# yzqin/s4g-release

Measured on AMD Instinct MI355X. Metric: scenes/sec (25.6k-pt clouds) end-to-end grasp inference, higher is better.
Workload: dtype f32 (f16x2 split)

## Files before the change

include/s4g_ops.h:

```cpp
#ifndef S4G_OPS_H_
#define S4G_OPS_H_

#include <stddef.h>
#include <stdint.h>

#ifdef __cplusplus
extern "C" {
#endif

#define S4G_ABI_VERSION 14


#define S4G_OK 0
#define S4G_EINVAL (-1)
#define S4G_EWORKSPACE (-2)
#define S4G_EUNSUPPORTED (-3)

#define S4G_FLAG_FMAD 1

typedef void *s4g_stream_t;

#define S4G_OP_FPS 1
#define S4G_OP_BALL_QUERY 2
#define S4G_OP_THREE_NN 3

int s4g_abi_version(void);
int s4g_build_variants(void);
int s4g_test_knobs_enabled(void);
const char *s4g_error_string(int code);

size_t s4g_workspace_bytes(int op, int64_t B, int64_t d0, int64_t d1, int64_t d2);

int s4g_fps_f32(const float *xyz_b3n, int64_t B, int64_t N, int64_t M,
                int64_t *idx_bm, void *ws, size_t ws_bytes, int flags,
                s4g_stream_t stream);

int s4g_ball_query_f32(const float *xyz_b3n, const float *ctr_b3m, int64_t B,
                       int64_t N, int64_t M, float radius, int64_t K,
                       int64_t *idx_bmk, int64_t *cnt_bm, void *ws,
                       size_t ws_bytes, int flags, s4g_stream_t stream);

int s4g_group_points_f32(const float *in_bcn, const int64_t *idx_bmk, int64_t B,
                         int64_t C, int64_t N, int64_t M, int64_t K,
                         float *out_bcmk, s4g_stream_t stream);

int s4g_group_points_xyz_f32(const float *xyz_b3n, const int64_t *idx_bmk, int64_t B, int64_t N,
                             int64_t M, int64_t K, float *out_b3mk, void *ws, size_t ws_bytes,
                             s4g_stream_t stream);
int s4g_group_points_ws_f32(const float *feat_bcn, const int64_t *idx_bmk, int64_t B, int64_t C,
                            int64_t N, int64_t M, int64_t K, float *out_bcmk, void *ws,
                            size_t ws_bytes, s4g_stream_t stream);
int s4g_group_points_backward_f32(const float *gout_bcmk,
                                  const int64_t *idx_bmk, int64_t B, int64_t C,
                                  int64_t N, int64_t M, int64_t K,
                                  float *gin_bcn, s4g_stream_t stream);

int s4g_gather_points_f32(const float *in_bcn, const int64_t *idx_bm, int64_t B,
                          int64_t C, int64_t N, int64_t M, float *out_bcm,
                          s4g_stream_t stream);

int s4g_three_nn_f32(const float *q_b3n1, const float *k_b3n2, int64_t B,
                     int64_t N1, int64_t N2, int64_t *idx_bn3, float *d2_bn3,
                     void *ws, size_t ws_bytes, int flags, s4g_stream_t stream);

int s4g_three_interpolate_f32(const float *feat_bcn2, const int64_t *idx_bn3,
                              const float *w_bn3, int64_t B, int64_t C,
                              int64_t N2, int64_t N1, float *out_bcn1,
                              int flags, s4g_stream_t stream);

int s4g_three_interpolate_ws_f32(const float *feat_bcn2, const int64_t *idx_bn3, const float *w_bn3,
                                 int64_t B, int64_t C, int64_t N2, int64_t N1, float *out_bcn1,
                                 void *ws, size_t ws_bytes, int flags, s4g_stream_t stream);
int s4g_interp_add_cl_f32(const float *y_pc, const float *sparse_rc, const int32_t *nidx_p3,
                          const float *nw_p3, const float *bias_c, int64_t B, int64_t N1, int64_t N2,
                          int64_t C, int relu, float *out_pc, float *out_amax64, s4g_stream_t stream);
int s4g_three_interpolate_backward_f32(const float *gout_bcn1,
                                       const int64_t *idx_bn3,
                                       const float *w_bn3, int64_t B, int64_t C,
                                       int64_t N2, int64_t N1, float *gin_bcn2,
                                       s4g_stream_t stream);

size_t s4g_scatter_det_workspace_bytes(int64_t B, int64_t N, int64_t T);
size_t s4g_scatter_det_workspace_bytes_c(int64_t B, int64_t C, int64_t N, int64_t T, int weighted);
int s4g_group_points_backward_det_f32(const float *gout_bcmk, const int64_t *idx_bmk, int64_t B, int64_t C,
                                      int64_t N, int64_t M, int64_t K, float *gin_bcn, void *ws,
                                      size_t ws_bytes, s4g_stream_t stream);
int s4g_three_interpolate_backward_det_f32(const float *gout_bcn1, const int64_t *idx_bn3, const float *w_bn3,
                                           int64_t B, int64_t C, int64_t N2, int64_t N1, float *gin_bcn2,
                                           void *ws, size_t ws_bytes, s4g_stream_t stream);

int s4g_interp_weights_f32(const float *d2_bn3, int64_t B, int64_t N1,
                           float eps, float *w_bn3, s4g_stream_t stream);


#define S4G_GEMM_LOAD_PLAIN 0
#define S4G_GEMM_LOAD_GATHER 1
#define S4G_GEMM_LOAD_INTERP 2
#define S4G_GEMM_LOAD_GATHER_MLP1 3
#define S4G_GEMM_LOAD_GATHER_ADD 4
#define S4G_GEMM_LOAD_INTERP_ADD 5
#define S4G_GEMM_LOAD_CHANNEL_FIRST 6
#define S4G_GEMM_EPI_STORE 0
#define S4G_GEMM_EPI_MAX 1
#define S4G_GEMM_EPI_CHANNEL_FIRST 2
#define S4G_GEMM_EPI_MAX_CHANNEL_FIRST 3
#define S4G_GEMM_FP32 0
#define S4G_GEMM_BF16X3 1
#define S4G_GEMM_BF16 2
#define S4G_GEMM_F16X2 3

typedef struct s4g_gemm_desc {
  int32_t loader, epilogue, groups, relu;
  int32_t P, Cin, Kpad, Cout;
  const float *W;
  const float *bias;
  int32_t w_gstride, b_gstride;
  const float *A;
  int32_t lda, a_coff, a_gcol;
  const int32_t *gidx;
  const float *feat;
  const float *xyz;
  const float *ctr;
  int32_t Cf, N, M, K;
  const int32_t *nidx;
  const float *nw;
  const float *sparse;
  const float *dense;
  int32_t C2, C1, N2, N1;
  float *out;
  int32_t ldc, c_coff, c_gcol;
  float *cf_ptr[4];
  int32_t cf_start[5];
  int32_t cf_sigmoid_from, cf_N;
  int32_t precision, Kpad16;
  const void *W_bf16x3;
  const float *mlp1_w;
  const void *W_f16x2;
  const float *w_inv_scale;
  const float *a_amax, *a_amax2;
  float a_amax_floor;
  float *out_amax;
  const void *W_f16x2_frag;
  const void *W2_f16x2_frag;
  const float *w2_inv_scale;
  const float *bias2;
  int32_t Cout2, relu2;
  const void *W3_f16x2_frag;
  const float *w3_inv_scale;
  const float *bias3;
  int32_t Cout3, relu3;
  const float *loader_bias;
  int32_t rows_per_scene;
  const float *rel_xyz4;
  const int32_t *seg4;
  const int32_t *seg_rows;
  float *out2;
  int32_t ldc2, split_n;
  float *out_amax2;
  int32_t a_L;
} s4g_gemm_desc_t;

int s4g_mlp_gemm_f32(const s4g_gemm_desc_t *desc, s4g_stream_t stream);

typedef struct s4g_heads_desc {
  int32_t precision, P, N, ldx;
  int32_t C, H0, H1, H2, H3;
  const float *X;
  const void *W_frag[5];
  const float *bias[5];
  const float *w_inv_scale[5];
  float *out[4];
  int32_t channels[4];
  int32_t sigmoid_head;
  const float *a_amax;
  float a_amax_floor;
  int32_t rows_per_scene;
  const void *pre_W_frag[2];
  const float *pre_bias[2];
  const float *pre_w_inv_scale[2];
  const int32_t *pre_nidx;
  const float *pre_nw;
  const float *pre_sparse;
  const float *pre_dense;
  const float *pre_lbias;
  const float *pre_a_amax2;
  int32_t pre_N2;
  int64_t out_batch_stride;
  int32_t head_mask;
} s4g_heads_desc_t;

int s4g_heads_chain_f32(const s4g_heads_desc_t *desc, s4g_stream_t stream);

int s4g_amax_per_scene_f32(const float *x, int64_t B, int64_t n_per_scene, float *out_slots, s4g_stream_t stream);

int s4g_gemm_chain_supported(int loader, int epilogue, int C, int Kpad16);

int s4g_ball_query_i32(const float *xyz_b3n, const float *ctr_b3m, int64_t B,
                       int64_t N, int64_t M, float radius, int64_t K,
                       int32_t *idx_bmk, int32_t *cnt_bm, void *ws,
                       size_t ws_bytes, int flags, s4g_stream_t stream);
int s4g_three_nn_weights_i32(const float *q_b3n1, const float *k_b3n2, int64_t B,
                             int64_t N1, int64_t N2, float eps, int32_t *idx_bn3,
                             float *w_bn3, void *ws, size_t ws_bytes, int flags,
                             s4g_stream_t stream);
size_t s4g_three_nn_grid_workspace_bytes(int64_t B, int64_t N1, int64_t N2);
size_t s4g_three_nn_grid_header_offset(int64_t B, int64_t N2);
int s4g_three_nn_weights_grid_i32(const float *q_b3n1, const float *k_b3n2, int64_t B,
                                  int64_t N1, int64_t N2, float eps, float cell,
                                  int32_t *idx_bn3, float *w_bn3, void *ws,
                                  size_t ws_bytes, int flags, s4g_stream_t stream);

int s4g_three_nn_grid_f32(const float *q_b3n1, const float *k_b3n2, int64_t B, int64_t N1,
                          int64_t N2, float cell, int64_t *idx_bn3, float *d2_bn3, void *ws,
                          size_t ws_bytes, int flags, s4g_stream_t stream);

int s4g_query_group_f32(const float *xyz_b3n, const float *ctr_b3m, int64_t B,
                        int64_t N, int64_t M, float radius, int64_t K,
                        int64_t *idx_bmk, int64_t *cnt_bm, float *grouped_b3mk,
                        void *ws, size_t ws_bytes, int flags, s4g_stream_t stream);

int s4g_group_rel_xyz_i32(const float *xyz_b3n, const float *ctr_b3m, const int32_t *idx_bmk,
                          int64_t B, int64_t N, int64_t M, int64_t K, float *rel_pk4,
                          s4g_stream_t stream);

int s4g_group_rel_xyz_unique_i32(const float *xyz_b3n, const float *ctr_b3m, const int32_t *idx_bmk,
                                 const int32_t *cnt_bm, int64_t B, int64_t N, int64_t M, int64_t K,
                                 float *rel_pk4, int32_t *seg4, int32_t *row_start_bm, int32_t *rows_b,
                                 s4g_stream_t stream);

int s4g_fps_gather_i32(const float *xyz_b3n, int64_t B, int64_t N, int64_t M,
                       int32_t *idx_bm, float *ctr_b3m, void *ws, size_t ws_bytes,
                       int flags, s4g_stream_t stream);

int s4g_fps_gather_ex_i32(const float *xyz_b3n, int64_t B, int64_t N, int64_t M, int32_t *idx_bm,
                          float *ctr_b3m, float *dist_bm, const int32_t *run_b, void *ws,
                          size_t ws_bytes, int flags, s4g_stream_t stream);
int s4g_fps_prefix_check_f32(const float *ctr_b3m, const float *dist_bm, int64_t B, int64_t M1,
                             int64_t M2, int32_t *run_b, int flags, s4g_stream_t stream);

int s4g_fps_prepass_f32(const float *xyz_b3n, int64_t B, int64_t N, int64_t G, int32_t *perm_bn,
                        float *gbox_bg6, s4g_stream_t stream);

int s4g_expected_score_f32(const float *logits_bcn, int64_t B, int64_t C, int64_t N,
                           const float *values_c, float *score_bn, s4g_stream_t stream);
int s4g_decode_poses_f32(const float *xyz_b3n, const float *frame_R_b9n,
                         const float *frame_t_btn, const int64_t *sel_bk, int64_t B,
                         int64_t N, int64_t K, int64_t TC, const float *t_bins,
                         float *H_bk44, s4g_stream_t stream);

int s4g_contact_heads_f32(const float *raw_b17m, const float *xyz_b3n, const int64_t *index_bm, int64_t B,
                          int64_t N, int64_t M, float *out_b20m, s4g_stream_t stream);
int s4g_decode_poses_abs_f32(const float *frame_R_b9n, const float *frame_t_b3n, const int64_t *sel_bk,
                             int64_t B, int64_t N, int64_t K, float *H_bk44, s4g_stream_t stream);

int s4g_collision_counts_f32(const float *xyz_b3n, const float *g2l_bk44, int64_t B,
                             int64_t N, int64_t K, const float *gripper6,
                             int32_t *counts_bk2, s4g_stream_t stream);
int s4g_collision_counts_n_f32(const float *xyz_b3n, const float *g2l_bk44, int64_t B, int64_t N,
                               int64_t K, const float *gripper6, const int64_t *pose_count_b,
                               int invert_se3, int32_t *counts_bk2, s4g_stream_t stream);

size_t s4g_eval_frames_workspace_bytes(int64_t B, int64_t N, int64_t K);
int s4g_eval_frames_f32(const float *xyz_b3n, const float *normals_b3n, const int32_t *labels_bn,
                        const float *g2l_bk44, int64_t B, int64_t N, int64_t K, const float *params10,
                        const int64_t *pose_count_b, int invert_se3, int32_t *ints_bk8, float *floats_bk5,
                        void *workspace, size_t workspace_bytes, s4g_stream_t stream);

size_t s4g_local_search_workspace_bytes(int64_t B, int64_t N, int64_t F, int64_t L, int64_t T);
int s4g_local_search_f32(const float *points_bf3, const float *frames_bf33, const float *xyz_b3n,
                         const float *normals_b3n, const int32_t *labels_bn, int64_t B, int64_t N, int64_t F,
                         int64_t L, int64_t T, const float *params13, int32_t no_label, const float *tables_3l2t,
                         const int64_t *frame_count_b, int32_t *ints_bfp6, float *scores_bfp, int32_t *slab_bfl,
                         int32_t *valid_bf, int32_t *valid_index_bf, int64_t *count_b, void *workspace,
                         size_t workspace_bytes, s4g_stream_t stream);

int s4g_best_placement_f32(const float *points_bf3, const float *frames_bf33, const float *scores_bfp,
                           const float *tables_3l2t, int64_t B, int64_t F, int64_t L, int64_t T, int32_t *index_bf,
                           float *score_bf, float *g2l_bf44, int32_t *valid_index_bf, int64_t *count_b,
                           s4g_stream_t stream);
size_t s4g_close_region_workspace_bytes(int64_t B, int64_t N, int64_t F, int64_t capacity);
int s4g_close_region_f32(const float *g2l_bf44, const float *xyz_b3n, const float *normals_b3n,
                         const int32_t *live_bf, const int64_t *frame_count_b, int64_t B, int64_t N, int64_t F,
                         int64_t capacity, int64_t R, const float *params13, int32_t *count_bf, int64_t *offset_bf1,
                         float *points_b3c, float *normals_b3c, int32_t *index_bc, float *maps_bf12rr,
                         int32_t *flags_bf, void *workspace, size_t workspace_bytes, s4g_stream_t stream);

size_t s4g_gpd_pack_bytes(int Cin, int classes);
int s4g_gpd_pack_f32(const float *conv1_w, const float *conv1_b, const float *conv2_w, const float *conv2_b,
                     const float *fc1_w, const float *fc1_b, const float *fc2_w, const float *fc2_b, int Cin, int classes,
                     void *packed, s4g_stream_t stream);
size_t s4g_gpd_workspace_bytes(int64_t chunk, int Cin, int classes);
int s4g_gpd_forward_f32(const float *maps, int64_t image_stride, int64_t channel_stride, const int32_t *index, int64_t G,
                        int64_t num_images, const void *packed, int Cin, int classes, int64_t chunk, float *pool1,
                        float *pool2, float *hidden, float *logits, void *workspace, size_t workspace_bytes,
                        s4g_stream_t stream);

size_t s4g_pngpd_pack_bytes(int classes);
int s4g_pngpd_pack_f32(const float *const *weights12, const float *const *biases12, int classes, void *packed,
                       s4g_stream_t stream);
size_t s4g_pngpd_workspace_bytes(int64_t chunk, int classes);
int s4g_pngpd_forward_f32(const float *points, int64_t set_stride, int64_t channel_stride, int64_t n_points,
                          const int64_t *offset, const int32_t *count, const int32_t *flags, int64_t F, int64_t capacity,
                          const int32_t *index, int64_t G, int64_t num_sets, const void *packed, int classes,
                          int64_t chunk, float *stn_global, float *trans, float *global_feat, float *hidden,
                          int32_t *status, float *logits, void *workspace, size_t workspace_bytes, s4g_stream_t stream);

size_t s4g_darboux_frames_workspace_bytes(int64_t B, int64_t N, int64_t F);
int s4g_darboux_frames_f32(const float *xyz_b3n, const float *normals_b3n, const int32_t *frame_index_bf,
                           const int64_t *frame_count_b, int64_t B, int64_t N, int64_t F, float radius,
                           int32_t min_neighbours, float *frames_bf33, float *points_bf3, int32_t *count_bf,
                           int32_t *flags_bf, void *workspace, size_t workspace_bytes, s4g_stream_t stream);

size_t s4g_match_normals_workspace_bytes(int64_t B, int64_t N, int64_t M);
int s4g_match_normals_f32(const float *query_b3n, const float *scene_b3m, const float *scene_normals_b3m,
                          const float *camera_b3 , int64_t B, int64_t N, int64_t M, float radius,
                          int32_t max_nn, float *normals_b3n, int32_t *count_bn, int32_t *flags_bn,
                          void *workspace, size_t workspace_bytes, s4g_stream_t stream);

size_t s4g_estimate_normals_workspace_bytes(int64_t B, int64_t N);
int s4g_estimate_normals_f32(const float *cloud_b3n, const float *camera_b3 ,
                             const int32_t *live_b , int64_t B, int64_t N, float radius,
                             int32_t max_nn, float *normals_b3n, int32_t *count_bn, int32_t *flags_bn,
                             void *workspace, size_t workspace_bytes, s4g_stream_t stream);

int s4g_match_nearest_f32(const float *query_b3n, const float *scene_b3m, int64_t B, int64_t N, int64_t M,
                          float radius, int32_t *nearest_bn, void *workspace, size_t workspace_bytes,
                          s4g_stream_t stream);

size_t s4g_contact_search_workspace_bytes(int64_t B, int64_t M, int64_t F, int64_t P);
int s4g_contact_search_f32(const float *g2l_bf44, const float *xyz_b3m, const int32_t *labels_bm, int64_t B, int64_t M,
                           int64_t F, int64_t nz, int64_t ny, int64_t nx, const float *params10, int32_t no_label,
                           const float *tables_2z3y2x, const int64_t *frame_count_b, int32_t *ints_bfp4,
                           int32_t *table_bf, int32_t *valid_bf, int32_t *label_bf, int32_t *fail_bf, void *workspace,
                           size_t workspace_bytes, s4g_stream_t stream);

int s4g_contact_select_f32(const int32_t *nearest_bn, const float *cloud_b3n, const float *scene_normals_b3m,
                           const float *camera_b3, const int32_t *offsets_bm1, const int32_t *order_bf,
                           const int32_t *valid_bf, const float *search_bf, const float *antipodal_bf, int64_t B,
                           int64_t N, int64_t M, int64_t F, float *normals_b3n, int32_t *best_frame_bn,
                           float *point_score_bn, int32_t *valid_index_bn, int64_t *count_b, s4g_stream_t stream);

size_t s4g_contact_pairs_workspace_bytes(int64_t B, int64_t N);
int s4g_contact_pairs_f32(const float *xyz_b3n, const float *normals_b3n, const int64_t *count_b, int64_t B, int64_t N,
                          int64_t max_pairs, double max_distance, double cos_threshold, int32_t *pairs_bp2,
                          float *pair_score_bp, int64_t *pair_count_b, int32_t *flags_b, void *workspace,
                          size_t workspace_bytes, s4g_stream_t stream);
size_t s4g_contact_pair_grade_workspace_bytes(int64_t B, int64_t N, int64_t P, int64_t T, int64_t W);
int s4g_contact_pair_grade_f32(const float *xyz_b3n, const int64_t *count_b, const int32_t *pairs_bp2,
                               const float *pair_score_bp, const int64_t *pair_count_b, int64_t B, int64_t N, int64_t P,
                               int64_t T, int64_t W, const float *params5, const double *gates3,
                               const float *tables_12t2w, int64_t max_frames, int32_t *counts_bptw3,
                               int32_t *close_plane_bp, float *score_bpt, int32_t *valid_bpt, int32_t *fail_bp,
                               float *g2l_bf44, float *search_score_bf, float *antipodal_score_bf,
                               int32_t *frame_source_bf, int32_t *frame_point_index_bf, int64_t *frame_count_b,
                               int32_t *flags_b, void *workspace, size_t workspace_bytes, s4g_stream_t stream);

size_t s4g_darboux_object_frames_workspace_bytes(int64_t B, int64_t N);
int s4g_darboux_object_frames_f32(const float *xyz_b3n, const float *normals_b3n, const int64_t *count_b, int64_t B,
                                  int64_t N, float radius, int32_t min_neighbours, float *frames_bn33,
                                  float *inv_frames_bn33, int32_t *neighbours_bn, int32_t *flags_bn, void *workspace,
                                  size_t workspace_bytes, s4g_stream_t stream);
size_t s4g_darboux_object_grade_workspace_bytes(int64_t B, int64_t N, int64_t F, int64_t L, int64_t T, int64_t S);
int s4g_darboux_object_grade_f32(const float *xyz_b3n, const float *normals_b3n, const int64_t *count_b,
                                 const float *frames_bf33, const float *inv_frames_bf33, const int32_t *frame_index_bf,
                                 int64_t B, int64_t N, int64_t F, int64_t L, int64_t T, int64_t S, const float *params9,
                                 const float *tables_3l2t2s, int32_t *search_bf2lt, float *antipodal_bf2lt,
                                 int32_t *counts_bf2lts3, int32_t *slab_bf2l, int32_t *fail_bf2, void *workspace,
                                 size_t workspace_bytes, s4g_stream_t stream);

size_t s4g_sort_pairs_workspace_bytes(int64_t n);
int s4g_sort_pairs_u32(uint32_t *keys_in, uint32_t *vals_in, int64_t n, int bits, uint32_t *keys_out,
                       uint32_t *vals_out, void *ws, size_t ws_bytes, s4g_stream_t stream);
size_t s4g_exclusive_scan_workspace_bytes(int64_t n);
int s4g_exclusive_scan_i32(const int32_t *in, int32_t *out, int64_t n, void *ws, size_t ws_bytes,
                           s4g_stream_t stream);

int s4g_crop_indices_f32(const float *xyz_3n, int64_t N, const float *workspace6,
// ... 33 lines not shown
```

s4g_release_amd/_cabi.py:

```python
import ctypes
import os

_HERE = os.path.dirname(os.path.abspath(__file__))
LIB_PATH = os.environ.get("S4G_HIP_LIB") or os.path.join(_HERE, "libs4g_hip.so")

S4G_ABI_VERSION = 14
S4G_EINVAL = -1
S4G_EWORKSPACE = -2
S4G_EUNSUPPORTED = -3
S4G_FLAG_FMAD = 1
S4G_OP_FPS, S4G_OP_BALL_QUERY, S4G_OP_THREE_NN = 1, 2, 3

_vp = ctypes.c_void_p
_i64 = ctypes.c_int64
_sz = ctypes.c_size_t
_int = ctypes.c_int
_f32 = ctypes.c_float

_i32 = ctypes.c_int32


class GemmDesc(ctypes.Structure):
    _fields_ = [
        ("loader", _i32), ("epilogue", _i32), ("groups", _i32), ("relu", _i32),
        ("P", _i32), ("Cin", _i32), ("Kpad", _i32), ("Cout", _i32),
        ("W", _vp), ("bias", _vp), ("w_gstride", _i32), ("b_gstride", _i32),
        ("A", _vp), ("lda", _i32), ("a_coff", _i32), ("a_gcol", _i32),
        ("gidx", _vp), ("feat", _vp), ("xyz", _vp), ("ctr", _vp),
        ("Cf", _i32), ("N", _i32), ("M", _i32), ("K", _i32),
        ("nidx", _vp), ("nw", _vp), ("sparse", _vp), ("dense", _vp),
        ("C2", _i32), ("C1", _i32), ("N2", _i32), ("N1", _i32),
        ("out", _vp), ("ldc", _i32), ("c_coff", _i32), ("c_gcol", _i32),
        ("cf_ptr", _vp * 4), ("cf_start", _i32 * 5), ("cf_sigmoid_from", _i32), ("cf_N", _i32),
        ("precision", _i32), ("Kpad16", _i32), ("W_bf16x3", _vp), ("mlp1_w", _vp),
        ("W_f16x2", _vp), ("w_inv_scale", _vp), ("a_amax", _vp), ("a_amax2", _vp),
        ("a_amax_floor", _f32), ("out_amax", _vp), ("W_f16x2_frag", _vp),
        ("W2_f16x2_frag", _vp), ("w2_inv_scale", _vp), ("bias2", _vp), ("Cout2", _i32), ("relu2", _i32),
        ("W3_f16x2_frag", _vp), ("w3_inv_scale", _vp), ("bias3", _vp), ("Cout3", _i32), ("relu3", _i32),
        ("loader_bias", _vp), ("rows_per_scene", _i32), ("rel_xyz4", _vp), ("seg4", _vp), ("seg_rows", _vp),
        ("out2", _vp), ("ldc2", _i32), ("split_n", _i32), ("out_amax2", _vp),
        ("a_L", _i32),
    ]


class HeadsDesc(ctypes.Structure):
    _fields_ = [
        ("precision", _i32), ("P", _i32), ("N", _i32), ("ldx", _i32),
        ("C", _i32), ("H0", _i32), ("H1", _i32), ("H2", _i32), ("H3", _i32),
        ("X", _vp), ("W_frag", _vp * 5), ("bias", _vp * 5), ("w_inv_scale", _vp * 5),
        ("out", _vp * 4), ("channels", _i32 * 4), ("sigmoid_head", _i32),
        ("a_amax", _vp), ("a_amax_floor", _f32), ("rows_per_scene", _i32),
        ("pre_W_frag", _vp * 2), ("pre_bias", _vp * 2), ("pre_w_inv_scale", _vp * 2),
        ("pre_nidx", _vp), ("pre_nw", _vp), ("pre_sparse", _vp), ("pre_dense", _vp),
        ("pre_lbias", _vp), ("pre_a_amax2", _vp), ("pre_N2", _i32), ("out_batch_stride", _i64), ("head_mask", _i32),
    ]


SIGNATURES = {
    "s4g_mlp_gemm_f32": (_int, [ctypes.POINTER(GemmDesc), _vp]),
    "s4g_heads_chain_f32": (_int, [ctypes.POINTER(HeadsDesc), _vp]),
    "s4g_ball_query_i32": (_int, [_vp, _vp, _i64, _i64, _i64, _f32, _i64, _vp, _vp, _vp, _sz,
                                  _int, _vp]),
    "s4g_three_nn_weights_i32": (_int, [_vp, _vp, _i64, _i64, _i64, _f32, _vp, _vp, _vp, _sz,
                                        _int, _vp]),
    "s4g_three_nn_grid_workspace_bytes": (_sz, [_i64, _i64, _i64]),
    "s4g_three_nn_grid_header_offset": (_sz, [_i64, _i64]),
    "s4g_three_nn_weights_grid_i32": (_int, [_vp, _vp, _i64, _i64, _i64, _f32, _f32, _vp, _vp, _vp,
                                             _sz, _int, _vp]),
    "s4g_three_nn_grid_f32": (_int, [_vp, _vp, _i64, _i64, _i64, _f32, _vp, _vp, _vp, _sz, _int, _vp]),
    "s4g_group_points_xyz_f32": (_int, [_vp, _vp, _i64, _i64, _i64, _i64, _vp, _vp, _sz, _vp]),
    "s4g_gemm_chain_supported": (_int, [_int, _int, _int, _int]),
    "s4g_amax_per_scene_f32": (_int, [_vp, _i64, _i64, _vp, _vp]),
    "s4g_interp_add_cl_f32": (_int, [_vp, _vp, _vp, _vp, _vp, _i64, _i64, _i64, _i64, _int, _vp, _vp, _vp]),
    "s4g_group_points_ws_f32": (_int, [_vp, _vp, _i64, _i64, _i64, _i64, _i64, _vp, _vp, _sz, _vp]),
    "s4g_three_interpolate_ws_f32": (_int, [_vp, _vp, _vp, _i64, _i64, _i64, _i64, _vp, _vp, _sz, _int, _vp]),
    "s4g_fps_gather_i32": (_int, [_vp, _i64, _i64, _i64, _vp, _vp, _vp, _sz, _int, _vp]),
    "s4g_fps_prepass_f32": (_int, [_vp, _i64, _i64, _i64, _vp, _vp, _vp]),
    "s4g_fps_gather_ex_i32": (_int, [_vp, _i64, _i64, _i64, _vp, _vp, _vp, _vp, _vp, _sz, _int, _vp]),
    "s4g_fps_prefix_check_f32": (_int, [_vp, _vp, _i64, _i64, _i64, _vp, _int, _vp]),
    "s4g_build_variants": (_int, []),
    "s4g_test_knobs_enabled": (_int, []),
    "s4g_fps_f64": (_int, [_vp, _i64, _i64, _i64, _vp, _vp, _sz, _int, _vp]),
    "s4g_ball_query_f64": (_int, [_vp, _vp, _i64, _i64, _i64, _f32, _i64, _vp, _vp, _int, _vp]),
    "s4g_three_nn_f64": (_int, [_vp, _vp, _i64, _i64, _i64, _vp, _vp, _int, _vp]),
    "s4g_group_points_f64": (_int, [_vp, _vp, _i64, _i64, _i64, _i64, _i64, _vp, _vp]),
    "s4g_group_points_backward_f64": (_int, [_vp, _vp, _i64, _i64, _i64, _i64, _i64, _vp, _vp]),
    "s4g_three_interpolate_f64": (_int, [_vp, _vp, _vp, _i64, _i64, _i64, _i64, _vp, _int, _vp]),
    "s4g_three_interpolate_backward_f64": (_int, [_vp, _vp, _vp, _i64, _i64, _i64, _i64, _vp, _vp]),
    "s4g_scatter_det_workspace_bytes": (_sz, [_i64, _i64, _i64]),
    "s4g_scatter_det_workspace_bytes_c": (_sz, [_i64, _i64, _i64, _i64, _int]),
    "s4g_group_points_backward_det_f32": (_int, [_vp, _vp, _i64, _i64, _i64, _i64, _i64, _vp, _vp, _sz, _vp]),
    "s4g_three_interpolate_backward_det_f32": (_int, [_vp, _vp, _vp, _i64, _i64, _i64, _i64, _vp, _vp, _sz, _vp]),
    "s4g_group_rel_xyz_i32": (_int, [_vp, _vp, _vp, _i64, _i64, _i64, _i64, _vp, _vp]),
    "s4g_group_rel_xyz_unique_i32": (_int, [_vp, _vp, _vp, _vp, _i64, _i64, _i64, _i64, _vp, _vp, _vp, _vp, _vp]),
    "s4g_expected_score_f32": (_int, [_vp, _i64, _i64, _i64, _vp, _vp, _vp]),
    "s4g_decode_poses_f32": (_int, [_vp, _vp, _vp, _vp, _i64, _i64, _i64, _i64, _vp, _vp, _vp]),
    "s4g_contact_heads_f32": (_int, [_vp, _vp, _vp, _i64, _i64, _i64, _vp, _vp]),
    "s4g_decode_poses_abs_f32": (_int, [_vp, _vp, _vp, _i64, _i64, _i64, _vp, _vp]),
    "s4g_collision_counts_f32": (_int, [_vp, _vp, _i64, _i64, _i64, ctypes.POINTER(ctypes.c_float),
                                        _vp, _vp]),
    "s4g_collision_counts_n_f32": (_int, [_vp, _vp, _i64, _i64, _i64, ctypes.POINTER(ctypes.c_float),
                                          _vp, _int, _vp, _vp]),
    "s4g_eval_frames_workspace_bytes": (_sz, [_i64, _i64, _i64]),
    "s4g_eval_frames_f32": (_int, [_vp, _vp, _vp, _vp, _i64, _i64, _i64, ctypes.POINTER(ctypes.c_float), _vp, _int,
                                   _vp, _vp, _vp, _sz, _vp]),
    "s4g_local_search_workspace_bytes": (_sz, [_i64, _i64, _i64, _i64, _i64]),
    "s4g_local_search_f32": (_int, [_vp, _vp, _vp, _vp, _vp, _i64, _i64, _i64, _i64, _i64,
                                    ctypes.POINTER(ctypes.c_float), _i32, _vp, _vp, _vp, _vp, _vp, _vp, _vp, _vp, _vp,
                                    _sz, _vp]),
    "s4g_best_placement_f32": (_int, [_vp, _vp, _vp, _vp, _i64, _i64, _i64, _i64, _vp, _vp, _vp, _vp, _vp, _vp]),
    "s4g_close_region_workspace_bytes": (_sz, [_i64, _i64, _i64, _i64]),
    "s4g_close_region_f32": (_int, [_vp, _vp, _vp, _vp, _vp, _i64, _i64, _i64, _i64, _i64,
                                    ctypes.POINTER(ctypes.c_float), _vp, _vp, _vp, _vp, _vp, _vp, _vp, _vp, _sz, _vp]),
    "s4g_gpd_pack_bytes": (_sz, [_int, _int]),
    "s4g_gpd_pack_f32": (_int, [_vp, _vp, _vp, _vp, _vp, _vp, _vp, _vp, _int, _int, _vp, _vp]),
    "s4g_gpd_workspace_bytes": (_sz, [_i64, _int, _int]),
    "s4g_gpd_forward_f32": (_int, [_vp, _i64, _i64, _vp, _i64, _i64, _vp, _int, _int, _i64, _vp, _vp, _vp, _vp, _vp, _sz,
                                   _vp]),
    "s4g_pngpd_pack_bytes": (_sz, [_int]),
    "s4g_pngpd_pack_f32": (_int, [_vp, _vp, _int, _vp, _vp]),
    "s4g_pngpd_workspace_bytes": (_sz, [_i64, _int]),
    "s4g_pngpd_forward_f32": (_int, [_vp, _i64, _i64, _i64, _vp, _vp, _vp, _i64, _i64, _vp, _i64, _i64, _vp, _int, _i64,
                                     _vp, _vp, _vp, _vp, _vp, _vp, _vp, _sz, _vp]),
    "s4g_darboux_frames_workspace_bytes": (_sz, [_i64, _i64, _i64]),
    "s4g_darboux_frames_f32": (_int, [_vp, _vp, _vp, _vp, _i64, _i64, _i64, _f32, _i32, _vp, _vp, _vp, _vp, _vp, _sz,
                                      _vp]),
    "s4g_match_normals_workspace_bytes": (_sz, [_i64, _i64, _i64]),
    "s4g_match_normals_f32": (_int, [_vp, _vp, _vp, _vp, _i64, _i64, _i64, _f32, _i32, _vp, _vp, _vp, _vp, _sz, _vp]),
    "s4g_match_nearest_f32": (_int, [_vp, _vp, _i64, _i64, _i64, _f32, _vp, _vp, _sz, _vp]),
    "s4g_estimate_normals_workspace_bytes": (_sz, [_i64, _i64]),
    "s4g_estimate_normals_f32": (_int, [_vp, _vp, _vp, _i64, _i64, _f32, _i32, _vp, _vp, _vp, _vp, _sz, _vp]),
    "s4g_contact_search_workspace_bytes": (_sz, [_i64, _i64, _i64, _i64]),
    "s4g_contact_search_f32": (_int, [_vp, _vp, _vp, _i64, _i64, _i64, _i64, _i64, _i64, ctypes.POINTER(ctypes.c_float),
                                      _i32, _vp, _vp, _vp, _vp, _vp, _vp, _vp, _vp, _sz, _vp]),
    "s4g_contact_select_f32": (_int, [_vp, _vp, _vp, _vp, _vp, _vp, _vp, _vp, _vp, _i64, _i64, _i64, _i64, _vp, _vp,
                                      _vp, _vp, _vp, _vp]),
    "s4g_contact_pairs_workspace_bytes": (_sz, [_i64, _i64]),
    "s4g_contact_pairs_f32": (_int, [_vp, _vp, _vp, _i64, _i64, _i64, ctypes.c_double, ctypes.c_double, _vp, _vp, _vp,
                                     _vp, _vp, _sz, _vp]),
    "s4g_contact_pair_grade_workspace_bytes": (_sz, [_i64, _i64, _i64, _i64, _i64]),
    "s4g_contact_pair_grade_f32": (_int, [_vp, _vp, _vp, _vp, _vp, _i64, _i64, _i64, _i64, _i64,
                                          ctypes.POINTER(ctypes.c_float), ctypes.POINTER(ctypes.c_double), _vp, _i64,
                                          _vp, _vp, _vp, _vp, _vp, _vp, _vp, _vp, _vp, _vp, _vp, _vp, _vp, _sz, _vp]),
    "s4g_darboux_object_frames_workspace_bytes": (_sz, [_i64, _i64]),
    "s4g_darboux_object_frames_f32": (_int, [_vp, _vp, _vp, _i64, _i64, _f32, _i32, _vp, _vp, _vp, _vp, _vp, _sz, _vp]),
    "s4g_darboux_object_grade_workspace_bytes": (_sz, [_i64, _i64, _i64, _i64, _i64, _i64]),
    "s4g_darboux_object_grade_f32": (_int, [_vp, _vp, _vp, _vp, _vp, _vp, _i64, _i64, _i64, _i64, _i64, _i64,
                                            ctypes.POINTER(ctypes.c_float), _vp, _vp, _vp, _vp, _vp, _vp, _vp, _sz,
                                            _vp]),
    "s4g_sort_pairs_workspace_bytes": (_sz, [_i64]),
    "s4g_sort_pairs_u32": (_int, [_vp, _vp, _i64, _int, _vp, _vp, _vp, _sz, _vp]),
    "s4g_exclusive_scan_workspace_bytes": (_sz, [_i64]),
    "s4g_exclusive_scan_i32": (_int, [_vp, _vp, _i64, _vp, _sz, _vp]),
    "s4g_query_group_f32": (_int, [_vp, _vp, _i64, _i64, _i64, _f32, _i64, _vp, _vp, _vp, _vp, _sz,
                                   _int, _vp]),
    "s4g_crop_indices_f32": (_int, [_vp, _i64, ctypes.POINTER(ctypes.c_float), _vp, _vp, _vp]),
    "s4g_voxel_down_sample_workspace_bytes": (_sz, [_i64]),
    "s4g_voxel_down_sample_f32": (_int, [_vp, _i64, _f32, ctypes.POINTER(ctypes.c_float),
                                         ctypes.POINTER(ctypes.c_int32), _vp, _vp, _vp, _sz, _vp]),
    "s4g_radius_outlier_workspace_bytes": (_sz, [_i64]),
    "s4g_radius_outlier_mask_f32": (_int, [_vp, _i64, _f32, _i32, _vp, _vp, _sz, _int, _vp]),
    "s4g_abi_version": (_int, []),
    "s4g_error_string": (ctypes.c_char_p, [_int]),
    "s4g_workspace_bytes": (_sz, [_int, _i64, _i64, _i64, _i64]),
    "s4g_fps_f32": (_int, [_vp, _i64, _i64, _i64, _vp, _vp, _sz, _int, _vp]),
    "s4g_ball_query_f32": (_int, [_vp, _vp, _i64, _i64, _i64, _f32, _i64, _vp, _vp, _vp, _sz,
                                  _int, _vp]),
    "s4g_group_points_f32": (_int, [_vp, _vp, _i64, _i64, _i64, _i64, _i64, _vp, _vp]),
    "s4g_group_points_backward_f32": (_int, [_vp, _vp, _i64, _i64, _i64, _i64, _i64, _vp, _vp]),
    "s4g_gather_points_f32": (_int, [_vp, _vp, _i64, _i64, _i64, _i64, _vp, _vp]),
    "s4g_three_nn_f32": (_int, [_vp, _vp, _i64, _i64, _i64, _vp, _vp, _vp, _sz, _int, _vp]),
    "s4g_three_interpolate_f32": (_int, [_vp, _vp, _vp, _i64, _i64, _i64, _i64, _vp, _int, _vp]),
    "s4g_three_interpolate_backward_f32": (_int, [_vp, _vp, _vp, _i64, _i64, _i64, _i64, _vp,
                                                  _vp]),
    "s4g_interp_weights_f32": (_int, [_vp, _i64, _i64, _f32, _vp, _vp]),
}

_lib = None


def lib():
    global _lib
    if _lib is not None:
        return _lib
    if not os.path.exists(LIB_PATH):
        raise RuntimeError(
            "libs4g_hip.so not found at %s -- build it with "
            "`python -c 'import __graft_entry__ as g; g.build()'` or "
            "`make -C s4g_release_amd/csrc`. There is no CPU fallback." % LIB_PATH)
    import torch
    if os.environ.get("S4G_HIP_LIB"):
        import warnings
        warnings.warn("S4G_HIP_LIB overrides the shipped library: loading %s" % LIB_PATH, RuntimeWarning,
                      stacklevel=2)
    L = ctypes.CDLL(LIB_PATH)
    for name, (res, args) in SIGNATURES.items():
        try:
            fn = getattr(L, name)
        except AttributeError:
            raise RuntimeError("libs4g_hip.so does not export %s" % name)
        fn.restype = res
        fn.argtypes = args
    ver = L.s4g_abi_version()
    if ver != S4G_ABI_VERSION:
        raise RuntimeError("libs4g_hip.so ABI version %d != expected %d" % (ver, S4G_ABI_VERSION))
    _lib = L
    return _lib


def knob(name, default=None):
    if os.environ.get("S4G_TEST_KNOBS") != "1":
        return default
    return os.environ.get(name, default)


def check(code, what):
    if code != 0:
        msg = lib().s4g_error_string(code)
        raise RuntimeError("%s failed: %s (code %d)" % (what, msg.decode() if msg else "?", code))
```

s4g_release_amd/csrc/group.hip:

```cpp
#include "s4g_common.h"

namespace s4g {

constexpr int GP_THREADS = 256;
constexpr int GP_CG = 8;

__global__ __launch_bounds__(GP_THREADS) void group_points_vec4_kernel(
    const float* __restrict__ in, const int64_t* __restrict__ idx, int C, int N,
    int64_t MK, float* __restrict__ out) {
  const int b = blockIdx.z;
  const int c0 = blockIdx.y * GP_CG;
  const int64_t t4 = ((int64_t)blockIdx.x * GP_THREADS + threadIdx.x) * 4;
  if (t4 >= MK) return;
  const longlong2* ip =
      reinterpret_cast<const longlong2*>(idx + (size_t)b * MK + t4);
  const longlong2 a = ip[0], c = ip[1];
  const int j0 = (int)a.x, j1 = (int)a.y, j2 = (int)c.x, j3 = (int)c.y;
  const int cend = min(c0 + GP_CG, C);
  for (int ch = c0; ch < cend; ++ch) {
    const float* __restrict__ src = in + ((size_t)b * C + ch) * N;
    float4 v;
    v.x = src[j0];
    v.y = src[j1];
    v.z = src[j2];
// ... 6 lines not shown
                                                                float4* __restrict__ aos) {
  const int j = blockIdx.x * GP_THREADS + threadIdx.x;
  const int b = blockIdx.y;
  if (j >= N) return;
  const float* p = in + (size_t)b * 3 * N;
  aos[(size_t)b * N + j] = make_float4(p[j], p[N + j], p[2 * (size_t)N + j], 0.f);
}

__global__ __launch_bounds__(GP_THREADS) void group_xyz_aos_kernel(const float4* __restrict__ aos,
                                                                   const int64_t* __restrict__ idx,
                                                                   int N, int64_t MK,
                                                                   float* __restrict__ out) {
  const int b = blockIdx.y;
  const int64_t t4 = ((int64_t)blockIdx.x * GP_THREADS + threadIdx.x) * 4;
  if (t4 >= MK) return;
  const longlong2* ip = reinterpret_cast<const longlong2*>(idx + (size_t)b * MK + t4);
  const longlong2 a = ip[0], c = ip[1];
  const float4* __restrict__ src = aos + (size_t)b * N;
  const float4 p0 = src[(int)a.x], p1 = src[(int)a.y], p2 = src[(int)c.x], p3 = src[(int)c.y];
  float* o = out + (size_t)b * 3 * MK + t4;
  *reinterpret_cast<float4*>(o) = make_float4(p0.x, p1.x, p2.x, p3.x);
  *reinterpret_cast<float4*>(o + MK) = make_float4(p0.y, p1.y, p2.y, p3.y);
  *reinterpret_cast<float4*>(o + 2 * MK) = make_float4(p0.z, p1.z, p2.z, p3.z);
}

__global__ __launch_bounds__(GP_THREADS) void group_rel_xyz_kernel(const float* __restrict__ xyz,
                                                                   const float* __restrict__ ctr,
                                                                   const int* __restrict__ idx, int N,
                                                                   int M, int K,
                                                                   float4* __restrict__ out) {
  const int b = blockIdx.y;
  const int64_t MK = (int64_t)M * K;
  const int64_t t = (int64_t)blockIdx.x * GP_THREADS + threadIdx.x;
  if (t >= MK) return;
  const int m = (int)(t / K);
  const int j = idx[(size_t)b * MK + t];
  const float* __restrict__ x = xyz + (size_t)b * 3 * N;
  const float* __restrict__ c = ctr + (size_t)b * 3 * M;
  out[(size_t)b * MK + t] = make_float4(__fsub_rn(x[j], c[m]), __fsub_rn(x[N + j], c[M + m]),
                                        __fsub_rn(x[2 * (size_t)N + j], c[2 * (size_t)M + m]), 0.f);
}

constexpr int GU_THREADS = 1024, GU_TILE = 256;
__global__ __launch_bounds__(GU_THREADS) void group_unique_scan_kernel(const int* __restrict__ cnt, int M, int K,
                                                                       int* __restrict__ row_start,
                                                                       int* __restrict__ rows,
                                                                       float4* __restrict__ out,
                                                                       int* __restrict__ seg4) {
  __shared__ int wsum[GU_THREADS / 64];
  __shared__ int total_s;
  const int b = blockIdx.x, t = threadIdx.x, lane = t & 63, wave = t >> 6;
  const int per = (M + GU_THREADS - 1) / GU_THREADS;
  const int m0 = t * per;
  int local = 0;
  for (int i = 0; i < per; ++i) {
    const int m = m0 + i;
    if (m < M) local += (max(cnt[(size_t)b * M + m], 1) + 3) & ~3;
  }
  int incl = local;
#pragma unroll
  for (int o = 1; o < 64; o <<= 1) {
    const int v = __shfl_up(incl, o);
    if (lane >= o) incl += v;
  }
  if (lane == 63) wsum[wave] = incl;
  __syncthreads();
  if (t == 0) {
    int run = 0;
    for (int w = 0; w < GU_THREADS / 64; ++w) {
      const int v = wsum[w];
      wsum[w] = run;
      run += v;
    }
    total_s = run;
  }
  __syncthreads();
  int start = wsum[wave] + incl - local;
  for (int i = 0; i < per; ++i) {
    const int m = m0 + i;
    if (m < M) {
      row_start[(size_t)b * M + m] = start;
      start += (max(cnt[(size_t)b * M + m], 1) + 3) & ~3;
    }
  }
  if (total_s > (int)((int64_t)M * K / 8 * 7) || (total_s + GU_TILE - 1) / GU_TILE * GU_TILE >= M * K) {
    for (int i = 0; i < per; ++i) {
      const int m = m0 + i;
      if (m < M) row_start[(size_t)b * M + m] = m * K;
    }
    if (t == 0) rows[b] = M * K;
    return;
  }
  const int total = total_s;
  const int padded = (total + GU_TILE - 1) / GU_TILE * GU_TILE;
  if (t == 0) rows[b] = padded;
  const size_t base = (size_t)b * M * K;
  for (int r = total + t; r < padded; r += GU_THREADS) {
    out[base + r] = make_float4(0.f, 0.f, 0.f, 0.f);
    if ((r & 3) == 0) seg4[(base + r) >> 2] = -1;
  }
}

__global__ __launch_bounds__(GP_THREADS) void group_rel_unique_kernel(const float* __restrict__ xyz,
                                                                      const float* __restrict__ ctr,
                                                                      const int* __restrict__ idx,
                                                                      const int* __restrict__ cnt,
                                                                      const int* __restrict__ row_start,
                                                                      const int* __restrict__ rows, int N,
                                                                      int M, int K, float4* __restrict__ out,
                                                                      int* __restrict__ seg4) {
  const int b = blockIdx.y;
  const int64_t MK = (int64_t)M * K;
  const int64_t t = (int64_t)blockIdx.x * GP_THREADS + threadIdx.x;
  if (t >= MK) return;
  const int m = (int)(t / K), k = (int)(t - (int64_t)m * K);
  const int c4 = rows[b] == M * K ? K : (max(cnt[(size_t)b * M + m], 1) + 3) & ~3;
  if (k >= c4) return;
  const int j = idx[(size_t)b * MK + t];
  const float* __restrict__ x = xyz + (size_t)b * 3 * N;
  const float* __restrict__ c = ctr + (size_t)b * 3 * M;
  const size_t row = (size_t)b * MK + row_start[(size_t)b * M + m] + k;
  out[row] = make_float4(__fsub_rn(x[j], c[m]), __fsub_rn(x[N + j], c[M + m]),
                         __fsub_rn(x[2 * (size_t)N + j], c[2 * (size_t)M + m]), 0.f);
  if ((k & 3) == 0) seg4[row >> 2] = b * M + m;
}

__global__ __launch_bounds__(GP_THREADS) void group_points_scalar_kernel(
    const float* __restrict__ in, const int64_t* __restrict__ idx, int C, int N,
    int64_t MK, float* __restrict__ out) {
  const int b = blockIdx.z;
  const int c0 = blockIdx.y * GP_CG;
  const int64_t t = (int64_t)blockIdx.x * GP_THREADS + threadIdx.x;
  if (t >= MK) return;
  const int j = (int)idx[(size_t)b * MK + t];
  const int cend = min(c0 + GP_CG, C);
  for (int ch = c0; ch < cend; ++ch)
    out[((size_t)b * C + ch) * MK + t] = in[((size_t)b * C + ch) * N + j];
}

__global__ __launch_bounds__(GP_THREADS) void group_points_backward_kernel(
    const float* __restrict__ gout, const int64_t* __restrict__ idx, int C,
    int N, int64_t MK, float* __restrict__ gin) {
  const int b = blockIdx.z;
  const int c0 = blockIdx.y * GP_CG;
  const int64_t t = (int64_t)blockIdx.x * GP_THREADS + threadIdx.x;
  if (t >= MK) return;
  const int j = (int)idx[(size_t)b * MK + t];
  const int cend = min(c0 + GP_CG, C);
  for (int ch = c0; ch < cend; ++ch)
    atomicAdd(gin + ((size_t)b * C + ch) * N + j,
              gout[((size_t)b * C + ch) * MK + t]);
}

}

extern "C" int s4g_group_points_f32(const float* in_bcn,
                                    const int64_t* idx_bmk, int64_t B,
                                    int64_t C, int64_t N, int64_t M, int64_t K,
                                    float* out_bcmk, s4g_stream_t stream) {
  if (B < 0 || C < 0 || N <= 0 || M < 0 || K < 0 || B > 65535 ||
      N >= (1ll << 31))
    return S4G_EINVAL;
  const int64_t MK = M * K;
  if (B == 0 || C == 0 || MK == 0) return S4G_OK;
  if (!in_bcn || !idx_bmk || !out_bcmk) return S4G_EINVAL;
  hipStream_t st = (hipStream_t)stream;
  const unsigned gy = (unsigned)((C + s4g::GP_CG - 1) / s4g::GP_CG);
  if (gy > 65535) return S4G_EINVAL;
  const bool aligned = ((uintptr_t)idx_bmk % 16 == 0) && ((uintptr_t)out_bcmk % 16 == 0);
  if (MK % 4 == 0 && aligned) {
    const dim3 grid((unsigned)((MK / 4 + s4g::GP_THREADS - 1) / s4g::GP_THREADS),
                    gy, (unsigned)B);
    hipLaunchKernelGGL(s4g::group_points_vec4_kernel, grid,
                       dim3(s4g::GP_THREADS), 0, st, in_bcn, idx_bmk, (int)C,
                       (int)N, MK, out_bcmk);
  } else {
    const dim3 grid((unsigned)((MK + s4g::GP_THREADS - 1) / s4g::GP_THREADS),
                    gy, (unsigned)B);
    hipLaunchKernelGGL(s4g::group_points_scalar_kernel, grid,
                       dim3(s4g::GP_THREADS), 0, st, in_bcn, idx_bmk, (int)C,
                       (int)N, MK, out_bcmk);
  }
  S4G_LAUNCH_CHECK();
  return S4G_OK;
}

extern "C" int s4g_group_points_xyz_f32(const float* xyz_b3n, const int64_t* idx_bmk, int64_t B,
                                        int64_t N, int64_t M, int64_t K, float* out_b3mk,
                                        void* ws, size_t ws_bytes, s4g_stream_t stream) {
  const int64_t MK = M * K;
  const bool aligned = ((uintptr_t)idx_bmk % 16 == 0) && ((uintptr_t)out_b3mk % 16 == 0) &&
                       ((uintptr_t)ws % 16 == 0);
  if (!ws || ws_bytes < (size_t)B * (size_t)N * sizeof(float4) || MK % 4 != 0 || !aligned ||
      B <= 0 || B > 65535 || N <= 0 || N >= (1ll << 31) || MK == 0)
    return s4g_group_points_f32(xyz_b3n, idx_bmk, B, 3, N, M, K, out_b3mk, stream);
  if (!xyz_b3n || !idx_bmk || !out_b3mk) return S4G_EINVAL;
  hipStream_t st = (hipStream_t)stream;
  float4* aos = (float4*)ws;
  hipLaunchKernelGGL(s4g::xyz_to_aos_kernel, dim3((unsigned)((N + s4g::GP_THREADS - 1) / s4g::GP_THREADS), (unsigned)B),
                     dim3(s4g::GP_THREADS), 0, st, xyz_b3n, (int)N, aos);
  S4G_LAUNCH_CHECK();
  hipLaunchKernelGGL(s4g::group_xyz_aos_kernel,
                     dim3((unsigned)((MK / 4 + s4g::GP_THREADS - 1) / s4g::GP_THREADS), (unsigned)B),
                     dim3(s4g::GP_THREADS), 0, st, aos, idx_bmk, (int)N, MK, out_b3mk);
  S4G_LAUNCH_CHECK();
  return S4G_OK;
}

extern "C" int s4g_group_rel_xyz_i32(const float* xyz_b3n, const float* ctr_b3m, const int32_t* idx_bmk,
                                     int64_t B, int64_t N, int64_t M, int64_t K, float* rel_pk4,
                                     s4g_stream_t stream) {
  if (B < 0 || N <= 0 || M < 0 || K < 0 || B > 65535 || N >= (1ll << 31) || M * K >= (1ll << 31))
    return S4G_EINVAL;
  const int64_t MK = M * K;
  if (B == 0 || MK == 0) return S4G_OK;
  if (!xyz_b3n || !ctr_b3m || !idx_bmk || !rel_pk4 || ((uintptr_t)rel_pk4 & 15)) return S4G_EINVAL;
  hipStream_t st = (hipStream_t)stream;
  hipLaunchKernelGGL(s4g::group_rel_xyz_kernel,
                     dim3((unsigned)((MK + s4g::GP_THREADS - 1) / s4g::GP_THREADS), (unsigned)B),
                     dim3(s4g::GP_THREADS), 0, st, xyz_b3n, ctr_b3m, idx_bmk, (int)N, (int)M, (int)K,
                     reinterpret_cast<float4*>(rel_pk4));
  S4G_LAUNCH_CHECK();
  return S4G_OK;
}

extern "C" int s4g_group_rel_xyz_unique_i32(const float* xyz_b3n, const float* ctr_b3m, const int32_t* idx_bmk,
                                            const int32_t* cnt_bm, int64_t B, int64_t N, int64_t M, int64_t K,
                                            float* rel_pk4, int32_t* seg4, int32_t* row_start_bm,
                                            int32_t* rows_b, s4g_stream_t stream) {
  if (B < 0 || N <= 0 || M < 0 || K < 0 || B > 65535 || N >= (1ll << 31) || B * M * K >= (1ll << 31))
    return S4G_EINVAL;
  const int64_t MK = M * K;
  if (B == 0 || MK == 0) return S4G_OK;
  if ((K & 3) || (MK % s4g::GU_TILE) || M > s4g::GU_THREADS * 64) return S4G_EUNSUPPORTED;
  if (!xyz_b3n || !ctr_b3m || !idx_bmk || !cnt_bm || !rel_pk4 || !seg4 || !row_start_bm || !rows_b ||
      ((uintptr_t)rel_pk4 & 15))
    return S4G_EINVAL;
  hipStream_t st = (hipStream_t)stream;
  hipLaunchKernelGGL(s4g::group_unique_scan_kernel, dim3((unsigned)B), dim3(s4g::GU_THREADS), 0, st, cnt_bm, (int)M,
                     (int)K, row_start_bm, rows_b, reinterpret_cast<float4*>(rel_pk4), seg4);
  S4G_LAUNCH_CHECK();
  hipLaunchKernelGGL(s4g::group_rel_unique_kernel,
                     dim3((unsigned)((MK + s4g::GP_THREADS - 1) / s4g::GP_THREADS), (unsigned)B),
                     dim3(s4g::GP_THREADS), 0, st, xyz_b3n, ctr_b3m, idx_bmk, cnt_bm, row_start_bm, rows_b, (int)N, (int)M,
                     (int)K, reinterpret_cast<float4*>(rel_pk4), seg4);
  S4G_LAUNCH_CHECK();
  return S4G_OK;
}

extern "C" int s4g_group_points_backward_f32(const float* gout_bcmk,
                                             const int64_t* idx_bmk, int64_t B,
                                             int64_t C, int64_t N, int64_t M,
                                             int64_t K, float* gin_bcn,
                                             s4g_stream_t stream) {
  if (B < 0 || C < 0 || N <= 0 || M < 0 || K < 0 || B > 65535 ||
      N >= (1ll << 31))
    return S4G_EINVAL;
  if (B == 0 || C == 0) return S4G_OK;
  if (!gin_bcn) return S4G_EINVAL;
  hipStream_t st = (hipStream_t)stream;
  hipError_t e = hipMemsetAsync(gin_bcn, 0, sizeof(float) * (size_t)(B * C * N), st);
  if (e != hipSuccess) return (int)e;
  const int64_t MK = M * K;
  if (MK == 0) return S4G_OK;
  if (!gout_bcmk || !idx_bmk) return S4G_EINVAL;
  const unsigned gy = (unsigned)((C + s4g::GP_CG - 1) / s4g::GP_CG);
  if (gy > 65535) return S4G_EINVAL;
  const dim3 grid((unsigned)((MK + s4g::GP_THREADS - 1) / s4g::GP_THREADS), gy,
                  (unsigned)B);
  hipLaunchKernelGGL(s4g::group_points_backward_kernel, grid,
                     dim3(s4g::GP_THREADS), 0, st, gout_bcmk, idx_bmk, (int)C,
                     (int)N, MK, gin_bcn);
  S4G_LAUNCH_CHECK();
  return S4G_OK;
}

extern "C" int s4g_gather_points_f32(const float* in_bcn, const int64_t* idx_bm,
                                     int64_t B, int64_t C, int64_t N, int64_t M,
                                     float* out_bcm, s4g_stream_t stream) {
  return s4g_group_points_f32(in_bcn, idx_bm, B, C, N, M, 1, out_bcm, stream);
}
```

s4g_release_amd/csrc/mlp_gemm.hip:

```cpp
#include <stdlib.h>

#include "mlp_common.h"

#include <type_traits>

#ifndef S4G_CHAIN_ABLATE
#define S4G_CHAIN_ABLATE 0
#endif

namespace s4g {


constexpr int GM_BM = 128;
constexpr int GM_BN = 128;
constexpr int GM_BK = 32;
constexpr int GM_LDS = 36;
constexpr int GM_THREADS = 256;

enum { LOAD_PLAIN = 0, LOAD_GATHER = 1, LOAD_INTERP = 2, LOAD_GATHER_MLP1 = 3, LOAD_GATHER_ADD = 4,
       LOAD_INTERP_ADD = 5, LOAD_CHANNEL_FIRST = 6,
       LOAD_REL_MLP1 = 64,
       LOAD_ADD_MFMA0 = 65 };
enum { EPI_STORE = 0, EPI_MAX = 1, EPI_CHANNEL_FIRST = 2, EPI_MAX_CF = 3 };

struct GemmParams {
  int P, Cin, Kpad, Cout, relu;
  const float* W;
  const float* bias;
  const float* A;
  int lda, a_coff, a_gcol;
  int aL;
  const int* gidx;
  const float* feat;
  const float* xyz;
  const float* ctr;
  int Cf, N, M, K;
  int nscenes;
  const float4* mlp1;
  const float4* rel4;
  const int* seg4;
  const int* seg_rows;
  float* out2;
  int ldc2, split_n;
  uint32_t* out_amax2;
  const int* nidx;
  const float* nw;
  const float* sparse;
  const float* dense;
  int C2, C1, N2, N1;
  float* out;
  int ldc, c_coff, c_gcol;
  int w_gstride, b_gstride;
  float* cf_ptr[4];
  int cf_start[5];
  int cf_sigmoid_from;
  int cf_N;
  int mtiles, ntiles;
  const uint16_t* W3;
  int Kpad16;
  int bf16_single;
  size_t w3_plane;
  const uint16_t* Wh2;
  const float* w_inv_scale;
  const float* a_amax;
  const float* a_amax2;
  float a_amax_floor;
  uint32_t* out_amax;
  int rps;
  const uint16_t* Wfrag;
  const float* lbias;
  const uint16_t* Wfrag2;
  const float* w_inv_scale2;
  const float* bias2;
  int Cout2, relu2;
  const uint16_t* Wfrag3;
  const float* w_inv_scale3;
  const float* bias3;
  int Cout3, relu3;
};

__device__ __forceinline__ float4 f4zero() { return make_float4(0.f, 0.f, 0.f, 0.f); }

__device__ __forceinline__ void gather_row_bm(int M, int K, int p0, int r, int& b, int& m) {
  const int MK = M * K;
  const int b0 = __builtin_amdgcn_readfirstlane(p0 / MK);
  int rem = p0 - b0 * MK + r;
  b = b0;
  while (rem >= MK) {
    rem -= MK;
    ++b;
  }
  m = (K & (K - 1)) == 0 ? rem >> (31 - __clz(K)) : rem / K;
}

template <int LOADER, int RPT = 4, int RS = 32>
struct ALoader {
  static __device__ __forceinline__ int srow(int t) { return LOADER == LOAD_CHANNEL_FIRST ? (t & 31) : (t >> 3); }
  static __device__ __forceinline__ int chunk(int t) { return LOADER == LOAD_CHANNEL_FIRST ? (t >> 5) : (t & 7); }
  const float* src0[RPT];
  bool ok[RPT];
  float rel[RPT][3];
  int i3[RPT][3];
  float w3[RPT][3];
  size_t drow[RPT];

  __device__ __forceinline__ void init(const GemmParams& p, int p0, int g, int t) {
    constexpr bool GATHERS = LOADER == LOAD_GATHER_MLP1 || LOADER == LOAD_GATHER_ADD || LOADER == LOAD_GATHER;
    int pp_[RPT], j_[RPT], b_[RPT], m_[RPT];
#pragma unroll
    for (int s = 0; s < RPT; ++s) {
      const int r = srow(t) + RS * s;
      const int pos = p0 + r;
      ok[s] = pos < p.P;
      pp_[s] = ok[s] ? pos : 0;
      j_[s] = b_[s] = m_[s] = 0;
      if constexpr (GATHERS) {
        if (!(LOADER == LOAD_GATHER_MLP1 && p.rel4)) {
          gather_row_bm(p.M, p.K, p0, ok[s] ? r : 0, b_[s], m_[s]);
          j_[s] = p.gidx[pp_[s]];
        }
      }
    }
#pragma unroll
    for (int s = 0; s < RPT; ++s) {
      const int pp = pp_[s], j = j_[s], b = b_[s], m = m_[s];
      if constexpr (LOADER == LOAD_PLAIN) {
        src0[s] = p.A + (size_t)pp * p.lda + p.a_coff + g * p.a_gcol;
      } else if constexpr (LOADER == LOAD_CHANNEL_FIRST) {
        const int b = pp / p.aL;
        src0[s] = p.A + (size_t)b * p.Cin * p.aL + (pp - b * p.aL);
      } else if constexpr (LOADER == LOAD_GATHER_MLP1) {
        if (p.rel4) {
          const float4 r4 = p.rel4[pp];
          rel[s][0] = r4.x;
          rel[s][1] = r4.y;
          rel[s][2] = r4.z;
          continue;
        }
        const float* x = p.xyz + (size_t)b * 3 * p.N;
        const float* c = p.ctr + (size_t)b * 3 * p.M;
        rel[s][0] = __fsub_rn(x[j], c[m]);
        rel[s][1] = __fsub_rn(x[p.N + j], c[p.M + m]);
        rel[s][2] = __fsub_rn(x[2 * p.N + j], c[2 * p.M + m]);
      } else if constexpr (LOADER == LOAD_GATHER_ADD) {
        src0[s] = p.feat + ((size_t)b * p.N + j) * p.Cf;
        const float* x = p.xyz + (size_t)b * 3 * p.N;
        const float* c = p.ctr + (size_t)b * 3 * p.M;
        rel[s][0] = __fsub_rn(x[j], c[m]);
        rel[s][1] = __fsub_rn(x[p.N + j], c[p.M + m]);
        rel[s][2] = __fsub_rn(x[2 * p.N + j], c[2 * p.M + m]);
      } else if constexpr (LOADER == LOAD_GATHER) {
        src0[s] = p.feat ? p.feat + ((size_t)b * p.N + j) * p.Cf : nullptr;
        if ((t & 7) == ((p.Cf & 31) >> 2)) {
          const float* x = p.xyz + (size_t)b * 3 * p.N;
          const float* c = p.ctr + (size_t)b * 3 * p.M;
          rel[s][0] = __fsub_rn(x[j], c[m]);
          rel[s][1] = __fsub_rn(x[p.N + j], c[p.M + m]);
          rel[s][2] = __fsub_rn(x[2 * p.N + j], c[2 * p.M + m]);
        }
      } else {
        const int bq = pp / p.N1;
#pragma unroll
        for (int k = 0; k < 3; ++k) {
          i3[s][k] = bq * p.N2 + p.nidx[(size_t)pp * 3 + k];
          w3[s][k] = p.nw[(size_t)pp * 3 + k];
        }
        drow[s] = (size_t)pp;
      }
    }
  }

  __device__ __forceinline__ float4 load(const GemmParams& p, int s, int k0, int t) const {
    if constexpr (LOADER == LOAD_GATHER_MLP1) {
      const bool live = ok[s] && k0 < p.Cin;
      const int kk = k0 < p.Cin ? k0 : 0;
      float4 r;
      float* rp = reinterpret_cast<float*>(&r);
#pragma unroll
      for (int e = 0; e < 4; ++e) {
        const float4 w = p.mlp1[kk + e];
        const float v = __fmaf_rn(w.z, rel[s][2], __fmaf_rn(w.y, rel[s][1], __fmaf_rn(w.x, rel[s][0], w.w)));
        rp[e] = live ? fmaxf(v, 0.f) : 0.f;
      }
      return r;
    }
    if constexpr (LOADER == LOAD_GATHER_ADD) {
      const bool live = ok[s] && k0 < p.Cin;
      const int kk = k0 < p.Cin ? k0 : 0;
      const float4 f = *reinterpret_cast<const float4*>(src0[s] + kk);
      const float fv[4] = {f.x, f.y, f.z, f.w};
      float4 r;
      float* rp = reinterpret_cast<float*>(&r);
#pragma unroll
      for (int e = 0; e < 4; ++e) {
        const float4 w = p.mlp1[kk + e];
        const float v = __fmaf_rn(w.z, rel[s][2], __fmaf_rn(w.y, rel[s][1], __fmaf_rn(w.x, rel[s][0], w.w)));
        rp[e] = live ? fmaxf(__fadd_rn(fv[e], v), 0.f) : 0.f;
      }
      return r;
    }
    if (!ok[s]) return f4zero();
    if constexpr (LOADER == LOAD_PLAIN) {
      if (k0 >= p.Cin) return f4zero();
      return *reinterpret_cast<const float4*>(src0[s] + k0);
    } else if constexpr (LOADER == LOAD_CHANNEL_FIRST) {
      float v[4];
#pragma unroll
      for (int e = 0; e < 4; ++e) v[e] = k0 + e < p.Cin ? src0[s][(size_t)(k0 + e) * p.aL] : 0.f;
      return make_float4(v[0], v[1], v[2], v[3]);
    } else if constexpr (LOADER == LOAD_INTERP_ADD) {
      if (k0 >= p.Cin) return f4zero();
      const float4 a = *reinterpret_cast<const float4*>(p.sparse + (size_t)i3[s][0] * p.C2 + k0);
      const float4 b = *reinterpret_cast<const float4*>(p.sparse + (size_t)i3[s][1] * p.C2 + k0);
      const float4 c = *reinterpret_cast<const float4*>(p.sparse + (size_t)i3[s][2] * p.C2 + k0);
      const float4 bb = *reinterpret_cast<const float4*>(p.lbias + k0);
      float4 y = f4zero();
      if (p.dense) y = *reinterpret_cast<const float4*>(p.dense + drow[s] * p.C2 + k0);
      const float av[4] = {a.x, a.y, a.z, a.w}, bv[4] = {b.x, b.y, b.z, b.w}, cv[4] = {c.x, c.y, c.z, c.w};
      const float yv[4] = {y.x, y.y, y.z, y.w}, bi[4] = {bb.x, bb.y, bb.z, bb.w};
      float4 r;
      float* rp = reinterpret_cast<float*>(&r);
#pragma unroll
      for (int e = 0; e < 4; ++e) {
        float acc = __fmul_rn(av[e], w3[s][0]);
        acc = __fadd_rn(acc, __fmul_rn(bv[e], w3[s][1]));
        acc = __fadd_rn(acc, __fmul_rn(cv[e], w3[s][2]));
        rp[e] = fmaxf(__fadd_rn(__fadd_rn(yv[e], acc), bi[e]), 0.f);
      }
      return r;
    } else if constexpr (LOADER == LOAD_GATHER) {
      if (k0 < p.Cf) return *reinterpret_cast<const float4*>(src0[s] + k0);
      if (k0 == p.Cf) return make_float4(rel[s][0], rel[s][1], rel[s][2], 0.f);
      return f4zero();
    } else {
      if (k0 < p.C2) {
        const float4 a = *reinterpret_cast<const float4*>(p.sparse + (size_t)i3[s][0] * p.C2 + k0);
        const float4 b = *reinterpret_cast<const float4*>(p.sparse + (size_t)i3[s][1] * p.C2 + k0);
        const float4 c = *reinterpret_cast<const float4*>(p.sparse + (size_t)i3[s][2] * p.C2 + k0);
        float4 r;
        r.x = __fadd_rn(__fadd_rn(__fmul_rn(a.x, w3[s][0]), __fmul_rn(b.x, w3[s][1])), __fmul_rn(c.x, w3[s][2]));
        r.y = __fadd_rn(__fadd_rn(__fmul_rn(a.y, w3[s][0]), __fmul_rn(b.y, w3[s][1])), __fmul_rn(c.y, w3[s][2]));
        r.z = __fadd_rn(__fadd_rn(__fmul_rn(a.z, w3[s][0]), __fmul_rn(b.z, w3[s][1])), __fmul_rn(c.z, w3[s][2]));
        r.w = __fadd_rn(__fadd_rn(__fmul_rn(a.w, w3[s][0]), __fmul_rn(b.w, w3[s][1])), __fmul_rn(c.w, w3[s][2]));
        return r;
      }
// ... 572 lines not shown
#pragma unroll
    for (int pl = 0; pl < PL; ++pl)
#pragma unroll
      for (int s = 0; s < WPT; ++s)
        rw[pl][s] = (wlive && wok[s])
                        ? *reinterpret_cast<const uint4*>(Wg + pl * p.w3_plane + woff[s] + kt * BK)
                        : make_uint4(0u, 0u, 0u, 0u);
  };
  auto lstore = [&]() {
#pragma unroll
    for (int s = 0; s < RPT; ++s) {
      uint16_t* dst = Ah + (srow + RS * s) * GH_STR + (((chunk >> 1) ^ ((srow >> 2) & 3)) * 8) + (chunk & 1) * 4;
      if constexpr (PL == 2) {
        uint2 h, l;
        split2_h<LOADER == LOAD_GATHER>(ra[s], sa, h, l);
        *reinterpret_cast<uint2*>(dst) = h;
        *reinterpret_cast<uint2*>(dst + APLANE) = l;
      } else {
        *reinterpret_cast<uint2*>(dst) = make_uint2(cvt_pk_bf16(ra[s].x, ra[s].y), cvt_pk_bf16(ra[s].z, ra[s].w));
      }
    }
#pragma unroll
    for (int pl = 0; pl < PL; ++pl)
#pragma unroll
      for (int s = 0; s < WPT; ++s)
        *reinterpret_cast<uint4*>(Wh + pl * WPLANE + (wrow + WRS * s) * GH_STR +
                                  ((wchunk ^ ((wrow >> 2) & 3)) * 8)) = rw[pl][s];
  };

#define S4G_H2_TERM(PA, PB)                                                        \
  acc[0][cp] = chain_mfma<PL>(af[0][PA], bf[0][PB], acc[0][cp]);                     \
  acc[0][cp + 1] = chain_mfma<PL>(af[0][PA], bf[1][PB], acc[0][cp + 1]);             \
  acc[1][cp] = chain_mfma<PL>(af[1][PA], bf[0][PB], acc[1][cp]);                     \
  acc[1][cp + 1] = chain_mfma<PL>(af[1][PA], bf[1][PB], acc[1][cp + 1]);
  auto compute_ks = [&](int ks) {
    uint4 af[2][PL];
#pragma unroll
    for (int rb = 0; rb < 2; ++rb)
#pragma unroll
      for (int pl = 0; pl < PL; ++pl)
        af[rb][pl] = *reinterpret_cast<const uint4*>(Ah + pl * APLANE + a_row + rb * 32 * GH_STR + f_off[ks]);
#pragma unroll
    for (int cp = 0; cp < NCB; cp += 2) {
      uint4 bf[2][PL];
#pragma unroll
      for (int cb = 0; cb < 2; ++cb)
#pragma unroll
        for (int pl = 0; pl < PL; ++pl)
          bf[cb][pl] = *reinterpret_cast<const uint4*>(Wh + pl * WPLANE + b_row + (cp + cb) * 32 * GH_STR + f_off[ks]);
      if constexpr (PL == 2) {
        S4G_H2_TERM(0, 1)
        S4G_H2_TERM(1, 0)
      }
      S4G_H2_TERM(0, 0)
    }
  };

  gload(0);
  for (int kt = 0; kt < ntile_k; ++kt) {
    lstore();
    __syncthreads();
    if (kt + 1 < ntile_k) gload(kt + 1);
    const int krem = p.Kpad16 - kt * BK;
    const int nks = krem >= BK ? 2 : 1;
    for (int ks = 0; ks < nks; ++ks) compute_ks(ks);
    __syncthreads();
  }
#undef S4G_H2_TERM

  float tmax = 0.f;
#pragma unroll
  for (int cb = 0; cb < NCB; ++cb) {
    const int n = n0 + wc * 32 * NCB + cb * 32 + li;
    const bool nok = n < p.Cout;
    const float sc = nok ? (PL == 2 ? inv_sa * p.w_inv_scale[(size_t)g * p.b_gstride + n] : 1.f) : 0.f;
    const float bias = nok ? bg[n] : 0.f;
    float mx = -__builtin_inff(), mn = __builtin_inff();
#pragma unroll
    for (int rb = 0; rb < 2; ++rb)
#pragma unroll
      for (int r = 0; r < 16; ++r) {
        const float v = acc[rb][cb][r] * sc;
        acc[rb][cb][r] = v;
        mx = fmaxf(mx, v);
        mn = fminf(mn, v);
      }
    const float hi = mx + bias, lo = mn + bias;
    tmax = fmaxf(tmax, p.relu ? hi : fmaxf(fabsf(hi), fabsf(lo)));
  }
  if (PL == 2 && po.out_amax) {
    const uint32_t wm = wave_max_u32(__float_as_uint(fmaxf(tmax, 0.f)));
    if (lane == 0) amax_publish(po.out_amax, wm, blockIdx.x * 4 + wave, p0, p_hi, p.rps);
  }
  if constexpr (EPI == EPI_MAX_CF)
    max_cf_epilogue<NCB>(po, acc, bg, p0, n0, wr, wc, li, lh, smemf);
  else
    gemm_epilogue<EPI, NCB>(po, acc, bg, g, p0, n0, wave, wr, wc, li, lh, smemf);
}

template <int LOADER, int EPI, int NCB, int PL>
static int launch_gemm_f16x2_cfg(GemmParams p, int groups, hipStream_t st) {
  constexpr int BN = 64 * NCB;
  p.ntiles = (p.Cout + BN - 1) / BN;
  size_t lds = sizeof(uint16_t) * PL * (GM_BM + BN) * GH_STR;
  const size_t epi = sizeof(float) * 4 * 32 * (32 * NCB + 4);
  if (lds < epi) lds = epi;
  static LdsAttrCache lds_cache;
  if (int rc = allow_dynamic_lds(reinterpret_cast<const void*>(&mlp_gemm_f16x2_kernel<LOADER, EPI, NCB, PL>), lds, lds_cache)) return rc;
  const dim3 grid((unsigned)(p.mtiles * p.ntiles), (unsigned)groups);
  hipLaunchKernelGGL((mlp_gemm_f16x2_kernel<LOADER, EPI, NCB, PL>), grid, dim3(256), lds, st, p);
  S4G_LAUNCH_CHECK();
  return S4G_OK;
}

__device__ __forceinline__ void chain_keep_alive(const f32x16& v) { asm volatile("" ::"v"(v)); }

#ifdef S4G_CHAIN_STAMPS
__device__ unsigned long long g_chain_stamps[512 * 16];
#define S4G_STAMP(i)                                                                       \
  do {                                                                                     \
    const unsigned sb_ = gridDim.x >= 1024 ? blockIdx.x - gridDim.x / 2 : blockIdx.x;    \
    if (threadIdx.x == 0 && sb_ < 512u && blockIdx.y == 0)                                 \
      g_chain_stamps[sb_ * 16 + (i)] = __builtin_amdgcn_s_memtime();                      \
  } while (0)
#else
#define S4G_STAMP(i)
#endif
constexpr int GF_RING_F16X2 = 2;
#ifndef S4G_CHAIN_RING1
#define S4G_CHAIN_RING1 2
#endif
#ifndef S4G_CHAIN_BF16_NRB
#define S4G_CHAIN_BF16_NRB 4
#endif

template <int LOADER, int EPI2, int RW, int KC, int PL>
__global__ __launch_bounds__(RW == 8 ? 512 : 256, (PL == 1 && RW != 8 && S4G_CHAIN_BF16_NRB == 2) ? 3 : 2) void mlp_chain_kernel(const GemmParams p) {
  constexpr int GF_RING = PL == 2 ? GF_RING_F16X2 : S4G_CHAIN_RING1;
  constexpr int NRB = PL == 1 ? S4G_CHAIN_BF16_NRB : 2, WROWS = 32 * NRB;
  constexpr int CW = RW == 8 ? 8 : 4 / RW, RWN = RW == 8 ? 1 : RW;
  constexpr int BM = WROWS * RWN, K = 64 * CW, NW = RWN * CW;
  constexpr int RS = 8 * NW, RPT = BM / RS;
  constexpr int astr = K + 8, aplane = BM * astr, KS = K >> 4;
  extern __shared__ __attribute__((aligned(16))) float smemf[];
  uint16_t* Ah = reinterpret_cast<uint16_t*>(smemf);
  float* scr = reinterpret_cast<float*>(Ah + PL * aplane);
  const int g = blockIdx.y;

  const int t = threadIdx.x;
  const int lane = t & 63;
  const int wave = t >> 6;

  constexpr bool ADD0 = LOADER == LOAD_ADD_MFMA0;
  constexpr bool ADD_BOUNDS = LOADER == LOAD_GATHER_ADD || LOADER == LOAD_INTERP_ADD || ADD0;
  constexpr bool MFMA0 = LOADER == LOAD_REL_MLP1;
  static_assert(!(MFMA0 || ADD0) || (PL == 2 && KC == 1), "phase 0 on the matrix cores: f16x2, one panel");
  static_assert(!ADD0 || EPI2 == EPI_MAX, "a wave's 64 rows are one centroid's neighbours");
  constexpr bool SEGMAX = (LOADER == LOAD_GATHER_MLP1 || MFMA0) && EPI2 == EPI_MAX;
  const int tile = blockIdx.x;
  const int p0 = tile * BM;
  bool seg_scene = false;
  if constexpr (SEGMAX) {
    if (p.seg_rows) {
      const int sc = p0 / p.rps;
      const int nrows = p.seg_rows[sc];
      if (p0 - sc * p.rps >= nrows) return;
      seg_scene = nrows < p.rps;
    }
  }
  const int p_hi = min(p0 + BM, p.P) - 1;
  const int am_s0 = p.rps > 0 ? p0 / p.rps : 0, am_s1 = p.rps > 0 ? p_hi / p.rps : 0;
  float am_v1 = 0.f, am_v2 = 0.f;
  if (PL == 2 && p.a_amax) am_v1 = p.a_amax[(size_t)am_s0 * 64 + lane];
  if (PL == 2 && p.a_amax2) am_v2 = p.a_amax2[(size_t)am_s0 * 64 + lane];

  const int wr = wave / CW, wc = wave % CW;
  const int li = lane & 31, lh = lane >> 5;
  const int wc_u = __builtin_amdgcn_readfirstlane(wc);
  const uint32_t wf_lane = (uint32_t)lane * 16u;
  constexpr size_t cb_stride = (size_t)KS * PL * 1024;
  constexpr size_t strip_stride = (size_t)CW * 2 * cb_stride;
  constexpr int kchunks = KC;
  const size_t cbs1 = (size_t)kchunks * cb_stride;
  const WRef w1 = wref(p.Wfrag + (size_t)g * p.Cout * p.Kpad16 * PL, (size_t)(wc_u * 2) * cbs1);
  const bool tri = p.Wfrag3 != nullptr;
  const WRef wmid = wref(p.Wfrag2 + (size_t)g * p.Cout2 * K * PL, (size_t)(wc_u * 2) * cb_stride);
  const int CoutF = tri ? p.Cout3 : p.Cout2;
  const float* __restrict__ scF = PL == 2 ? (tri ? p.w_inv_scale3 : p.w_inv_scale2) + (size_t)g * CoutF : nullptr;
  const float* __restrict__ bgF = (tri ? p.bias3 : p.bias2) + (size_t)g * CoutF;
  const WRef w2 = tri ? wref(p.Wfrag3 + (size_t)g * CoutF * K * PL, (size_t)(wc_u * 2) * cb_stride) : wmid;
  const int nstrip2 = (CoutF + 64 * CW - 1) / (64 * CW);
  const bool active0 = wc_u * 64 < CoutF;

  uint4 ring[GF_RING][2][PL];
#pragma unroll
  for (int d = 0; d < GF_RING; ++d)
#pragma unroll
    for (int cb = 0; cb < 2; ++cb)
#pragma unroll
      for (int pl = 0; pl < PL; ++pl)
        ring[d][cb][pl] = wref_load(w1, wf_lane + pl * 1024, (uint32_t)(cb * cbs1 + (size_t)d * PL * 1024));

  S4G_STAMP(0);
  ALoader<LOADER, RPT, RS> ld;
  float4 rv0[NRB];
  float4 wv0 = f4zero();
  constexpr int NKT0 = ADD0 ? K / 32 : 1, RPT0 = ADD0 ? RPT : 1;
  float4 fa[NKT0][RPT0];
  constexpr int fstr = K + 4;
  if constexpr (ADD0) {
    const int rows_left = p.P - p0;
    const __amdgpu_buffer_rsrc_t ridx = __builtin_amdgcn_make_buffer_rsrc(
        const_cast<int*>(p.gidx + p0), 0, (rows_left < BM ? rows_left : BM) * 4, 0x00020000);
    const __amdgpu_buffer_rsrc_t rxyz = __builtin_amdgcn_make_buffer_rsrc(
        const_cast<float*>(p.xyz), 0, p.nscenes * 3 * p.N * 4, 0x00020000);
    const __amdgpu_buffer_rsrc_t rfeat = __builtin_amdgcn_make_buffer_rsrc(
        const_cast<float*>(p.feat), 0, p.nscenes * p.N * p.Cf * 4, 0x00020000);
    constexpr uint32_t OOB = 0x80000000u;
    int jr[NRB], jg[RPT];
#pragma unroll
    for (int rb = 0; rb < NRB; ++rb)
      jr[rb] = __builtin_amdgcn_raw_buffer_load_b32(ridx, (wr * WROWS + rb * 32 + li) * 4, 0, 0);
#pragma unroll
    for (int s = 0; s < RPT; ++s) jg[s] = __builtin_amdgcn_raw_buffer_load_b32(ridx, ((t >> 3) + RS * s) * 4, 0, 0);
    {
      int bw, mw;
      gather_row_bm(p.M, p.K, p0, __builtin_amdgcn_readfirstlane(wr * WROWS), bw, mw);
      bw = __builtin_amdgcn_readfirstlane(bw);
      mw = __builtin_amdgcn_readfirstlane(mw);
      const bool okw = p0 + wr * WROWS < p.P;
      float cx = 0.f, cy = 0.f, cz = 0.f;
      if (okw) {
        const float* c = p.ctr + (size_t)bw * 3 * p.M + mw;
        cx = c[0];
        cy = c[p.M];
        cz = c[2 * p.M];
      }
      const uint32_t xb = okw ? (uint32_t)(bw * 3 * p.N) * 4u : OOB;
#pragma unroll
      for (int rb = 0; rb < NRB; ++rb) {
        const uint32_t vo = xb + (uint32_t)jr[rb] * 4u;
        const float x = __builtin_bit_cast(float, __builtin_amdgcn_raw_buffer_load_b32(rxyz, vo, 0, 0));
        const float y = __builtin_bit_cast(float, __builtin_amdgcn_raw_buffer_load_b32(rxyz, vo + (uint32_t)p.N * 4u, 0, 0));
        const float z = __builtin_bit_cast(float, __builtin_amdgcn_raw_buffer_load_b32(rxyz, vo + (uint32_t)p.N * 8u, 0, 0));
        rv0[rb] = make_float4(__fsub_rn(x, cx), __fsub_rn(y, cy), __fsub_rn(z, cz), 0.f);
      }
    }
    uint32_t rowoff[RPT];
#pragma unroll
    for (int s = 0; s < RPT; ++s) {
      const int c64 = (RS * s) / 64 * 64;
      int bc, mc;
      gather_row_bm(p.M, p.K, p0, c64, bc, mc);
      bc = __builtin_amdgcn_readfirstlane(bc);
      rowoff[s] = p0 + c64 < p.P ? (uint32_t)((bc * p.N + jg[s]) * p.Cf + (t & 7) * 4) * 4u : OOB;
    }
    if (p.Cin >= K) {
#pragma unroll
      for (int kt = 0; kt < NKT0; ++kt)
#pragma unroll
        for (int s = 0; s < RPT; ++s)
          fa[kt][s] = __builtin_bit_cast(float4, __builtin_amdgcn_raw_buffer_load_b128(rfeat, rowoff[s] + kt * 128, 0, 0));
    } else {
#pragma unroll
      for (int kt = 0; kt < NKT0; ++kt)
#pragma unroll
        for (int s = 0; s < RPT; ++s)
          fa[kt][s] = __builtin_bit_cast(float4, __builtin_amdgcn_raw_buffer_load_b128(
                                                     rfeat, kt * 32 + (t & 7) * 4 < p.Cin ? rowoff[s] + kt * 128 : OOB, 0, 0));
    }
    const int ch = wc * 64 + lane;
    if (ch < p.Cin) wv0 = p.mlp1[ch];
  } else if constexpr (MFMA0) {
    const int rows_left = p.P - p0;
    const __amdgpu_buffer_rsrc_t rrel = __builtin_amdgcn_make_buffer_rsrc(
        const_cast<float4*>(p.rel4 + p0), 0, (rows_left < BM ? rows_left : BM) * 16, 0x00020000);
#pragma unroll
    for (int rb = 0; rb < NRB; ++rb)
      rv0[rb] = __builtin_bit_cast(float4, __builtin_amdgcn_raw_buffer_load_b128(
                                               rrel, (wr * WROWS + rb * 32 + li) * 16, 0, 0));
    const int ch = wc * 64 + lane;
    if (ch < p.Cin) wv0 = p.mlp1[ch];
  } else {
    ld.init(p, p0, g, t);
  }
  S4G_STAMP(1);
  float amax = PL == 2 ? p.a_amax_floor : 1.f;
  if (PL == 2 && p.a_amax) {
    float m = __uint_as_float(wave_max_u32(__float_as_uint(am_v1)));
    for (int sc = am_s0 + 1; sc <= am_s1; ++sc) m = fmaxf(m, amax_slots(p.a_amax + (size_t)sc * 64, lane));
    amax = ADD_BOUNDS ? amax + m : fmaxf(amax, m);
  }
  if (PL == 2 && p.a_amax2) {
    float m = __uint_as_float(wave_max_u32(__float_as_uint(am_v2)));
    for (int sc = am_s0 + 1; sc <= am_s1; ++sc) m = fmaxf(m, amax_slots(p.a_amax2 + (size_t)sc * 64, lane));
    amax = ADD_BOUNDS ? amax + m : fmaxf(amax, m);
  }
  uint32_t ex = __float_as_uint(amax) >> 23;
  ex = ex < 15u ? 15u : (ex > 240u ? 240u : ex);
  ex = __builtin_amdgcn_readfirstlane(ex);
  const float sa = PL == 2 ? __uint_as_float((268u - ex) << 23) : 1.f;
  const float inv_sa = PL == 2 ? __uint_as_float((ex - 14u) << 23) : 1.f;
  auto load_panel = [&](int kc, auto depth_tag) {
    constexpr int DEPTH = decltype(depth_tag)::value;
    const int chunk = t & 7, srow = t >> 3;
    constexpr int NKT = K / 32;
#pragma unroll
    for (int kt0 = 0; kt0 < NKT; kt0 += DEPTH) {
      float4 ra[DEPTH][RPT];
#pragma unroll
      for (int kt = 0; kt < DEPTH; ++kt)
#pragma unroll
        for (int s = 0; s < RPT; ++s) ra[kt][s] = ld.load(p, s, kc * K + (kt0 + kt) * 32 + chunk * 4, t);
#pragma unroll
      for (int kt = 0; kt < DEPTH; ++kt)
#pragma unroll
        for (int s = 0; s < RPT; ++s) {
          uint16_t* dst = Ah + (srow + RS * s) * astr + (kt0 + kt) * 32 + chunk * 4;
          if constexpr (PL == 2) {
            uint2 h, l;
            split2_h<false>(ra[kt][s], sa, h, l);
            *reinterpret_cast<uint2*>(dst) = h;
            *reinterpret_cast<uint2*>(dst + aplane) = l;
          } else {
            *reinterpret_cast<uint2*>(dst) = make_uint2(cvt_pk_bf16(ra[kt][s].x, ra[kt][s].y),
                                                        cvt_pk_bf16(ra[kt][s].z, ra[kt][s].w));
          }
        }
      if (DEPTH < NKT) __builtin_amdgcn_sched_barrier(0);
    }
  };
  const uint16_t* a_lane = Ah + (wr * WROWS + li) * astr + 8 * lh;
  float* epi_s = scr + wave * 128;
  f32x16 acc[2][NRB];
  if constexpr (MFMA0 || ADD0) {
    float m = 0.f;
#pragma unroll
    for (int rb = 0; rb < NRB; ++rb)
      m = fmaxf(m, fmaxf(fmaxf(fabsf(rv0[rb].x), fabsf(rv0[rb].y)), fabsf(rv0[rb].z)));
    uint32_t ea = wave_max_u32(__float_as_uint(m)) >> 23;
    ea = ea < 90u ? 90u : (ea > 240u ? 240u : ea);
    ea = __builtin_amdgcn_readfirstlane(ea);
    const float s_a = __uint_as_float((268u - ea) << 23), inv_a = __uint_as_float((ea - 14u) << 23);
    const float one = __uint_as_float((ea + 1u) << 23), inv_one = __uint_as_float((253u - ea) << 23);
    const float bq = wv0.w * inv_one;
    const float mw = fmaxf(fmaxf(fabsf(wv0.x), fabsf(wv0.y)), fmaxf(fabsf(wv0.z), fabsf(bq)));
    uint32_t ew = __float_as_uint(mw) >> 23;
    ew = ew < 15u ? 15u : (ew > 240u ? 240u : ew);
    const float s_w = __uint_as_float((268u - ew) << 23);
    epi_s[lane] = __uint_as_float((ew - 14u) << 23) * inv_a * (ADD0 ? 1.f : sa);
    uint32_t wh01, wl01, wh23, wl23;
    split_quad_h(wv0.x, wv0.y, wv0.z, bq, s_w, wh01, wl01, wh23, wl23);
    uint4 af0[NRB][2], bf0[2][2];
#pragma unroll
    for (int cb = 0; cb < 2; ++cb) {
      bf0[cb][0] = make_uint4(lh == cb ? wh01 : 0u, lh == cb ? wh23 : 0u, 0u, 0u);
      bf0[cb][1] = make_uint4(lh == cb ? wl01 : 0u, lh == cb ? wl23 : 0u, 0u, 0u);
    }
#pragma unroll
    for (int rb = 0; rb < NRB; ++rb) {
      const float one_r = p0 + wr * WROWS + rb * 32 + li < p.P ? one : 0.f;
      uint32_t h01, l01, h23, l23;
      split_quad_h(rv0[rb].x, rv0[rb].y, rv0[rb].z, one_r, s_a, h01, l01, h23, l23);
      af0[rb][0] = make_uint4(h01, h23, 0u, 0u);
      af0[rb][1] = make_uint4(l01, l23, 0u, 0u);
    }
    f32x16 z16;
#pragma unroll
    for (int r = 0; r < 16; ++r) z16[r] = 0.f;
#pragma unroll
    for (int rb = 0; rb < NRB; ++rb)
      asm volatile("s_nop 7" : "+v"(af0[rb][0].x), "+v"(af0[rb][0].y), "+v"(af0[rb][1].x), "+v"(af0[rb][1].y));
    __builtin_amdgcn_sched_barrier(0);
#pragma unroll
    for (int cb = 0; cb < 2; ++cb)
#pragma unroll
      for (int rb = 0; rb < NRB; ++rb) {
        acc[cb][rb] = chain_mfma<PL>(bf0[cb][1], af0[rb][0], z16);
        acc[cb][rb] = chain_mfma<PL>(bf0[cb][0], af0[rb][1], acc[cb][rb]);
        acc[cb][rb] = chain_mfma<PL>(bf0[cb][0], af0[rb][0], acc[cb][rb]);
      }
    if constexpr (ADD0) {
      float* Fs = smemf;
#pragma unroll
      for (int kt = 0; kt < NKT0; ++kt)
#pragma unroll
        for (int s = 0; s < RPT; ++s)
          *reinterpret_cast<float4*>(Fs + ((t >> 3) + RS * s) * fstr + kt * 32 + (t & 7) * 4) = fa[kt][s];
      __syncthreads();
#pragma unroll
      for (int nb = 0; nb < 2; ++nb)
#pragma unroll
        for (int j = 0; j < 4; ++j) {
          const float4 f4 = *reinterpret_cast<const float4*>(epi_s + nb * 32 + 8 * j + 4 * lh);
#pragma unroll
          for (int pb = 0; pb < NRB; ++pb) {
            const float4 fv = *reinterpret_cast<const float4*>(Fs + (wr * WROWS + pb * 32 + li) * fstr + wc * 64 + nb * 32 +
                                                               8 * j + 4 * lh);
            acc[nb][pb][4 * j] = __fmaf_rn(acc[nb][pb][4 * j], f4.x, fv.x);
            acc[nb][pb][4 * j + 1] = __fmaf_rn(acc[nb][pb][4 * j + 1], f4.y, fv.y);
            acc[nb][pb][4 * j + 2] = __fmaf_rn(acc[nb][pb][4 * j + 2], f4.z, fv.z);
            acc[nb][pb][4 * j + 3] = __fmaf_rn(acc[nb][pb][4 * j + 3], f4.w, fv.w);
          }
        }
      __syncthreads();
#pragma unroll
      for (int nb = 0; nb < 2; ++nb)
#pragma unroll
        for (int j = 0; j < 4; ++j)
#pragma unroll
          for (int pb = 0; pb < NRB; ++pb) {
            uint16_t* dst = Ah + (wr * WROWS + pb * 32 + li) * astr + wc * 64 + nb * 32 + 8 * j + 4 * lh;
            uint2 h, l;
            split_quad_h(fmaxf(acc[nb][pb][4 * j], 0.f), fmaxf(acc[nb][pb][4 * j + 1], 0.f),
                         fmaxf(acc[nb][pb][4 * j + 2], 0.f), fmaxf(acc[nb][pb][4 * j + 3], 0.f), sa, h.x, l.x, h.y, l.y);
            *reinterpret_cast<uint2*>(dst) = h;
            *reinterpret_cast<uint2*>(dst + aplane) = l;
          }
    } else {
#pragma unroll
      for (int nb = 0; nb < 2; ++nb)
#pragma unroll
        for (int j = 0; j < 4; ++j) {
          const float4 f4 = *reinterpret_cast<const float4*>(epi_s + nb * 32 + 8 * j + 4 * lh);
#pragma unroll
          for (int pb = 0; pb < NRB; ++pb) {
            uint16_t* dst = Ah + (wr * WROWS + pb * 32 + li) * astr + wc * 64 + nb * 32 + 8 * j + 4 * lh;
            uint2 h, l;
            split_quad_h2(fmaxf(acc[nb][pb][4 * j], 0.f), fmaxf(acc[nb][pb][4 * j + 1], 0.f),
                          fmaxf(acc[nb][pb][4 * j + 2], 0.f), fmaxf(acc[nb][pb][4 * j + 3], 0.f), f4.x, f4.y, f4.z, f4.w,
                          h.x, l.x, h.y, l.y);
            *reinterpret_cast<uint2*>(dst) = h;
            *reinterpret_cast<uint2*>(dst + aplane) = l;
          }
        }
    }
  } else {
    if (!(S4G_CHAIN_ABLATE & 16)) load_panel(0, std::integral_constant<int, (K / 32) / (NRB / 2)>{});
  }
  S4G_STAMP(2);
  __syncthreads();
  S4G_STAMP(3);

  auto zero_acc = [&]() {
#pragma unroll
    for (int i = 0; i < 2; ++i)
#pragma unroll
      for (int j = 0; j < NRB; ++j)
#pragma unroll
        for (int r = 0; r < 16; ++r) acc[i][j][r] = 0.f;
  };
  uint4 afn[NRB][PL];
  auto prime_a = [&]() {
#pragma unroll
    for (int rb = 0; rb < NRB; ++rb)
#pragma unroll
      for (int pl = 0; pl < PL; ++pl)
        afn[rb][pl] = *reinterpret_cast<const uint4*>(a_lane + pl * aplane + rb * 32 * astr);
  };

#define S4G_F2_STRIP(SWAPPED, ZFIRST, wcur, cbs_cur, wnext, cbs_next)                                                     \
  _Pragma("unroll") for (int ks = 0; ks < KS; ++ks) {                                                  \
    const int d = ks % GF_RING;                                                                        \
    const int ksn = ks + 1 == KS ? 0 : ks + 1;                                                         \
    uint4 af[NRB][PL], bf[2][PL];                                                                      \
    _Pragma("unroll") for (int rb = 0; rb < NRB; ++rb) _Pragma("unroll") for (int pl = 0; pl < PL; ++pl) { \
      af[rb][pl] = afn[rb][pl];                                                                        \
      if (!(S4G_CHAIN_ABLATE & 2))                                                                     \
        afn[rb][pl] = *reinterpret_cast<const uint4*>(a_lane + pl * aplane + rb * 32 * astr + ksn * 16); \
    }                                                                                                  \
    _Pragma("unroll") for (int cb = 0; cb < 2; ++cb) _Pragma("unroll") for (int pl = 0; pl < PL; ++pl)  \
      bf[cb][pl] = ring[d][cb][pl];                                                                    \
    {                                                                                                  \
      const int kr = ks + GF_RING;                                                                     \
      const WRef src = kr < KS ? (wcur) : (wnext);                                                     \
      const size_t cbs = kr < KS ? (cbs_cur) : (cbs_next);                                             \
      const int kk = kr < KS ? kr : kr - KS;                                                           \
      _Pragma("unroll") for (int cb = 0; cb < 2; ++cb) _Pragma("unroll") for (int pl = 0; pl < PL; ++pl) \
        if (!(S4G_CHAIN_ABLATE & 1))                                                                   \
          ring[d][cb][pl] = wref_load(src, wf_lane + pl * 1024, (uint32_t)(cb * cbs + (size_t)kk * PL * 1024)); \
    }                                                                                                  \
    if constexpr (PL == 2) {                                                                           \
      S4G_F2_TERM(SWAPPED, 0, 1, (ZFIRST) && ks == 0)                                                  \
      S4G_F2_TERM(SWAPPED, 1, 0, false)                                                                \
      S4G_F2_TERM(SWAPPED, 0, 0, false)                                                                \
    } else {                                                                                           \
      S4G_F2_TERM(SWAPPED, 0, 0, (ZFIRST) && ks == 0)                                                  \
    }                                                                                                  \
    _Pragma("unroll") for (int q = 0; q < 2 * PL; ++q) {                                               \
      __builtin_amdgcn_sched_group_barrier(0x008, 1, 0);                                               \
      __builtin_amdgcn_sched_group_barrier(0x100, 1, 0);                                               \
      __builtin_amdgcn_sched_group_barrier(0x008, 1, 0);                                               \
      __builtin_amdgcn_sched_group_barrier(0x020, 1, 0);                                               \
    }                                                                                                  \
    if constexpr (PL == 2) __builtin_amdgcn_sched_group_barrier(0x008, 4, 0);                          \
    if constexpr (PL == 1 && NRB == 4) {             \
      _Pragma("unroll") for (int q = 0; q < 2; ++q) {                                                  \
        __builtin_amdgcn_sched_group_barrier(0x100, 1, 0);                                             \
        __builtin_amdgcn_sched_group_barrier(0x008, 2, 0);                                             \
      }                                                                                                \
    }                                                                                                  \
    __builtin_amdgcn_sched_barrier(0);                                                                 \
  }
#define S4G_F2_TERM(SWAPPED, PA, PB, Z)                                                                \
  _Pragma("unroll") for (int cb = 0; cb < 2; ++cb) _Pragma("unroll") for (int rb = 0; rb < NRB; ++rb)  \
    if constexpr (SWAPPED)                                                                             \
      acc[cb][rb] = chain_mfma<PL>(bf[cb][PB], af[rb][PA], (Z) ? zero16 : acc[cb][rb]);                \
    else                                                                                               \
      acc[cb][rb] = chain_mfma<PL>(af[rb][PA], bf[cb][PB], (Z) ? zero16 : acc[cb][rb]);
  f32x16 zero16;
#pragma unroll
  for (int r = 0; r < 16; ++r) zero16[r] = 0.f;

  WRef wcur = w1;
  const float* __restrict__ scp = PL == 2 ? p.w_inv_scale + (size_t)g * p.b_gstride : nullptr;
  const float* __restrict__ bp = p.bias + (size_t)g * p.b_gstride;
  int relu_ph = p.relu;
  float inv_in = inv_sa, inv_sh = 1.f;
  const int npanel = tri ? 2 : 1;
  for (int ph = 0; ph < npanel; ++ph) {
  const WRef wnxt = ph + 1 < npanel ? wmid : (active0 ? w2 : wcur);
  prime_a();
  {
    const int n = wc * 64 + lane;
    epi_s[lane] = PL == 2 ? inv_in * scp[n] : 1.f;
    epi_s[64 + lane] = bp[n];
  }
  if (KC > 1 && ph == 0) {
    zero_acc();
    for (int kc = 0; kc < kchunks; ++kc) {
      if (kc > 0) {
        __syncthreads();
        load_panel(kc, std::integral_constant<int, 2>{});
        __syncthreads();
        prime_a();
      }
      const WRef wc1 = w1 + (size_t)kc * cb_stride;
      const bool lastc = kc + 1 == kchunks;
      const WRef wn1 = lastc ? wnxt : wc1 + cb_stride;
      const size_t cbsn = lastc ? cb_stride : cbs1;
      S4G_F2_STRIP(true, false, wc1, cbs1, wn1, cbsn)
    }
  } else {
    S4G_F2_STRIP(true, true, wcur, cb_stride, wnxt, cb_stride)
  }
  S4G_STAMP(4 + 4 * ph);
  if (S4G_CHAIN_ABLATE & 4) {
    chain_keep_alive(acc[0][0]); chain_keep_alive(acc[0][1]); chain_keep_alive(acc[1][0]); chain_keep_alive(acc[1][1]);
    __syncthreads();
    __syncthreads();
  } else {
  float tmax = 0.f;
  const float relu_lo = relu_ph ? 0.f : -__builtin_inff();
#pragma unroll
  for (int nb = 0; nb < 2; ++nb)
#pragma unroll
    for (int j = 0; j < 4; ++j) {
      const float4 sc4 = *reinterpret_cast<const float4*>(epi_s + nb * 32 + 8 * j + 4 * lh);
      const float4 b4 = *reinterpret_cast<const float4*>(epi_s + 64 + nb * 32 + 8 * j + 4 * lh);
      const float scv[4] = {sc4.x, sc4.y, sc4.z, sc4.w};
      const float bv[4] = {b4.x, b4.y, b4.z, b4.w};
#pragma unroll
      for (int pb = 0; pb < NRB; ++pb) {
        const f32x2 x01 = pk_fma(f32x2{acc[nb][pb][4 * j], acc[nb][pb][4 * j + 1]}, f32x2{scv[0], scv[1]}, f32x2{bv[0], bv[1]});
        const f32x2 x23 = pk_fma(f32x2{acc[nb][pb][4 * j + 2], acc[nb][pb][4 * j + 3]}, f32x2{scv[2], scv[3]}, f32x2{bv[2], bv[3]});
        const float x[4] = {fmaxf(x01.x, relu_lo), fmaxf(x01.y, relu_lo), fmaxf(x23.x, relu_lo), fmaxf(x23.y, relu_lo)};
#pragma unroll
        for (int e = 0; e < 4; ++e) acc[nb][pb][4 * j + e] = x[e];
        if constexpr (PL == 2) {
          tmax = fmaxf(fmaxf(tmax, fabsf(x[0])), fabsf(x[1]));
          tmax = fmaxf(fmaxf(tmax, fabsf(x[2])), fabsf(x[3]));
        }
      }
    }
  if constexpr (LOADER == LOAD_PLAIN && EPI2 == EPI_STORE) {
    if (!p.Wfrag2) {
      const bool second = p.split_n > 0 && g * p.c_gcol >= p.split_n;
      float* __restrict__ obase = second ? p.out2 - p.split_n : p.out + p.c_coff;
      const int old = second ? p.ldc2 : p.ldc;
      uint32_t* __restrict__ oamax = second ? p.out_amax2 : p.out_amax;
#pragma unroll
      for (int nb = 0; nb < 2; ++nb)
#pragma unroll
        for (int j = 0; j < 4; ++j) {
          const int nn = wc * 64 + nb * 32 + 8 * j + 4 * lh;
#pragma unroll
          for (int pb = 0; pb < NRB; ++pb) {
            const int row = p0 + wr * WROWS + pb * 32 + li;
            if (row < p.P)
              *reinterpret_cast<float4*>(obase + (size_t)row * old + g * p.c_gcol + nn) =
                  make_float4(acc[nb][pb][4 * j], acc[nb][pb][4 * j + 1], acc[nb][pb][4 * j + 2], acc[nb][pb][4 * j + 3]);
          }
        }
      if (PL == 2 && oamax) {
        const uint32_t wm = wave_max_u32(__float_as_uint(tmax));
        if (lane == 0) amax_publish(oamax, wm, (tile * 4 + wave) * 5 + g, p0, p_hi, p.rps);
      }
      return;
    }
  }
  float sh = 1.f;
  if constexpr (PL == 2) {
    const uint32_t wm = wave_max_u32(__float_as_uint(tmax));
    if (lane == 0) scr[NW * 128 + wave] = __uint_as_float(wm);
  }
  S4G_STAMP(5 + 4 * ph);
  __syncthreads();
  S4G_STAMP(6 + 4 * ph);
  if constexpr (PL == 2) {
    float hmax = scr[NW * 128];
#pragma unroll
    for (int w = 1; w < NW; ++w) hmax = fmaxf(hmax, scr[NW * 128 + w]);
    uint32_t exh = __float_as_uint(hmax) >> 23;
    exh = exh < 15u ? 15u : (exh > 240u ? 240u : exh);
    exh = __builtin_amdgcn_readfirstlane(exh);
    sh = __uint_as_float((268u - exh) << 23);
    inv_sh = __uint_as_float((exh - 14u) << 23);
  }
#pragma unroll
  for (int nb = 0; nb < 2; ++nb)
#pragma unroll
    for (int j = 0; j < 4; ++j)
#pragma unroll
      for (int pb = 0; pb < NRB; ++pb) {
        uint16_t* dst = Ah + (wr * WROWS + pb * 32 + li) * astr + wc * 64 + nb * 32 + 8 * j + 4 * lh;
        if constexpr (PL == 2) {
          const float4 v = make_float4(acc[nb][pb][4 * j], acc[nb][pb][4 * j + 1], acc[nb][pb][4 * j + 2],
                                       acc[nb][pb][4 * j + 3]);
          uint2 h, l;
          split2_h<false>(v, sh, h, l);
          *reinterpret_cast<uint2*>(dst) = h;
          *reinterpret_cast<uint2*>(dst + aplane) = l;
        } else {
          *reinterpret_cast<uint2*>(dst) = make_uint2(cvt_pk_bf16(acc[nb][pb][4 * j], acc[nb][pb][4 * j + 1]),
                                                      cvt_pk_bf16(acc[nb][pb][4 * j + 2], acc[nb][pb][4 * j + 3]));
        }
      }
  S4G_STAMP(7 + 4 * ph);
  __syncthreads();
  }
  inv_in = inv_sh;
  wcur = wmid;
  scp = PL == 2 ? p.w_inv_scale2 + (size_t)g * p.Cout2 : nullptr;
  bp = p.bias2 + (size_t)g * p.Cout2;
  relu_ph = p.relu2;
  }

  GemmParams q = p;
  q.Cout = CoutF;
  q.relu = tri ? p.relu3 : p.relu2;
  prime_a();
  WRef wstrip = w2;
  const float* __restrict__ bg2 = bgF;
  int sidv[NRB / 2][8] = {};
  if constexpr (SEGMAX) {
    if (seg_scene) {
#pragma unroll
      for (int c = 0; c < NRB / 2; ++c) {
        const int4* sp = reinterpret_cast<const int4*>(p.seg4 + ((p0 + wr * WROWS + c * 64 + lh * 32) >> 2));
        const int4 s0 = sp[0], s1 = sp[1];
        sidv[c][0] = s0.x; sidv[c][1] = s0.y; sidv[c][2] = s0.z; sidv[c][3] = s0.w;
        sidv[c][4] = s1.x; sidv[c][5] = s1.y; sidv[c][6] = s1.z; sidv[c][7] = s1.w;
      }
    }
  }
  for (int strip = 0; strip < nstrip2; ++strip, wstrip = wstrip + strip_stride) {
    if ((strip * CW + wc_u) * 64 >= CoutF) break;
    const int n = (strip * CW + wc) * 64 + lane;
    const float e_sc = PL == 2 ? inv_sh * scF[n] : 1.f;
    const float e_bias = bg2[n];
    const WRef wnext = ((strip + 1) * CW + wc_u) * 64 < CoutF ? wstrip + strip_stride : wstrip;
    S4G_STAMP(12 + 2 * (strip & 1));
    S4G_F2_STRIP(EPI2 == EPI_STORE, true, wstrip, cb_stride, wnext, cb_stride)
    S4G_STAMP(13 + 2 * (strip & 1));
    if (S4G_CHAIN_ABLATE & 8) {
      chain_keep_alive(acc[0][0]); chain_keep_alive(acc[0][1]); chain_keep_alive(acc[1][0]); chain_keep_alive(acc[1][1]);
      continue;
    }
    const int n0 = (strip * CW + wc) * 64;
    float omax = 0.f;
    if constexpr (EPI2 == EPI_STORE) {
      epi_s[lane] = e_sc;
      epi_s[64 + lane] = e_bias;
#pragma unroll
      for (int nb = 0; nb < 2; ++nb)
#pragma unroll
        for (int j = 0; j < 4; ++j) {
          const int nn = n0 + nb * 32 + 8 * j + 4 * lh;
          const float4 sc4 = *reinterpret_cast<const float4*>(epi_s + nb * 32 + 8 * j + 4 * lh);
          const float4 b4 = *reinterpret_cast<const float4*>(epi_s + 64 + nb * 32 + 8 * j + 4 * lh);
          const float scv[4] = {sc4.x, sc4.y, sc4.z, sc4.w};
          const float bv[4] = {b4.x, b4.y, b4.z, b4.w};
#pragma unroll
          for (int pb = 0; pb < NRB; ++pb) {
            float v[4];
#pragma unroll
            for (int e = 0; e < 4; ++e) {
              float x = __fmaf_rn(acc[nb][pb][4 * j + e], scv[e], bv[e]);
              if (q.relu) x = fmaxf(x, 0.f);
              v[e] = x;
              omax = fmaxf(omax, fabsf(x));
            }
            const int row = p0 + wr * WROWS + pb * 32 + li;
            if (row < p.P)
              *reinterpret_cast<float4*>(p.out + (size_t)row * p.ldc + p.c_coff + g * p.c_gcol + nn) =
                  make_float4(v[0], v[1], v[2], v[3]);
          }
        }
      if (p.out_amax) {
        const uint32_t wm = wave_max_u32(__float_as_uint(omax));
        if (lane == 0) amax_publish(p.out_amax, wm, tile * 4 + wave + strip, p0, p_hi, p.rps);
      }
    } else if (SEGMAX && seg_scene) {
      uint32_t* __restrict__ outu = reinterpret_cast<uint32_t*>(p.out);
#pragma unroll
      for (int cb = 0; cb < 2; ++cb) {
        const float sc = __shfl(e_sc, cb * 32 + li);
        const float bias = __shfl(e_bias, cb * 32 + li);
        const int nn = n0 + cb * 32 + li;
#pragma unroll
        for (int c = 0; c < NRB / 2; ++c) {
        float v[8];
#pragma unroll
        for (int qd = 0; qd < 4; ++qd) {
          const float o0 = fmaxf(fmaxf(acc[cb][2 * c][4 * qd], acc[cb][2 * c][4 * qd + 1]),
                                 fmaxf(acc[cb][2 * c][4 * qd + 2], acc[cb][2 * c][4 * qd + 3]));
          const float o1 = fmaxf(fmaxf(acc[cb][2 * c + 1][4 * qd], acc[cb][2 * c + 1][4 * qd + 1]),
                                 fmaxf(acc[cb][2 * c + 1][4 * qd + 2], acc[cb][2 * c + 1][4 * qd + 3]));
          const auto r = __builtin_amdgcn_permlane32_swap(__float_as_uint(o0), __float_as_uint(o1), false, false);
          v[2 * qd] = __uint_as_float(r[0]);
          v[2 * qd + 1] = __uint_as_float(r[1]);
        }
        auto emit = [&](int seg, float m) {
// ... 11 lines not shown
          m = chg ? v[i] : fmaxf(m, v[i]);
          cur = sidv[c][i];
        }
        emit(cur, m);
        }
      }
      if (PL == 2 && p.out_amax) {
        const uint32_t wm = wave_max_u32(__float_as_uint(omax));
        if (lane == 0) amax_publish(p.out_amax, wm, tile * 4 + wave + strip, p0, p_hi, p.rps);
      }
    } else if (q.relu && p.K == 64) {
#pragma unroll
      for (int cb = 0; cb < 2; ++cb) {
        const float sc = __shfl(e_sc, cb * 32 + li);
        const float bias = __shfl(e_bias, cb * 32 + li);
        const int nn = n0 + cb * 32 + li;
#pragma unroll
        for (int c = 0; c < NRB / 2; ++c) {
          float m = acc[cb][2 * c][0];
#pragma unroll
          for (int rb = 2 * c; rb < 2 * c + 2; ++rb)
#pragma unroll
            for (int r = 0; r < 16; ++r) m = fmaxf(m, acc[cb][rb][r]);
          m = fmaxf(m, __shfl_xor(m, 32));
          const float v = fmaxf(m * sc + bias, 0.f);
          omax = fmaxf(omax, v);
          const int row0 = p0 + wr * WROWS + c * 64;
          if (nn < CoutF && lh == 0 && row0 < p.P) p.out[(size_t)(row0 >> 6) * p.ldc + p.c_coff + nn] = v;
        }
      }
      if (PL == 2 && p.out_amax) {
        const uint32_t wm = wave_max_u32(__float_as_uint(omax));
        if (lane == 0) amax_publish(p.out_amax, wm, tile * 4 + wave + strip, p0, p_hi, p.rps);
      }
    } else if constexpr (NRB == 2) {
      f32x16 acct[2][2];
#pragma unroll
      for (int cb = 0; cb < 2; ++cb) {
        const float sc = __shfl(e_sc, cb * 32 + li);
        const float bias = __shfl(e_bias, cb * 32 + li);
        float mx = -__builtin_inff(), mn = __builtin_inff();
#pragma unroll
        for (int rb = 0; rb < 2; ++rb)
#pragma unroll
          for (int r = 0; r < 16; ++r) {
            const float v = acc[cb][rb][r] * sc;
            acct[rb][cb][r] = v;
            mx = fmaxf(mx, v);
            mn = fminf(mn, v);
          }
        const float hi = mx + bias, lo = mn + bias;
        omax = fmaxf(omax, q.relu ? hi : fmaxf(fabsf(hi), fabsf(lo)));
      }
      if (p.out_amax) {
        const uint32_t wm = wave_max_u32(__float_as_uint(fmaxf(omax, 0.f)));
        if (lane == 0) amax_publish(p.out_amax, wm, tile * 4 + wave + strip, p0, p_hi, p.rps);
      }
      gemm_epilogue<EPI_MAX, 2>(q, acct, bg2, g, p0, n0, wave, wr, 0, li, lh, smemf);
    }
  }
  S4G_STAMP(11);
#undef S4G_F2_STRIP
#undef S4G_F2_TERM
}

template <int LOADER, int EPI2, int RW, int KC, int PL>
static int launch_mlp_chain(const GemmParams& p, int groups, hipStream_t st) {
  constexpr int CW = RW == 8 ? 8 : 4 / RW, RWN = RW == 8 ? 1 : RW;
  constexpr int NRB = PL == 1 ? S4G_CHAIN_BF16_NRB : 2;
  constexpr int BM = 32 * NRB * RWN, K = 64 * CW, NW = RWN * CW;
  constexpr size_t lds = sizeof(uint16_t) * PL * BM * (size_t)(K + 8) + sizeof(float) * (NW * 128 + 16);
  static_assert(lds <= (RW == 8 ? 160 : 80) * 1024, "two workgroups per CU (one for the 8-wave form)");
  static LdsAttrCache lds_cache;
  if (int rc = allow_dynamic_lds(reinterpret_cast<const void*>(&mlp_chain_kernel<LOADER, EPI2, RW, KC, PL>), lds, lds_cache)) return rc;
  const dim3 grid((unsigned)((p.P + BM - 1) / BM), (unsigned)groups);
  hipLaunchKernelGGL((mlp_chain_kernel<LOADER, EPI2, RW, KC, PL>), grid, dim3(64 * NW), lds, st, p);
  S4G_LAUNCH_CHECK();
  return S4G_OK;
}

template <int LOADER, int EPI, int PL = 2>
static int launch_gemm_f16x2(const GemmParams& p, int groups, hipStream_t st) {
  constexpr int force = 0;
  const int64_t wide_wgs = (int64_t)((p.P + GM_BM - 1) / GM_BM) * ((p.Cout + 255) / 256) * groups;
  const bool wide = force ? force == 4
                          : p.Cout > 256 && wide_wgs >= 512 &&
                                (LOADER == LOAD_PLAIN || LOADER == LOAD_GATHER_MLP1 || LOADER == LOAD_GATHER_ADD);
  if (wide) return launch_gemm_f16x2_cfg<LOADER, EPI, 4, PL>(p, groups, st);
  return launch_gemm_f16x2_cfg<LOADER, EPI, 2, PL>(p, groups, st);
}

template <int LOADER, int EPI, int NS, int WAVES>
static int launch_gemm_bf16x3_cfg(const GemmParams& p, int groups, hipStream_t st) {
  constexpr int BK = 32 * NS;
  size_t lds = sizeof(float) * GM_BM * (BK + 4) + sizeof(uint16_t) * 3 * GM_BN * (BK + 8);
  const size_t epi = sizeof(float) * 4 * 32 * 68;
  if (lds < epi) lds = epi;
  static LdsAttrCache lds_cache;
  if (int rc = allow_dynamic_lds(reinterpret_cast<const void*>(&mlp_gemm_bf16x3_kernel<LOADER, EPI, NS, WAVES>), lds, lds_cache)) return rc;
  const dim3 grid((unsigned)(p.mtiles * p.ntiles), (unsigned)groups);
  hipLaunchKernelGGL((mlp_gemm_bf16x3_kernel<LOADER, EPI, NS, WAVES>), grid, dim3(64 * WAVES), lds,
                     st, p);
  S4G_LAUNCH_CHECK();
  return S4G_OK;
}

template <int LOADER, int EPI>
static int launch_gemm_bf16x3(const GemmParams& p, int groups, hipStream_t st) {
  return launch_gemm_bf16x3_cfg<LOADER, EPI, 1, 4>(p, groups, st);
}

template <int LOADER, int EPI>
static int launch_gemm(const GemmParams& p, int groups, hipStream_t st) {
  const size_t lds = sizeof(float) * 2 * (GM_BM + GM_BN) * GM_LDS;
  static LdsAttrCache lds_cache;
  if (int rc = allow_dynamic_lds(reinterpret_cast<const void*>(&mlp_gemm_kernel<LOADER, EPI>), lds, lds_cache)) return rc;
  const dim3 grid((unsigned)(p.mtiles * p.ntiles), (unsigned)groups);
  hipLaunchKernelGGL((mlp_gemm_kernel<LOADER, EPI>), grid, dim3(GM_THREADS), lds, st, p);
  S4G_LAUNCH_CHECK();
  return S4G_OK;
}

}

#define S4G_FUSED2_LIST(X)                                                                       \
  X(LOAD_GATHER_MLP1, EPI_MAX, 2, 1)                                                             \
  X(LOAD_GATHER_MLP1, EPI_MAX, 1, 1)                                                             \
  X(LOAD_GATHER_ADD, EPI_MAX, 2, 1)                                                              \
  X(LOAD_GATHER_ADD, EPI_MAX, 1, 1)                                                              \
  X(LOAD_GATHER_ADD, EPI_MAX, 8, 1)       \
  X(LOAD_PLAIN, EPI_MAX, 2, 1)                                                                   \
  X(LOAD_PLAIN, EPI_MAX, 1, 1)                                                                   \
  X(LOAD_PLAIN, EPI_MAX, 8, 1)                                                                   \
  X(LOAD_PLAIN, EPI_STORE, 2, 1)                                                                 \
  X(LOAD_PLAIN, EPI_STORE, 1, 1)                                                                 \
  X(LOAD_PLAIN, EPI_STORE, 1, 2)            \
  X(LOAD_PLAIN, EPI_STORE, 1, 4)         \
  X(LOAD_PLAIN, EPI_STORE, 8, 1)                                                                 \
  X(LOAD_INTERP_ADD, EPI_STORE, 2, 1)                                                            \
  X(LOAD_INTERP_ADD, EPI_STORE, 1, 1)                                                            \
  X(LOAD_INTERP_ADD, EPI_STORE, 8, 1)

#ifdef S4G_CHAIN_STAMPS
extern "C" int s4g_debug_chain_stamps(unsigned long long* host_out_512x16) {
  return (int)hipMemcpyFromSymbol(host_out_512x16, HIP_SYMBOL(s4g::g_chain_stamps), sizeof(unsigned long long) * 512 * 16);
}
#endif

extern "C" int s4g_gemm_chain_supported(int loader, int epilogue, int C, int Kpad16) {
  using namespace s4g;
  const int r = C == 128 ? 2 : (C == 256 ? 1 : (C == 512 ? 8 : 0));
  if (r == 0 || Kpad16 <= 0 || Kpad16 % C) return 0;
  const int kc = Kpad16 / C;
#define S4G_FUSED2_Q(L, E, R, KCH) \
  if (loader == L && epilogue == (int)E && r == R && kc == KCH) return 1;
  S4G_FUSED2_LIST(S4G_FUSED2_Q)
#undef S4G_FUSED2_Q
  return 0;
}

extern "C" int s4g_mlp_gemm_f32(const s4g_gemm_desc_t* d, s4g_stream_t stream) {
  using namespace s4g;
  if (!d || d->P < 0 || d->Cout <= 0 || d->groups <= 0 || !d->bias) return S4G_EINVAL;
  const bool split = d->precision == S4G_GEMM_BF16X3 || d->precision == S4G_GEMM_BF16;
  const bool h2 = d->precision == S4G_GEMM_F16X2;
  if (h2) {
    if (!d->W_f16x2 || !d->w_inv_scale || d->Kpad16 <= 0 || (d->Kpad16 & 15) ||
        !(d->a_amax_floor >= 0.f) || (!d->a_amax && !d->a_amax2 && !(d->a_amax_floor > 0.f)))
      return S4G_EINVAL;
  } else if (split) {
    if (!d->W_bf16x3 || d->Kpad16 <= 0 || (d->Kpad16 & 15)) return S4G_EINVAL;
  } else if (d->precision == S4G_GEMM_FP32) {
    if (!d->W || d->Kpad <= 0 || (d->Kpad & 7)) return S4G_EINVAL;
  } else {
    return S4G_EINVAL;
  }
  if (d->P == 0) return S4G_OK;
  GemmParams p;
  p.P = d->P; p.Cin = d->Cin; p.Kpad = d->Kpad; p.Cout = d->Cout; p.relu = d->relu;
  p.W = d->W; p.bias = d->bias;
  p.A = d->A; p.lda = d->lda; p.a_coff = d->a_coff; p.a_gcol = d->a_gcol; p.aL = d->a_L;
  p.gidx = d->gidx; p.feat = d->feat; p.xyz = d->xyz; p.ctr = d->ctr;
  p.Cf = d->Cf; p.N = d->N; p.M = d->M; p.K = d->K;
  p.nscenes = d->M > 0 && d->K > 0 ? (int)((d->P + (int64_t)d->M * d->K - 1) / ((int64_t)d->M * d->K)) : 0;
  p.mlp1 = (const float4*)d->mlp1_w;
  p.rel4 = (const float4*)d->rel_xyz4;
  p.seg4 = d->seg4;
  p.seg_rows = d->seg_rows;
  p.out2 = d->out2;
  p.ldc2 = d->ldc2;
  p.split_n = d->out2 ? d->split_n : 0;
  p.out_amax2 = (uint32_t*)d->out_amax2;
  p.nidx = d->nidx; p.nw = d->nw; p.sparse = d->sparse; p.dense = d->dense;
  p.C2 = d->C2; p.C1 = d->C1; p.N2 = d->N2; p.N1 = d->N1;
  p.out = d->out; p.ldc = d->ldc; p.c_coff = d->c_coff; p.c_gcol = d->c_gcol;
  p.w_gstride = d->w_gstride; p.b_gstride = d->b_gstride;
  for (int i = 0; i < 4; ++i) p.cf_ptr[i] = d->cf_ptr[i];
  for (int i = 0; i < 5; ++i) p.cf_start[i] = d->cf_start[i];
  p.cf_sigmoid_from = d->cf_sigmoid_from; p.cf_N = d->cf_N;
  p.W3 = (const uint16_t*)d->W_bf16x3;
  p.Kpad16 = d->Kpad16;
  p.bf16_single = d->precision == S4G_GEMM_BF16 ? 1 : 0;
  p.w3_plane = (size_t)d->groups * (size_t)d->Cout * (size_t)d->Kpad16;
  p.Wh2 = (const uint16_t*)d->W_f16x2;
  p.w_inv_scale = d->w_inv_scale;
  p.a_amax = d->a_amax; p.a_amax2 = d->a_amax2; p.a_amax_floor = d->a_amax_floor;
  p.out_amax = (uint32_t*)d->out_amax;
  p.rps = d->rows_per_scene > 0 ? d->rows_per_scene : 0;
  p.Wfrag = (const uint16_t*)d->W_f16x2_frag;
  p.lbias = d->loader_bias;
  p.Wfrag2 = (const uint16_t*)d->W2_f16x2_frag;
  p.w_inv_scale2 = d->w2_inv_scale;
  p.bias2 = d->bias2;
  p.Cout2 = d->Cout2;
  p.relu2 = d->relu2;
  p.Wfrag3 = (const uint16_t*)d->W3_f16x2_frag;
  p.w_inv_scale3 = d->w3_inv_scale;
  p.bias3 = d->bias3;
  p.Cout3 = d->Cout3;
  p.relu3 = d->relu3;
  p.mtiles = (d->P + GM_BM - 1) / GM_BM;
  p.ntiles = (d->Cout + GM_BN - 1) / GM_BN;
  hipStream_t st = (hipStream_t)stream;

  if (d->loader == S4G_GEMM_LOAD_PLAIN) {
    if (!d->A || (d->lda & 3) || (d->a_coff & 3) || (d->a_gcol & 3) || (d->Cin & 3)) return S4G_EINVAL;
  } else if (d->loader == S4G_GEMM_LOAD_GATHER) {
    if (!d->gidx || !d->xyz || !d->ctr || (d->Cf & 3) || (d->Cf > 0 && !d->feat) ||
        d->K <= 0 || d->M <= 0 || d->N <= 0 || d->groups != 1)
      return S4G_EINVAL;
  } else if (d->loader == S4G_GEMM_LOAD_GATHER_MLP1) {
    if ((!d->rel_xyz4 && (!d->gidx || !d->xyz || !d->ctr)) || ((uintptr_t)d->rel_xyz4 & 15) ||
        !d->mlp1_w || (d->Cin & 3) || d->K <= 0 || d->M <= 0 || d->N <= 0 || d->groups != 1 ||
        ((uintptr_t)d->mlp1_w & 15))
      return S4G_EINVAL;
    if ((d->seg4 != nullptr) != (d->seg_rows != nullptr)) return S4G_EINVAL;
    if (d->seg4 && (!d->rel_xyz4 || !d->W2_f16x2_frag || d->epilogue != S4G_GEMM_EPI_MAX || d->K != 64 ||
                    d->rows_per_scene <= 0 || (d->rows_per_scene & 255) || !d->relu2 || d->W3_f16x2_frag))
      return S4G_EINVAL;
  } else if (d->loader == S4G_GEMM_LOAD_GATHER_ADD) {
    if (!d->gidx || !d->xyz || !d->ctr || !d->mlp1_w || !d->feat || (d->Cin & 3) || d->Cf != d->Cin ||
        d->K <= 0 || d->M <= 0 || d->N <= 0 || d->groups != 1 || ((uintptr_t)d->mlp1_w & 15) ||
        ((uintptr_t)d->feat & 15))
      return S4G_EINVAL;
  } else if (d->loader == S4G_GEMM_LOAD_INTERP_ADD) {
    if (!d->nidx || !d->nw || !d->sparse || !d->loader_bias || (d->Cin & 3) || d->C2 != d->Cin ||
        d->N1 <= 0 || d->N2 <= 0 || d->groups != 1 ||
        (((uintptr_t)d->sparse | (uintptr_t)d->dense | (uintptr_t)d->loader_bias) & 15))
      return S4G_EINVAL;
  } else if (d->loader == S4G_GEMM_LOAD_INTERP) {
    if (!d->nidx || !d->nw || !d->sparse || (d->C2 & 3) || (d->C1 & 3) ||
        (d->C1 > 0 && !d->dense) || d->N1 <= 0 || d->N2 <= 0 || d->groups != 1)
      return S4G_EINVAL;
  } else if (d->loader == S4G_GEMM_LOAD_CHANNEL_FIRST) {
    if (!d->A || d->Cin < 1 || d->a_L <= 0 || d->P % d->a_L || d->groups != 1 ||
        d->Cin > (h2 ? d->Kpad16 : d->Kpad))
      return S4G_EINVAL;
  } else {
    return S4G_EINVAL;
  }
  if (d->loader != S4G_GEMM_LOAD_GATHER_MLP1 && (d->seg4 || d->seg_rows)) return S4G_EINVAL;
  if (d->out2) {
    const bool bf1_ = d->precision == S4G_GEMM_BF16;
    if (!(h2 || bf1_) || d->loader != S4G_GEMM_LOAD_PLAIN || d->epilogue != S4G_GEMM_EPI_STORE || d->W2_f16x2_frag ||
        d->groups != 1 || d->split_n <= 0 || (d->split_n & 255) || d->split_n >= d->Cout || (d->Cout & 255) ||
        (d->ldc2 & 3) || ((uintptr_t)d->out2 & 15) || d->c_coff != 0 || (d->ldc & 3) || ((uintptr_t)d->out & 15))
      return S4G_EINVAL;
  }
  if (d->epilogue == S4G_GEMM_EPI_MAX) {
    if (!(d->K == 16 || d->K == 32 || d->K == 64) || d->groups != 1 || !d->out) return S4G_EINVAL;
  } else if (d->epilogue == S4G_GEMM_EPI_STORE) {
    if (!d->out) return S4G_EINVAL;
  } else if (d->epilogue == S4G_GEMM_EPI_CHANNEL_FIRST) {
    if (d->cf_N <= 0 || d->groups != 1) return S4G_EINVAL;
  } else if (d->epilogue == S4G_GEMM_EPI_MAX_CHANNEL_FIRST) {
    if (d->relu != 1 || d->K < 1 || d->M < 1 || d->P % ((int64_t)d->M * d->K) || d->groups != 1 || !d->out ||
        d->W2_f16x2_frag || d->out2)
      return S4G_EINVAL;
  } else {
    return S4G_EINVAL;
  }

  if (d->W2_f16x2_frag) {
    const bool c128 = d->Cout == 128 && d->Kpad16 == 128,
               c256 = d->Cout == 256 && (d->Kpad16 == 256 || d->Kpad16 == 512 || d->Kpad16 == 1024),
               c512 = d->Cout == 512 && d->Kpad16 == 512;
    const bool store = d->epilogue == S4G_GEMM_EPI_STORE;
    const bool bf1 = d->precision == S4G_GEMM_BF16;
    if ((!h2 && !bf1) || (!store && (d->epilogue != S4G_GEMM_EPI_MAX || d->K != 64 || (d->P & 63))) ||
        (!c128 && !c256 && !c512) || d->Cout2 <= 0 || (d->Cout2 & 63) || (!store && d->groups != 1) || !d->W_f16x2_frag ||
        (d->W3_f16x2_frag && (d->Cout2 != d->Cout || d->Cout3 <= 0 || (d->Cout3 & 63) ||
                              (h2 && !d->w3_inv_scale) || !d->bias3)) ||
        (h2 && !d->w2_inv_scale) || !d->bias2 ||
        (store && (((d->ldc | d->c_coff | d->c_gcol) & 3) || ((uintptr_t)d->out & 15))))
      return S4G_EINVAL;
    if (bf1 && !store && !(d->W3_f16x2_frag ? d->relu3 : d->relu2)) return S4G_EUNSUPPORTED;
    if (h2 && d->loader == S4G_GEMM_LOAD_GATHER_MLP1 && d->rel_xyz4 && d->epilogue == S4G_GEMM_EPI_MAX &&
        d->Kpad16 == d->Cout && d->Cin <= d->Cout && (c128 || c256)) {
      const char* m0 = s4g::knob("S4G_MLP1_MFMA");
      if (!(m0 && m0[0] == '0'))
        return c128 ? launch_mlp_chain<LOAD_REL_MLP1, EPI_MAX, 2, 1, 2>(p, d->groups, st)
                    : launch_mlp_chain<LOAD_REL_MLP1, EPI_MAX, 1, 1, 2>(p, d->groups, st);
    }
    if (h2 && d->loader == S4G_GEMM_LOAD_GATHER_ADD && d->epilogue == S4G_GEMM_EPI_MAX && d->Kpad16 == d->Cout &&
        (int64_t)p.nscenes * d->N * d->Cf * 4 < (1ll << 31) && (int64_t)p.nscenes * d->N * 12 < (1ll << 31))
      return c128   ? launch_mlp_chain<LOAD_ADD_MFMA0, EPI_MAX, 2, 1, 2>(p, d->groups, st)
             : c256 ? launch_mlp_chain<LOAD_ADD_MFMA0, EPI_MAX, 1, 1, 2>(p, d->groups, st)
                    : launch_mlp_chain<LOAD_ADD_MFMA0, EPI_MAX, 8, 1, 2>(p, d->groups, st);
#define S4G_FUSED2_CASE(L, E, R, KCH)                                                        \
  if (d->loader == L && (int)d->epilogue == (int)E && (c128 ? 2 : (c256 ? 1 : 8)) == R &&     \
      d->Kpad16 / d->Cout == KCH)                                                             \
    return bf1 ? launch_mlp_chain<L, E, R, KCH, 1>(p, d->groups, st)                 \
               : launch_mlp_chain<L, E, R, KCH, 2>(p, d->groups, st);
    S4G_FUSED2_LIST(S4G_FUSED2_CASE)
#undef S4G_FUSED2_CASE
    return S4G_EUNSUPPORTED;
  }
  {
    const char* sc_env = s4g::knob("S4G_GEMM_SINGLE_CHAIN");
    const bool single_chain = !(sc_env && sc_env[0] == '0');
    const bool bf1 = d->precision == S4G_GEMM_BF16;
    const int kc = d->Kpad16 / 256;
    if (single_chain && (h2 || bf1) && d->loader == S4G_GEMM_LOAD_PLAIN && d->epilogue == S4G_GEMM_EPI_STORE &&
        d->W_f16x2_frag && d->groups == 1 && d->Cout % 256 == 0 && d->Kpad16 % 256 == 0 &&
        (kc == 1 || kc == 2 || kc == 4) && ((d->ldc | d->c_coff) & 3) == 0 && ((uintptr_t)d->out & 15) == 0 &&
        (d->Cout >= 1024 || d->Kpad16 >= 1024 || (sc_env && sc_env[0] == '1'))) {
      GemmParams q = p;
      q.Cout = 256;
      q.a_gcol = 0;
      q.c_gcol = 256;
      q.b_gstride = 256;
      const int strips = d->Cout / 256;
#define S4G_SINGLE_CASE(KCH)                                                                     \
  if (kc == KCH)                                                                                 \
    return bf1 ? launch_mlp_chain<LOAD_PLAIN, EPI_STORE, 1, KCH, 1>(q, strips, st)               \
               : launch_mlp_chain<LOAD_PLAIN, EPI_STORE, 1, KCH, 2>(q, strips, st);
      S4G_SINGLE_CASE(1)
      S4G_SINGLE_CASE(2)
      S4G_SINGLE_CASE(4)
#undef S4G_SINGLE_CASE
    }
  }
  constexpr bool bf16_tiled = true;
#define S4G_GEMM_CASE(L, E)                                            \
  if (d->loader == L && d->epilogue == E)                              \
    return h2 ? launch_gemm_f16x2<L, E>(p, d->groups, st)              \
           : (p.bf16_single && bf16_tiled) ? launch_gemm_f16x2<L, E, 1>(p, d->groups, st) \
           : split ? launch_gemm_bf16x3<L, E>(p, d->groups, st)        \
                   : launch_gemm<L, E>(p, d->groups, st);
  S4G_GEMM_CASE(LOAD_PLAIN, EPI_STORE)
  S4G_GEMM_CASE(LOAD_PLAIN, EPI_MAX)
  S4G_GEMM_CASE(LOAD_PLAIN, EPI_CHANNEL_FIRST)
  S4G_GEMM_CASE(LOAD_GATHER, EPI_STORE)
  S4G_GEMM_CASE(LOAD_GATHER, EPI_MAX)
  S4G_GEMM_CASE(LOAD_INTERP, EPI_STORE)
  S4G_GEMM_CASE(LOAD_GATHER_MLP1, EPI_STORE)
  S4G_GEMM_CASE(LOAD_GATHER_MLP1, EPI_MAX)
  S4G_GEMM_CASE(LOAD_GATHER_ADD, EPI_STORE)
  S4G_GEMM_CASE(LOAD_GATHER_ADD, EPI_MAX)
  S4G_GEMM_CASE(LOAD_INTERP_ADD, EPI_STORE)
#undef S4G_GEMM_CASE
#define S4G_GEMM_CASE_CF(L, E)                                                           \
  if (d->loader == L && d->epilogue == E)                                                \
    return h2 ? launch_gemm_f16x2<L, E>(p, d->groups, st)                                \
              : d->precision == S4G_GEMM_FP32 ? launch_gemm<L, E>(p, d->groups, st) : S4G_EUNSUPPORTED;
  S4G_GEMM_CASE_CF(LOAD_CHANNEL_FIRST, EPI_STORE)
  S4G_GEMM_CASE_CF(LOAD_CHANNEL_FIRST, EPI_CHANNEL_FIRST)
  S4G_GEMM_CASE_CF(LOAD_CHANNEL_FIRST, EPI_MAX_CF)
  S4G_GEMM_CASE_CF(LOAD_PLAIN, EPI_MAX_CF)
#undef S4G_GEMM_CASE_CF
  return S4G_EUNSUPPORTED;
}

__global__ __launch_bounds__(256) void amax_per_scene_kernel(const float* __restrict__ x, int64_t n,
                                                             uint32_t* __restrict__ slots) {
  const int b = blockIdx.y;
  const float* xs = x + (size_t)b * n;
  float m = 0.f;
  for (int64_t i = (int64_t)blockIdx.x * 256 + threadIdx.x; i < n; i += (int64_t)gridDim.x * 256)
    m = fmaxf(m, fabsf(xs[i]));
  const uint32_t wm = s4g::wave_max_u32(__float_as_uint(m));
  if ((threadIdx.x & 63) == 0) atomicMax(slots + (size_t)b * 64 + ((blockIdx.x * 4 + (threadIdx.x >> 6)) & 63), wm);
}

extern "C" int s4g_amax_per_scene_f32(const float* x, int64_t B, int64_t n_per_scene, float* out_slots,
                                      s4g_stream_t stream) {
  if (B < 0 || n_per_scene < 0 || B > 65535 || ((!x || !out_slots) && B * n_per_scene > 0)) return S4G_EINVAL;
  if (B == 0 || n_per_scene == 0) return S4G_OK;
  const int64_t want = (n_per_scene + 256 * 16 - 1) / (256 * 16);
  const unsigned wgs = (unsigned)(want < 64 ? want : 64);
  hipLaunchKernelGGL(amax_per_scene_kernel, dim3(wgs, (unsigned)B), dim3(256), 0, (hipStream_t)stream, x, n_per_scene,
                     reinterpret_cast<uint32_t*>(out_slots));
  S4G_LAUNCH_CHECK();
  return S4G_OK;
}
```

s4g_release_amd/csrc/s4g_common.h:

```cpp
#pragma once
#include <hip/hip_runtime.h>
#include <stdint.h>

#include "../../include/s4g_ops.h"

#define S4G_WAVE 64

#define S4G_LAUNCH_CHECK()                        \
  do {                                            \
    hipError_t e_ = hipGetLastError();            \
    if (e_ != hipSuccess) return (int)e_;         \
  } while (0)

#include <atomic>
#include <cstdlib>
#include <cstring>

namespace s4g {
inline bool test_knobs_enabled() {
  const char* m = getenv("S4G_TEST_KNOBS");
  return m && m[0] == '1' && m[1] == 0;
}
inline const char* knob(const char* name) { return test_knobs_enabled() ? getenv(name) : nullptr; }
}

namespace s4g {

struct LdsAttrCache {
  std::atomic<int> bytes[64];
};
inline int allow_dynamic_lds(const void* func, size_t lds_bytes, LdsAttrCache& cache) {
  int dev = 0;
  hipError_t e = hipGetDevice(&dev);
  if (e != hipSuccess) return (int)e;
  const bool slot = dev >= 0 && dev < 64;
  if (slot && cache.bytes[dev].load(std::memory_order_relaxed) >= (int)lds_bytes) return 0;
  e = hipFuncSetAttribute(func, hipFuncAttributeMaxDynamicSharedMemorySize, (int)lds_bytes);
  if (e != hipSuccess) return (int)e;
  if (slot) cache.bytes[dev].store((int)lds_bytes, std::memory_order_relaxed);
  return 0;
}

template <bool FMAD>
__device__ __forceinline__ float dist2(float x1, float y1, float z1, float x2,
                                       float y2, float z2) {
  const float dx = __fsub_rn(x2, x1);
  const float dy = __fsub_rn(y2, y1);
  const float dz = __fsub_rn(z2, z1);
  if constexpr (FMAD) {
    float t = __fmul_rn(dx, dx);
    t = __fmaf_rn(dy, dy, t);
    t = __fmaf_rn(dz, dz, t);
    return t;
  } else {
    return __fadd_rn(__fadd_rn(__fmul_rn(dx, dx), __fmul_rn(dy, dy)),
                     __fmul_rn(dz, dz));
  }
}

template <int CTRL>
__device__ __forceinline__ uint32_t dpp_u32(uint32_t v) {
  return (uint32_t)__builtin_amdgcn_update_dpp(0, (int)v, CTRL, 0xF, 0xF, true);
}

__device__ __forceinline__ uint32_t row16_max_u32(uint32_t v) {
  v = max(v, dpp_u32<0xB1>(v));
  v = max(v, dpp_u32<0x4E>(v));
  v = max(v, dpp_u32<0x141>(v));
  v = max(v, dpp_u32<0x140>(v));
  return v;
}
__device__ __forceinline__ uint32_t row16_min_u32(uint32_t v) {
  v = min(v, dpp_u32<0xB1>(v));
  v = min(v, dpp_u32<0x4E>(v));
  v = min(v, dpp_u32<0x141>(v));
  v = min(v, dpp_u32<0x140>(v));
  return v;
}

__device__ __forceinline__ uint32_t wave_max_u32(uint32_t v) {
  v = row16_max_u32(v);
  const uint32_t a = __builtin_amdgcn_readlane(v, 0);
  const uint32_t b = __builtin_amdgcn_readlane(v, 16);
  const uint32_t c = __builtin_amdgcn_readlane(v, 32);
  const uint32_t d = __builtin_amdgcn_readlane(v, 48);
  return max(max(a, b), max(c, d));
}
__device__ __forceinline__ uint32_t wave_min_u32(uint32_t v) {
  v = row16_min_u32(v);
  const uint32_t a = __builtin_amdgcn_readlane(v, 0);
  const uint32_t b = __builtin_amdgcn_readlane(v, 16);
  const uint32_t c = __builtin_amdgcn_readlane(v, 32);
  const uint32_t d = __builtin_amdgcn_readlane(v, 48);
  return min(min(a, b), min(c, d));
}

__device__ __forceinline__ uint32_t wave_inclusive_scan_u32(uint32_t v) {
#define S4G_DPP0(CTRL, RM) \
  (uint32_t)__builtin_amdgcn_update_dpp(0, (int)v, CTRL, RM, 0xF, true)
  v += S4G_DPP0(0x111, 0xF);
  v += S4G_DPP0(0x112, 0xF);
  v += S4G_DPP0(0x114, 0xF);
  v += S4G_DPP0(0x118, 0xF);
  v += S4G_DPP0(0x142, 0xA);
  v += S4G_DPP0(0x143, 0xC);
#undef S4G_DPP0
  return v;
}

__device__ __forceinline__ int lane_id() {
  return (int)__builtin_amdgcn_mbcnt_hi(~0u, __builtin_amdgcn_mbcnt_lo(~0u, 0));
}

__device__ __forceinline__ int mask_rank(uint64_t mask) {
  return (int)__builtin_amdgcn_mbcnt_hi(
      (uint32_t)(mask >> 32), __builtin_amdgcn_mbcnt_lo((uint32_t)mask, 0));
}

__device__ __forceinline__ bool finite(float v) { return fabsf(v) <= 3.402823466e38f; }
__device__ __forceinline__ bool finite(double v) { return fabs(v) <= 1.7976931348623157e308; }

}
```

s4g_release_amd/fused.py:

```python
import ctypes
import os

import torch

from . import _cabi
from . import functions as _F

_i32 = ctypes.c_int32
_fp = ctypes.c_void_p
GemmDesc = _cabi.GemmDesc
HeadsDesc = _cabi.HeadsDesc

LOAD_PLAIN, LOAD_GATHER, LOAD_INTERP, LOAD_GATHER_MLP1, LOAD_GATHER_ADD, LOAD_INTERP_ADD = 0, 1, 2, 3, 4, 5
EPI_STORE, EPI_MAX, EPI_CF = 0, 1, 2

NETWORK_KINDS = {(9, 4): "PN2_CLS", (6, 3): "PN2"}
HEADS_CLS = ("score", "frame_R", "frame_t", "movable_logits")
HEADS_CONTACT = ("scene_score_logits", "frame_R", "frame_t", "movable_logits")
CONTACT_RAW_CHANNELS = (3, 6, 3, 5)
CONTACT_OUT_CHANNELS = (3, 9, 3, 5)


def fold_conv_bn(block):
    w = block.conv.weight.detach().double().flatten(1)
    if block.bn is None:
        b = block.conv.bias.detach().double() if block.conv.bias is not None else \
            torch.zeros(w.shape[0], dtype=torch.float64, device=w.device)
        return w.float(), b.float()
    bn = block.bn
    scale = bn.weight.detach().double() / torch.sqrt(bn.running_var.detach().double() + bn.eps)
    wf = w * scale[:, None]
    bf = bn.bias.detach().double() - bn.running_mean.detach().double() * scale
    if block.conv.bias is not None:
        bf = bf + block.conv.bias.detach().double() * scale
    return wf.float(), bf.float()


def _pad_k(w, mult=8):
    cout, k = w.shape
    kpad = (k + mult - 1) // mult * mult
    if kpad == k:
        return w.contiguous()
    out = w.new_zeros((cout, kpad))
    out[:, :k] = w
    return out


def split_bf16x3(w):
    w1 = w.to(torch.bfloat16)
    r1 = w - w1.float()
    w2 = r1.to(torch.bfloat16)
    r2 = r1 - w2.float()
    w3 = r2.to(torch.bfloat16)
    return torch.stack([w1, w2, w3], dim=0).contiguous()


def split_f16x2(w):
    amax = w.abs().amax(dim=-1)
    _, ex = torch.frexp(amax)
    ex = torch.where(amax > 0, ex, torch.zeros_like(ex)).clamp(-100, 100)
    one = torch.ones_like(amax)
    s = torch.ldexp(one, 15 - ex)
    ws = w * s[..., None]
    w1 = ws.to(torch.float16)
    w2 = (ws - w1.float()).to(torch.float16)
    return torch.stack([w1, w2], dim=0).contiguous(), torch.ldexp(one, ex - 15).contiguous()


def fragment_order(planes):
    if planes.dim() == 3:
        planes = planes.unsqueeze(1)
    npl, G, cout, k16 = planes.shape
    x = planes.reshape(npl, G, cout // 32, 32, k16 // 16, 2, 8)
    return x.permute(1, 2, 4, 0, 5, 3, 6).contiguous()


class _Layer:

    def __init__(self, W, bias, cin, groups=1):
        self.W = W.contiguous()
        self.bias = bias.contiguous()
        self.groups = groups
        self.cout = self.W.shape[-2]
        self.kpad = self.W.shape[-1]
        self.cin = cin
        self.kpad16 = (self.kpad + 15) // 16 * 16
        w16 = self.W.new_zeros(self.W.shape[:-1] + (self.kpad16,))
        w16[..., :self.kpad] = self.W
        self.W3 = split_bf16x3(w16)
        self.Wh2, self.w_inv_scale = split_f16x2(w16)
        self.Wfrag = fragment_order(self.Wh2) if self.cout % 32 == 0 else None
        self.Wfrag_bf16 = fragment_order(self.W3[:1])[:, :, :, 0].contiguous() if self.cout % 32 == 0 else None


_STREAM_POOL = {}


def _stream_pool(dev, n_geo, n_dense):
    key = (str(dev), int(n_geo), int(n_dense))
    pool = _STREAM_POOL.get(key)
    if pool is None:
        pool = _STREAM_POOL[key] = ([torch.cuda.Stream(device=dev, priority=-1) for _ in range(n_geo)],
                                    [torch.cuda.Stream(device=dev) for _ in range(n_dense)])
    return pool


class FusedPointNet2:

    def __init__(self, net, precision=None, fold_only=False, check_finite=False):
        self.check_finite = bool(check_finite)
        if precision is None:
            precision = os.environ.get("S4G_GEMM_MODE", "f16x2")
        if precision not in ("f16x2", "bf16x3", "fp32", "bf16"):
            raise ValueError("precision must be 'f16x2', 'bf16x3', 'fp32' or 'bf16'")
        self.precision = precision
        self.dense_streams = max(1, int(os.environ.get("S4G_DENSE_STREAMS", "1")))
        self.fuse2 = _cabi.knob("S4G_GEMM_FUSE2", "1") != "0"
        self.fp_linear_first = _cabi.knob("S4G_FP_LINEAR_FIRST", "1") != "0"
        self.geo_streams = max(1, int(os.environ.get("S4G_GEO_STREAMS", "2")))
        self.rel_xyz = _cabi.knob("S4G_REL_XYZ", "1") != "0"
        self.sa_unique = _cabi.knob("S4G_SA_UNIQUE", "1") != "0"
        self.heads_pre = _cabi.knob("S4G_HEADS_PRE", "1") != "0"
        self.merge_shared = _cabi.knob("S4G_MERGE_SHARED", "1") != "0"
        self.fp_chain_next = _cabi.knob("S4G_FP_CHAIN_NEXT", "1") != "0"
        self.fps_prefix = _cabi.knob("S4G_FPS_PREFIX", "1") != "0"
        self.packed_out = _cabi.knob("S4G_PACKED_OUT", "1") != "0"
        p = next(net.parameters())
        self.fold_only = bool(fold_only)
        if not p.is_cuda and not fold_only:
            raise RuntimeError("FusedPointNet2 needs the model on a HIP device (no CPU fallback)")
        if net.training:
            raise RuntimeError("FusedPointNet2 is inference-only: call net.eval() first")
        self.dev = p.device
        if not fold_only:
            _cabi.lib()
        self.sa = []
        for sa in net.sa_modules:
            if sa.sampler is None or sa.grouper is None:
                raise NotImplementedError("fast path covers sampled + grouped SA modules only")
            if sa.grouper.num_neighbours not in (16, 32, 64):
                raise NotImplementedError("fast path needs num_neighbours in {16, 32, 64}")
            layers = []
            mlp1 = None
            for li, blk in enumerate(sa.mlp):
                w, b = fold_conv_bn(blk)
                if li == 0 and sa.in_channels == 0 and len(sa.mlp) > 1 and w.shape[0] % 4 == 0:
                    mlp1 = torch.cat([w[:, :3], b[:, None]], dim=1).contiguous()
                if li == 0:
                    w = torch.cat([w[:, 3:], w[:, :3]], dim=1)
                    cin = w.shape[1]
                else:
                    cin = w.shape[1]
                layers.append(_Layer(_pad_k(w), b, cin))
            radius = float(sa.grouper.radius)
            pre = None
            if (sa.in_channels > 0 and sa.in_channels % 4 == 0 and len(sa.mlp) > 1 and
                    layers[0].cout % 4 == 0 and _cabi.knob("S4G_SA_LINEAR_FIRST", "1") != "0"):
                w0 = layers[0].W[:, :layers[0].cin]
                cf = sa.in_channels
                la = _Layer(_pad_k(w0[:, :cf].contiguous()), torch.zeros_like(layers[0].bias), cf)
                w1 = torch.cat([w0[:, cf:cf + 3], layers[0].bias[:, None]], dim=1).contiguous()
                bound = float((w1[:, :3].abs().sum(dim=1) * radius + w1[:, 3].abs()).max())
                pre = dict(la=la, w1=w1, bound=bound)
            mlp1_bound = 0.0 if mlp1 is None else float(
                (mlp1[:, :3].abs().sum(dim=1) * radius + mlp1[:, 3].abs()).max())
            self.sa.append(dict(M=sa.num_centroids, radius=radius,
# ... 118 lines not shown
        if c2 <= 0 or la.cin != c1 or la.cout % 256 or l0.cout % 256 or l0.cout > 1024 or len(fp["layers"]) < 2:
            return None
        _, lb, _ = self._fp_split(fp, l0, c2, c1)
        m = sa.get("merged")
        if m is None or m[1] is not lb:
            w = torch.cat([la.W[:, :c1], lb.W[:, :c1]], dim=0).contiguous()
            m = sa["merged"] = (_Layer(_pad_k(w), w.new_zeros(w.shape[0]), c1), lb)
        return m

    def _heads_take_tail(self, fi, fl, pending):
        return (self.heads_fused is not None and self.heads_pre and fi == len(self.fp) - 1 and len(fl) == 3 and
                pending["C2"] == 256 and all(l.cin == 256 and l.cout == 256 and l.groups == 1 and
                                             l.Wfrag is not None for l in fl[1:]) and
                self.head_layers[0].cin == 256)

    def _gemm(self, name, layer, P, loader, epi, relu=True, layer2=None, layer3=None, name3="heads.0",
              rows_per_scene=0, relu2=True, name2=None, rows_used=None, **kw):
        d = GemmDesc()
        d.loader, d.epilogue, d.groups, d.relu = loader, epi, layer.groups, int(relu)
        d.P, d.Cin, d.Kpad, d.Cout = P, layer.cin, layer.kpad, layer.cout
        d.rows_per_scene = rows_per_scene or (P // self._batch if P % self._batch == 0 else 0)
        d.W, d.bias = layer.W.data_ptr(), layer.bias.data_ptr()
        d.w_gstride, d.b_gstride = layer.cout * layer.kpad, layer.cout
        d.precision = {"fp32": 0, "bf16x3": 1, "bf16": 2, "f16x2": 3}[self.precision]
        d.Kpad16, d.W_bf16x3 = layer.kpad16, layer.W3.data_ptr()
        d.W_f16x2, d.w_inv_scale = layer.Wh2.data_ptr(), layer.w_inv_scale.data_ptr()
        bf16 = self.precision == "bf16"
        frag = (lambda l: l.Wfrag_bf16) if bf16 else (lambda l: l.Wfrag)
        if layer.Wfrag is not None:
            d.W_f16x2_frag = frag(layer).data_ptr()
        for k, v in kw.items():
            if isinstance(v, torch.Tensor):
                v = v.data_ptr()
            if v is not None:
                setattr(d, k, v)
        flops = 2.0 * P * layer.cout * layer.cin * layer.groups
        if layer2 is not None:
            d.W2_f16x2_frag = frag(layer2).data_ptr()
            d.w2_inv_scale, d.bias2 = layer2.w_inv_scale.data_ptr(), layer2.bias.data_ptr()
            d.Cout2, d.relu2 = layer2.cout, int(relu2)
            flops += 2.0 * P * layer2.cout * layer2.cin * layer2.groups
            name = "%s+%s" % (name, name2 or name[:-1] + str(int(name[-1]) + 1))
        if layer3 is not None:
            d.W3_f16x2_frag = frag(layer3).data_ptr()
            d.w3_inv_scale, d.bias3 = layer3.w_inv_scale.data_ptr(), layer3.bias.data_ptr()
            d.Cout3, d.relu3 = layer3.cout, 1
            flops += 2.0 * P * layer3.cout * layer3.cin * layer3.groups
            name += "+" + name3
        if rows_used is not None:
            per_row = flops / P
            flops = lambda: per_row * float(rows_used.sum().item())
        with _F._timed("gemm[%s P=%d K=%d N=%dx%d]" % (name, P, layer.cin, layer.groups, layer.cout),
                       0, flops):
            rc = _cabi.lib().s4g_mlp_gemm_f32(ctypes.byref(d), _F._stream())
        _cabi.check(rc, "mlp_gemm " + name)

    def _heads(self, x, x_amax, outs, B, N0, pre=None, head_mask=0):
        d = HeadsDesc()
        bf16 = self.precision == "bf16"
        d.precision = 2 if bf16 else 3
        d.P, d.N = B * N0, N0
        d.C, d.H0, d.H1, d.H2, d.H3 = 256, 512, 256, 256, 128
        flops = 0.0
        name = "heads.0-3+logits"
        if pre is None:
            d.X, d.ldx = x.data_ptr(), x.shape[1]
        else:
            frag = (lambda l: l.Wfrag_bf16) if bf16 else (lambda l: l.Wfrag)
            for i, layer in enumerate(pre["layers"]):
                d.pre_W_frag[i] = frag(layer).data_ptr()
                d.pre_bias[i] = layer.bias.data_ptr()
                d.pre_w_inv_scale[i] = layer.w_inv_scale.data_ptr()
                flops += 2.0 * B * N0 * layer.cout * layer.cin
            d.pre_nidx, d.pre_nw = pre["nidx"].data_ptr(), pre["nw"].data_ptr()
            d.pre_sparse, d.pre_N2 = pre["sparse"].data_ptr(), pre["N2"]
            d.pre_dense = None if pre["dense"] is None else pre["dense"].data_ptr()
            d.pre_lbias = pre["loader_bias"].data_ptr()
            d.pre_a_amax2 = None if pre["a_amax2"] is None else pre["a_amax2"].data_ptr()
            x_amax = pre["a_amax"]
            name = "%s+%s" % (pre["name"], name)
        nrun = len([h for h in range(4) if (head_mask or 15) >> h & 1])
        for l, layer in enumerate(self.heads_fused):
            d.W_frag[l] = (layer.Wfrag_bf16 if bf16 else layer.Wfrag).data_ptr()
            d.bias[l] = layer.bias.data_ptr()
            d.w_inv_scale[l] = layer.w_inv_scale.data_ptr()
            if l < 4:
                flops += 2.0 * B * N0 * layer.cout * layer.cin * layer.groups * nrun / 4.0
        flops += 2.0 * B * N0 * sum(c for h, c in enumerate(self.head_channels) if (head_mask or 15) >> h & 1) * 128
        d.head_mask = head_mask
        run = [h for h in range(4) if (head_mask or 15) >> h & 1]
        for h, o in enumerate(outs):
            d.channels[h] = self.head_channels[h]
            if h not in run:
                continue
            d.out[h] = o.data_ptr()
            if o.stride(0) != self.head_channels[h] * N0:
                d.out_batch_stride = o.stride(0)
        d.sigmoid_head = 3
        d.a_amax = None if x_amax is None else x_amax.data_ptr()
        d.a_amax_floor = 0.0 if pre is None else pre["a_amax_floor"]
        d.rows_per_scene = N0
        if head_mask not in (0, 15):
            name += "[heads %s]" % "".join(str(h) for h in range(4) if head_mask >> h & 1)
        with _F._timed("gemm[%s P=%d K=256 N=%dx(512,256,256,128,c)]" % (name, B * N0, nrun), 0, flops):
            rc = _cabi.lib().s4g_heads_chain_f32(ctypes.byref(d), _F._stream())
        _cabi.check(rc, "heads_chain")

    def _fps_gather(self, xyz, M, want_dist=False, run=None):
        B, _, N = xyz.shape
        idx = torch.empty((B, M), dtype=torch.int32, device=xyz.device)
        ctr = torch.empty((B, 3, M), dtype=torch.float32, device=xyz.device)
        ws, nbytes = _F._workspace(_cabi.S4G_OP_FPS, xyz.device, B, N, M, 0)
        dist = torch.empty((B, M), dtype=torch.float32, device=xyz.device) if want_dist else None
        with _F._timed("fps[N=%d,M=%d]" % (N, M), B * (12 * N + 8 * M)):
            if dist is not None or run is not None:
                rc = _cabi.lib().s4g_fps_gather_ex_i32(xyz.data_ptr(), B, N, M, idx.data_ptr(), ctr.data_ptr(),
                                                       None if dist is None else dist.data_ptr(),
                                                       None if run is None else run.data_ptr(),
                                                       _F._ptr(ws), nbytes, _F._DIST_FLAGS, _F._stream())
                if rc == _cabi.S4G_EUNSUPPORTED and run is None:
                    dist, rc = None, 0
                    rc = _cabi.lib().s4g_fps_gather_i32(xyz.data_ptr(), B, N, M, idx.data_ptr(), ctr.data_ptr(),
                                                        _F._ptr(ws), nbytes, _F._DIST_FLAGS, _F._stream())
            else:
                rc = _cabi.lib().s4g_fps_gather_i32(xyz.data_ptr(), B, N, M, idx.data_ptr(),
                                                    ctr.data_ptr(), _F._ptr(ws), nbytes,
                                                    _F._DIST_FLAGS, _F._stream())
        _cabi.check(rc, "fps_gather")
        return (idx, ctr, dist) if want_dist else (idx, ctr)

    def _fps_prefix_check(self, ctr, dist, M2):
        B, _, M1 = ctr.shape
        run = torch.empty((B,), dtype=torch.int32, device=ctr.device)
        with _F._timed("fps_prefix_check[M1=%d,M2=%d]" % (M1, M2), B * 16 * M1):
            rc = _cabi.lib().s4g_fps_prefix_check_f32(ctr.data_ptr(), dist.data_ptr(), B, M1, M2, run.data_ptr(),
                                                      _F._DIST_FLAGS, _F._stream())
        _cabi.check(rc, "fps_prefix_check")
        return run

    def _ball_query(self, xyz, ctr, radius, K):
        B, _, N = xyz.shape
        M = ctr.shape[2]
        idx = torch.empty((B, M, K), dtype=torch.int32, device=xyz.device)
        cnt = torch.empty((B, M), dtype=torch.int32, device=xyz.device)
        ws, nbytes = _F._workspace(_cabi.S4G_OP_BALL_QUERY, xyz.device, B, N, M, K)
        with _F._timed("ball_query[N=%d,M=%d,K=%d]" % (N, M, K),
                       B * (12 * N + 12 * M + 8 * M * K + 8 * M)):
            rc = _cabi.lib().s4g_ball_query_i32(xyz.data_ptr(), ctr.data_ptr(), B, N, M, radius, K,
                                                idx.data_ptr(), cnt.data_ptr(), _F._ptr(ws), nbytes,
                                                _F._DIST_FLAGS, _F._stream())
        _cabi.check(rc, "ball_query_i32")
        return idx, cnt

    def _group_rel_xyz(self, xyz, ctr, gidx):
        B, _, N = xyz.shape
        _, M, K = gidx.shape
        rel = torch.empty((B * M * K, 4), dtype=torch.float32, device=xyz.device)
        with _F._timed("group_rel_xyz[N=%d,M=%d,K=%d]" % (N, M, K), B * M * K * (4 + 12 + 16)):
            rc = _cabi.lib().s4g_group_rel_xyz_i32(xyz.data_ptr(), ctr.data_ptr(), gidx.data_ptr(),
                                                   B, N, M, K, rel.data_ptr(), _F._stream())
        _cabi.check(rc, "group_rel_xyz_i32")
        return rel

    def _group_rel_xyz_unique(self, xyz, ctr, gidx, gcnt):
        B, _, N = xyz.shape
        _, M, K = gidx.shape
        if K % 4 or (M * K) % 256:
            return None
        dev = xyz.device
        rel = torch.empty((B * M * K, 4), dtype=torch.float32, device=dev)
        seg4 = torch.empty((B * M * K // 4,), dtype=torch.int32, device=dev)
        row_start = torch.empty((B, M), dtype=torch.int32, device=dev)
        rows = torch.empty((B,), dtype=torch.int32, device=dev)
        with _F._timed("group_rel_xyz_unique[N=%d,M=%d,K=%d]" % (N, M, K), B * M * K * (4 + 12 + 16)):
            rc = _cabi.lib().s4g_group_rel_xyz_unique_i32(xyz.data_ptr(), ctr.data_ptr(), gidx.data_ptr(),
                                                          gcnt.data_ptr(), B, N, M, K, rel.data_ptr(),
                                                          seg4.data_ptr(), row_start.data_ptr(), rows.data_ptr(),
                                                          _F._stream())
        if rc == _cabi.S4G_EUNSUPPORTED:
            return None
        _cabi.check(rc, "group_rel_xyz_unique_i32")
        return rel, seg4, rows

    def _three_nn(self, q, k, eps, cell=0.0):
        B, _, N1 = q.shape
        N2 = k.shape[2]
        idx = torch.empty((B, N1, 3), dtype=torch.int32, device=q.device)
        w = torch.empty((B, N1, 3), dtype=torch.float32, device=q.device)
        if cell != 0.0 and 2048 <= N2 <= 65536 and _cabi.knob("S4G_NN_MODE", "grid") != "scan":
            nbytes = _cabi.lib().s4g_three_nn_grid_workspace_bytes(B, N1, N2)
            ws = torch.empty(nbytes, dtype=torch.uint8, device=q.device)
            with _F._timed("three_nn[N1=%d,N2=%d]" % (N1, N2), B * (12 * N2 + 12 * N1 + 24 * N1 + 12 * N1)):
                rc = _cabi.lib().s4g_three_nn_weights_grid_i32(q.data_ptr(), k.data_ptr(), B, N1, N2,
                                                               eps, cell, idx.data_ptr(),
                                                               w.data_ptr(), ws.data_ptr(), nbytes,
                                                               _F._DIST_FLAGS, _F._stream())
            _cabi.check(rc, "three_nn_weights_grid_i32")
            return idx, w
        with _F._timed("three_nn[N1=%d,N2=%d]" % (N1, N2), B * (12 * N2 + 12 * N1 + 24 * N1 + 12 * N1)):
            rc = _cabi.lib().s4g_three_nn_weights_i32(q.data_ptr(), k.data_ptr(), B, N1, N2, eps,
                                                      idx.data_ptr(), w.data_ptr(), None, 0,
                                                      _F._DIST_FLAGS, _F._stream())
        _cabi.check(rc, "three_nn_weights_i32")
        return idx, w

    def _sa_unique_ok(self, sa):
        layers = sa["layers"]
        return (self.precision in ("f16x2", "bf16") and len(layers) == 3 and layers[-1].groups == 1 and
                self._fusable(layers[-2], layers[-1], LOAD_GATHER_MLP1, EPI_MAX))

    def _geometry(self, xyz):
        B, _, N0 = xyz.shape
        geo = dict(level_xyz=[xyz], level_n=[N0], sa=[], fp=[], sa_events=[], rel=[])
        n_cur = N0
        run = None
        for li, sa in enumerate(self.sa):
            M, K = sa["M"], sa["K"]
            if not n_cur >= M:
                raise RuntimeError("num_points is not greater than or equal to num_centroids")
            dist = None
            if li == 0 and self.fps_prefix and len(self.sa) > 1 and self.sa[1]["M"] <= M:
                idx, ctr, dist = self._fps_gather(geo["level_xyz"][-1], M, want_dist=True)
            else:
                idx, ctr = self._fps_gather(geo["level_xyz"][-1], M, run=run if li > 0 else None)
            gidx, gcnt = self._ball_query(geo["level_xyz"][-1], ctr, sa["radius"], K)
            geo["sa"].append((idx, ctr, gidx, gcnt))
            rel = None
            if sa["mlp1"] is not None and self.rel_xyz:
                if self.sa_unique and K == 64 and self._sa_unique_ok(sa):
                    rel = self._group_rel_xyz_unique(geo["level_xyz"][-1], ctr, gidx, gcnt)
                    if rel is not None:
                        rel = rel + (torch.zeros((B * M, sa["layers"][-1].cout), dtype=torch.float32,
                                                 device=xyz.device),)
                if rel is None:
                    rel = self._group_rel_xyz(geo["level_xyz"][-1], ctr, gidx)
            geo["rel"].append(rel)
            geo["sa_events"].append(torch.cuda.current_stream().record_event())
            if dist is not None and all(self.sa[l + 1]["M"] <= self.sa[l]["M"] for l in range(1, len(self.sa) - 1)):
                run = self._fps_prefix_check(ctr, dist, self.sa[1]["M"])
            geo["level_xyz"].append(ctr)
            geo["level_n"].append(M)
            n_cur = M
        sparse_xyz = geo["level_xyz"][-1]
        for fi, fp in enumerate(self.fp):
            dense_xyz = geo["level_xyz"][-2 - fi]
            geo["fp"].append(self._three_nn(dense_xyz, sparse_xyz, fp["eps"], -1.0))
            sparse_xyz = dense_xyz
        return geo

    def _dense(self, xyz, geo, topk=None):
        B, _, N0 = xyz.shape
        dev = xyz.device
        self._batch = B
        level_xyz, level_n = geo["level_xyz"], geo["level_n"]
        keep = geo.get("feats")
        n_launch = sum(len(sa["layers"]) for sa in self.sa) + \
            sum(len(fp["layers"]) for fp in self.fp) + len(self.head_layers) + 1 + len(self.sa) + 2 * len(self.fp)
        amax = torch.zeros((n_launch, B, 64), dtype=torch.float32, device=dev)
        rows = iter(amax.unbind(0))
        level_feat = [(None, None)]
        shared = {}
        feat = feat_amax = None
        cur = torch.cuda.current_stream()
        for li, sa in enumerate(self.sa):
            M, K = sa["M"], sa["K"]
            _, ctr, gidx, _ = geo["sa"][li]
            cur.wait_event(geo["sa_events"][li])
            P = B * M * K
            layers = sa["layers"]
            x = x_amax = None
            pre = sa["pre"] if self.precision in ("f16x2", "bf16") else None
            lp = len(layers) - 2
            first_loader = (LOAD_GATHER_MLP1 if (lp == 1 and sa["mlp1"] is not None) else
                            LOAD_GATHER_ADD if (lp == 1 and pre is not None) else LOAD_PLAIN)
            fuse2 = (K == 64 and len(layers) >= 3 and layers[-1].groups == 1 and
                     self._fusable(layers[-2], layers[-1], first_loader, EPI_MAX))
            if pre is not None:
                fpre = torch.empty((B * level_n[li], layers[0].cout), dtype=torch.float32, device=dev)
                fpre_amax = next(rows)
                mg = self._shared_input_layer(li, feat.shape[1])
                if mg is not None:
                    fi = len(self.sa) - 1 - li
                    y = torch.empty((B * level_n[li], mg[1].cout), dtype=torch.float32, device=dev)
                    y_amax = next(rows)
                    self._gemm("sa%d.0f|fp%d.0d" % (li, fi), mg[0], B * level_n[li], LOAD_PLAIN, EPI_STORE,
                               relu=False, out=fpre, ldc=layers[0].cout, A=feat, lda=feat.shape[1],
                               a_amax=feat_amax, out_amax=fpre_amax, out2=y, ldc2=mg[1].cout,
                               split_n=layers[0].cout, out_amax2=y_amax)
                    shared[fi] = (y, y_amax)
                else:
                    self._gemm("sa%d.0f" % li, pre["la"], B * level_n[li], LOAD_PLAIN, EPI_STORE, relu=False,
                               out=fpre, ldc=layers[0].cout, A=feat, lda=feat.shape[1], a_amax=feat_amax,
                               out_amax=fpre_amax)
            for l, layer in enumerate(layers):
                if l == 0 and (sa["mlp1"] is not None or pre is not None):
                    continue
                if fuse2 and l == len(layers) - 1:
                    continue
                last = l == len(layers) - 1 or (fuse2 and l == len(layers) - 2)
                nrow = B * M if last else P
                l2 = layers[-1] if (fuse2 and l == len(layers) - 2) else None
                cout = l2.cout if l2 is not None else layer.cout
                rel = geo["rel"][li] if (l == 1 and sa["mlp1"] is not None) else None
                uniq = isinstance(rel, tuple) and l2 is not None
                out = rel[3] if uniq else torch.empty((nrow, cout), dtype=torch.float32, device=dev)
                out_amax = next(rows)
                kw = dict(out=out, ldc=cout, K=K, out_amax=out_amax, layer2=l2)
                if l == 1 and sa["mlp1"] is not None:
                    kw.update(gidx=gidx, xyz=level_xyz[li], ctr=ctr, N=level_n[li], M=M,
                              mlp1_w=sa["mlp1"], a_amax_floor=sa["mlp1_bound"])
                    if uniq:
                        kw.update(rel_xyz4=rel[0], seg4=rel[1], seg_rows=rel[2], rows_used=rel[2])
                    elif isinstance(rel, tuple):
                        raise RuntimeError("distinct-row records without the fused chain that consumes them")
                    elif rel is not None:
                        kw.update(rel_xyz4=rel)
                    loader = LOAD_GATHER_MLP1
                elif l == 1 and pre is not None:
                    kw.update(gidx=gidx, feat=fpre, Cf=layers[0].cout, xyz=level_xyz[li], ctr=ctr,
                              N=level_n[li], M=M, mlp1_w=pre["w1"], a_amax=fpre_amax,
                              a_amax_floor=pre["bound"])
                    loader = LOAD_GATHER_ADD
                elif l == 0:
                    kw.update(gidx=gidx, feat=feat, xyz=level_xyz[li], ctr=ctr, Cf=sa["cf"],
                              N=level_n[li], M=M, a_amax=feat_amax, a_amax_floor=sa["radius"])
                    loader = LOAD_GATHER
                else:
                    kw.update(A=x, lda=x.shape[1], a_amax=x_amax)
                    loader = LOAD_PLAIN
                self._gemm("sa%d.%d" % (li, l), layer, P, loader, EPI_MAX if last else EPI_STORE,
                           **kw)
                x, x_amax = out, out_amax
            feat, feat_amax = x, x_amax
            level_feat.append((feat, feat_amax))
            if keep is not None:
                keep["sa%d" % li] = feat.view(B, M, -1)

        cur.wait_event(geo["done"])
        (sparse_feat, sparse_amax), n_sparse = level_feat[-1], level_n[-1]
        heads0_fused = False
        heads_pre = None
        carried = None
        sparse_channels = 0
        for fi, fp in enumerate(self.fp):
            (dense_feat, dense_amax), n_dense = level_feat[-2 - fi], level_n[-2 - fi]
            nidx, nw = geo["fp"][fi]
            P = B * n_dense
            x = x_amax = None
            fl = fp["layers"]
            pending = None
            nxt = self.fp[fi + 1] if fi + 1 < len(self.fp) else None
            chain_next = (self.fp_chain_next and nxt is not None and len(fl) == 2 and self.fp_linear_first and
                          self.precision in ("f16x2", "bf16") and level_feat[-3 - fi][0] is None and
                          fl[1].cin == fl[1].cout and fl[1].kpad16 == fl[1].cout and fl[1].Wfrag is not None and
                          nxt["layers"][0].cin == fl[1].cout and nxt["layers"][0].cout % 64 == 0 and
                          nxt["layers"][0].cout <= 1024 and len(nxt["layers"]) >= 2 and
                          bool(_cabi.lib().s4g_gemm_chain_supported(LOAD_INTERP_ADD, EPI_STORE, fl[1].cout,
                                                                     fl[1].kpad16)))
            fuse2 = len(fl) >= 3 and self._fusable(fl[-2], fl[-1])
            h0 = self.head_layers[0]
            fuse3 = (fuse2 and fi == len(self.fp) - 1 and self.heads_fused is None and
                     fl[-1].cout == fl[-2].cout and
                     h0.groups == 1 and h0.cin == fl[-1].cout and h0.kpad16 == fl[-1].cout and
                     h0.cout % 64 == 0 and h0.Wfrag is not None)
            for l, layer in enumerate(fl):
                if fuse2 and l == len(fl) - 1:
                    continue
                if pending is not None and self._heads_take_tail(fi, fl, pending):
                    heads_pre = dict(pending, layers=[fl[-2], fl[-1]], name="fp%d.1+fp%d.2" % (fi, fi))
                    pending = None
                    x = x_amax = None
                    break
                if pending is not None and chain_next and l == 1:
                    nl = nxt["layers"][0]
                    nsp = self._fp_split(nxt, nl, layer.cout, 0)
                    s_next = torch.empty((P, nl.cout), dtype=torch.float32, device=dev)
                    s_next_amax = next(rows)
                    self._gemm("fp%d.%d" % (fi, l), layer, P, LOAD_INTERP_ADD, EPI_STORE, out=s_next,
                               ldc=nl.cout, out_amax=s_next_amax, layer2=nsp[0], relu2=False,
                               name2="fp%d.0s" % (fi + 1), **pending)
                    carried = (s_next, s_next_amax)
                    pending = None
                    x = x_amax = None
                    sparse_channels = layer.cout
                    break
                l2 = fl[-1] if (fuse2 and l == len(fl) - 2) else None
                l3 = h0 if (fuse3 and l2 is not None) else None
                out = torch.empty((P, (l3 or l2 or layer).cout), dtype=torch.float32, device=dev)
                out_amax = next(rows)
                if l == 0 and self.fp_linear_first and layer.cout % 4 == 0 and layer.cout <= 1024:
                    c2 = sparse_channels if sparse_feat is None else sparse_feat.shape[1]
                    c1 = 0 if dense_feat is None else dense_feat.shape[1]
                    la, lb, _ = self._fp_split(fp, layer, c2, c1)
                    s_out = None if carried is not None else \
                        torch.empty((B * n_sparse, layer.cout), dtype=torch.float32, device=dev)
                    in_loader = chain_next or (fuse2 and len(fl) == 3 and
                                               self._fusable(fl[-2], fl[-1], LOAD_INTERP_ADD, EPI_STORE))
                    in_loader = in_loader and self.precision in ("f16x2", "bf16") and len(fl) >= 2
                    if in_loader and fuse2 and not self._fusable(fl[-2], fl[-1], LOAD_INTERP_ADD, EPI_STORE):
                        in_loader = False
                    if carried is not None:
                        s_out, s_amax = carried
                        carried = None
                    else:
                        s_amax = next(rows) if in_loader else None
                        self._gemm("fp%d.0s" % fi, la, B * n_sparse, LOAD_PLAIN, EPI_STORE, relu=False,
                                   out=s_out, ldc=layer.cout, A=sparse_feat, lda=c2, a_amax=sparse_amax,
                                   out_amax=s_amax)
                    y = y_amax = None
                    if lb is not None and fi in shared:
                        y, y_amax = shared.pop(fi)
                    elif lb is not None:
                        y = torch.empty((P, layer.cout), dtype=torch.float32, device=dev)
                        y_amax = next(rows) if in_loader else None
                        self._gemm("fp%d.0d" % fi, lb, P, LOAD_PLAIN, EPI_STORE, relu=False, out=y,
                                   ldc=layer.cout, A=dense_feat, lda=c1, a_amax=dense_amax,
                                   out_amax=y_amax)
                    if in_loader:
                        pending = dict(sparse=s_out, dense=y, C2=layer.cout, N2=n_sparse, N1=n_dense,
                                       nidx=nidx, nw=nw, loader_bias=layer.bias, a_amax=s_amax,
                                       a_amax2=y_amax, a_amax_floor=fp["bias0_max"])
                        continue
                    with _F._timed("interp_add[P=%d,C=%d]" % (P, layer.cout),
                                   P * layer.cout * (8 if y is not None else 4) + P * 24):
                        rc = _cabi.lib().s4g_interp_add_cl_f32(
                            None if y is None else y.data_ptr(), s_out.data_ptr(), nidx.data_ptr(),
                            nw.data_ptr(), layer.bias.data_ptr(), B, n_dense, n_sparse, layer.cout, 1,
                            out.data_ptr(), out_amax.data_ptr(), _F._stream())
                    _cabi.check(rc, "interp_add_cl")
                elif l == 0:
                    c1 = 0 if dense_feat is None else dense_feat.shape[1]
                    self._gemm("fp%d.%d" % (fi, l), layer, P, LOAD_INTERP, EPI_STORE, out=out,
                               ldc=layer.cout, nidx=nidx, nw=nw, sparse=sparse_feat,
                               dense=dense_feat, C2=sparse_feat.shape[1], C1=c1, N2=n_sparse,
                               N1=n_dense, a_amax=sparse_amax, a_amax2=dense_amax,
                               out_amax=out_amax)
                elif pending is not None:
                    self._gemm("fp%d.%d" % (fi, l), layer, P, LOAD_INTERP_ADD, EPI_STORE, out=out,
                               ldc=out.shape[1], out_amax=out_amax, layer2=l2, layer3=l3, **pending)
                    heads0_fused = l3 is not None
                    pending = None
                else:
                    self._gemm("fp%d.%d" % (fi, l), layer, P, LOAD_PLAIN, EPI_STORE, out=out,
                               ldc=out.shape[1], A=x, lda=x.shape[1], a_amax=x_amax,
                               out_amax=out_amax, layer2=l2, layer3=l3)
                    heads0_fused = l3 is not None
                x, x_amax = out, out_amax
            sparse_feat, sparse_amax, n_sparse = x, x_amax, n_dense
            if keep is not None and x is not None and not heads0_fused:
                keep["fp%d" % fi] = x.view(B, n_dense, -1)

        P = B * N0
        x, x_amax = sparse_feat, sparse_amax
        names = ("score", "frame_R", "frame_t", "movable_logits")
        if topk is not None:
            if self.heads_fused is None or heads_pre is None:
                raise NotImplementedError("topk= needs the one-launch heads with the FP tail in front (the shipped widths)")
            return self._heads_topk(heads_pre, B, N0, int(topk), dev)
        if self.heads_fused is not None and (heads_pre is not None or x.shape[1] == 256):
            packed, outs = self._head_outputs(B, N0, dev)
            self._heads(x, x_amax, outs, B, N0, pre=heads_pre)
            return PackedPred(zip(names, outs), packed=packed)
        l0 = self.head_layers[0]
        if not heads0_fused:
            h = torch.empty((P, l0.cout), dtype=torch.float32, device=dev)
            h_amax = next(rows)
            self._gemm("heads.0", l0, P, LOAD_PLAIN, EPI_STORE, out=h, ldc=l0.cout, A=x,
                       lda=x.shape[1], a_amax=x_amax, out_amax=h_amax)
            x, x_amax = h, h_amax
        hl = self.head_layers
        l = 1
        while l < len(hl):
            layer = hl[l]
            l2 = hl[l + 1] if (l + 1 < len(hl) and self._fusable(layer, hl[l + 1])) else None
            l3 = None
            if (l2 is not None and l + 2 < len(hl) and l2.cout == layer.cout and
                    self._fusable(l2, hl[l + 2])):
                l3 = hl[l + 2]
            if l2 is not None and l3 is None and layer.kpad16 != layer.cout:
                l2 = None
            cout = (l3 or l2 or layer).cout
            h = torch.empty((P, layer.groups * cout), dtype=torch.float32, device=dev)
            h_amax = next(rows)
            self._gemm("heads.%d" % l, layer, P, LOAD_PLAIN, EPI_STORE, out=h,
                       ldc=layer.groups * cout, c_gcol=cout, A=x, lda=x.shape[1],
                       a_gcol=layer.cin, a_amax=x_amax, out_amax=h_amax, layer2=l2, layer3=l3,
                       name3="heads.%d" % (l + 2))
            x, x_amax = h, h_amax
            l += 3 if l3 is not None else (2 if l2 is not None else 1)
        names = ("score", "frame_R", "frame_t", "movable_logits")
        packed, outs = self._head_outputs(B, N0, dev)
        starts = [0]
        for c in self.head_channels:
            starts.append(starts[-1] + c)
        if packed is not None:
            cf_ptr = (_fp * 4)(*[packed.data_ptr()] * 4)
            cf_start = (_i32 * 5)(0, *[starts[-1]] * 4)
        else:
            cf_ptr = (_fp * 4)(*[o.data_ptr() for o in outs])
            cf_start = (_i32 * 5)(*starts)
        self._gemm("heads.logits", self.logit_layer, P, LOAD_PLAIN, EPI_CF, relu=False, A=x,
                   lda=x.shape[1], cf_ptr=cf_ptr, cf_start=cf_start,
                   cf_sigmoid_from=self.sigmoid_from, cf_N=N0, a_amax=x_amax)
        return PackedPred(zip(names, outs), packed=packed)

    def _heads_topk(self, pre, B, N0, K, dev):
        K = min(K, N0)
        score = torch.empty((B, self.head_channels[0], N0), dtype=torch.float32, device=dev)
        self._heads(None, None, [score, None, None, None], B, N0, pre=pre, head_mask=1)
        from . import postprocess as _pp
        es = _pp.expected_score(score, "demo")
        sel = torch.topk(es, K, dim=1, largest=True, sorted=True)[1]
        flat = (sel + torch.arange(B, device=dev).view(B, 1) * N0).reshape(-1)
        sub = dict(pre, nidx=pre["nidx"].reshape(B * N0, 3).index_select(0, flat).contiguous(),
                   nw=pre["nw"].reshape(B * N0, 3).index_select(0, flat).contiguous(),
                   dense=None if pre["dense"] is None else pre["dense"].index_select(0, flat).contiguous())
        packed = torch.empty((B, sum(self.head_channels), K), dtype=torch.float32, device=dev)
        outs = list(packed.split(self.head_channels, dim=1))
        outs[0].copy_(torch.gather(score, 2, sel.unsqueeze(1).expand(-1, score.shape[1], -1)))
        self._heads(None, None, outs, B, K, pre=sub, head_mask=0b1110)
        pred = PackedPred(zip(("score", "frame_R", "frame_t", "movable_logits"), outs), packed=packed)
        pred["index"] = sel
        return pred

    def _contact_outputs(self, raw, xyz):
        packed = raw.packed
        B, _, M = packed.shape
        index = raw.get("index")
        N = xyz.shape[2]
        out = torch.empty((B, sum(CONTACT_OUT_CHANNELS), M), dtype=torch.float32, device=packed.device)
        with _F._timed("contact_heads[M=%d]" % M, B * M * 4 * (sum(CONTACT_RAW_CHANNELS) + sum(CONTACT_OUT_CHANNELS) + 3)):
            rc = _cabi.lib().s4g_contact_heads_f32(packed.data_ptr(), xyz.data_ptr(),
                                                   None if index is None else index.data_ptr(), B, N, M,
                                                   out.data_ptr(), _F._stream())
        _cabi.check(rc, "contact_heads")
        pred = PackedPred(zip(HEADS_CONTACT, out.split(CONTACT_OUT_CHANNELS, dim=1)), packed=out)
        if index is not None:
            pred["index"] = index
        return pred

    def _head_outputs(self, B, N0, dev):
        if not self.packed_out and self.kind != "PN2":
            return None, [torch.empty((B, c, N0), dtype=torch.float32, device=dev) for c in self.head_channels]
        packed = torch.empty((B, sum(self.head_channels), N0), dtype=torch.float32, device=dev)
        return packed, list(packed.split(self.head_channels, dim=1))

    @torch.no_grad()
    def submit(self, data_batch, topk=None, keep_feats=False):
        if self.fold_only:
            raise RuntimeError("FusedPointNet2(fold_only=True) holds packed weights only: it cannot run a forward")
        xyz = _F._f32c(data_batch["scene_points"], "scene_points")
        if xyz.dim() != 3 or xyz.size(1) != 3:
            raise RuntimeError("scene_points must be (B, 3, N)")
        dev = xyz.device
        if self.check_finite:
            bad = (~torch.isfinite(xyz)).flatten(1).any(dim=1).nonzero().flatten().tolist()
            if bad:
                raise ValueError("scene_points: non-finite coordinates in scene(s) %s of the batch" % bad)
        _F.OpTimer.begin_pass()
        if self._streams is None or self._streams[0][0].device != dev:
            self._streams = _stream_pool(dev, self.geo_streams, self.dense_streams)
            self._submitted = 0
        gs = self._streams[0][self._submitted % len(self._streams[0])]
        ds = self._streams[1][self._submitted % len(self._streams[1])]
        self._submitted += 1
        with torch.cuda.device(dev):
            cur = torch.cuda.current_stream(dev)
            ev_in = cur.record_event()
            gs.wait_event(ev_in)
            with torch.cuda.stream(gs):
                geo = self._geometry(xyz)
                geo["done"] = gs.record_event()
                if keep_feats:
                    geo["feats"] = {}
            ds.wait_event(ev_in)
            with torch.cuda.stream(ds):
                pred = self._dense(xyz, geo, topk=topk)
                if self.kind == "PN2":
                    pred = self._contact_outputs(pred, xyz)
                ev_out = ds.record_event()
            xyz.record_stream(gs)
            xyz.record_stream(ds)
            for idx, ctr, gidx, gcnt in geo["sa"]:
                for t in (idx, ctr, gidx, gcnt):
                    t.record_stream(ds)
            for t in geo["rel"]:
                for u in (t if isinstance(t, tuple) else (t,)):
                    if u is not None:
                        u.record_stream(ds)
            for nidx, nw in geo["fp"]:
                nidx.record_stream(ds)
                nw.record_stream(ds)
        return Handle(pred, geo, ev_out)

    def graph(self, example_batch):
        return GraphedForward(self, example_batch)

    def __call__(self, data_batch, return_intermediates=False, topk=None):
        h = self.submit(data_batch, topk=topk, keep_feats=return_intermediates)
        pred = h.result()
        if return_intermediates:
            inter = {}
            h.event.synchronize()
            for name, t in h.geo["feats"].items():
                inter["feat_" + name] = t.transpose(1, 2)
            for li, (idx, ctr, gidx, gcnt) in enumerate(h.geo["sa"]):
                inter["fps%d" % li], inter["ball%d" % li], inter["cnt%d" % li] = idx, gidx, gcnt
            for fi, (nidx, nw) in enumerate(h.geo["fp"]):
                inter["nn%d" % fi], inter["nnw%d" % fi] = nidx, nw
            for li, rel in enumerate(h.geo["rel"]):
                if isinstance(rel, tuple):
                    inter["sa%d_rows" % li] = rel[2]
            return pred, inter
        return pred


class PackedPred(dict):

    def __init__(self, items=(), packed=None):
        super().__init__(items)
        self.packed = packed


class GraphedForward:

    def __init__(self, model, example):
        xyz = _F._f32c(example["scene_points"], "scene_points")
        self.static_in = xyz.clone()
        self.model = model
        dev = xyz.device
        side = torch.cuda.Stream(device=dev)
        side.wait_stream(torch.cuda.current_stream(dev))
        with torch.cuda.stream(side):
            for _ in range(2):
                model({"scene_points": self.static_in})
        torch.cuda.current_stream(dev).wait_stream(side)
        torch.cuda.synchronize(dev)
        was = _F.OpTimer.enabled
        _F.OpTimer.enabled = False
        self.graph = torch.cuda.CUDAGraph()
        try:
            with torch.cuda.graph(self.graph):
                self.static_out = model({"scene_points": self.static_in})
        finally:
            _F.OpTimer.enabled = was

    def __call__(self, data_batch):
        xyz = data_batch["scene_points"]
        if tuple(xyz.shape) != tuple(self.static_in.shape):
            raise RuntimeError("graph was recorded for scene_points of shape %s" % (tuple(self.static_in.shape),))
        if xyz.data_ptr() != self.static_in.data_ptr():
            self.static_in.copy_(xyz, non_blocking=True)
        self.graph.replay()
        return self.static_out


class Handle:

    def __init__(self, pred, geo, event):
        self.pred, self.geo, self.event = pred, geo, event

    def result(self):
        cur = torch.cuda.current_stream(next(iter(self.pred.values())).device)
        cur.wait_event(self.event)
        for t in self.pred.values():
            t.record_stream(cur)
        for li, (idx, ctr, gidx, gcnt) in enumerate(self.geo["sa"]):
            for t in (idx, ctr, gidx, gcnt):
                t.record_stream(cur)
        for nidx, nw in self.geo["fp"]:
            nidx.record_stream(cur)
            nw.record_stream(cur)
        return self.pred
```

Before: 2049.

## Split first SA layer into per-point affine and per-centroid term for centred gather

Rewrites the first grouped MLP layer of eligible SA levels as a per-point term and a per-centroid term. The xyz contribution, measured relative to the scene's first point, is folded into the per-point pre-GEMM epilogue, and a new small kernel precomputes the centroid term. A new gather loader then only subtracts the centroid term and applies ReLU, with no per-neighbour xyz work. This removes the per-neighbour xyz reads and the 3-wide dot products from the fused chain. In exchange it adds an extra kernel launch and buffer, forces the pre-GEMM onto the single-chain path, and changes rounding order because the terms are subtracted in fp32 and then split to f16x2.

```diff
diff --git a/include/s4g_ops.h b/include/s4g_ops.h
--- a/include/s4g_ops.h
+++ b/include/s4g_ops.h
@@ -100,6 +100,7 @@
 #define S4G_GEMM_LOAD_GATHER_ADD 4
 #define S4G_GEMM_LOAD_INTERP_ADD 5
 #define S4G_GEMM_LOAD_CHANNEL_FIRST 6
+#define S4G_GEMM_LOAD_GATHER_CENTRED 7
 #define S4G_GEMM_EPI_STORE 0
 #define S4G_GEMM_EPI_MAX 1
 #define S4G_GEMM_EPI_CHANNEL_FIRST 2
@@ -157,6 +158,10 @@
   float *out2;
   int32_t ldc2, split_n;
   float *out_amax2;
+  const float *aff_w;
+  const float *aff_xyz;
+  const float *ctr_term;
+  int32_t aff_N;
   int32_t a_L;
 } s4g_gemm_desc_t;
 
@@ -223,6 +228,9 @@
                           int64_t B, int64_t N, int64_t M, int64_t K, float *rel_pk4,
                           s4g_stream_t stream);
 
+int s4g_centroid_term_f32(const float *xyz_b3n, const float *ctr_b3m, const float *w4, int64_t B, int64_t N,
+                          int64_t M, int64_t C, float *out_bm_c, s4g_stream_t stream);
+
 int s4g_group_rel_xyz_unique_i32(const float *xyz_b3n, const float *ctr_b3m, const int32_t *idx_bmk,
                                  const int32_t *cnt_bm, int64_t B, int64_t N, int64_t M, int64_t K,
                                  float *rel_pk4, int32_t *seg4, int32_t *row_start_bm, int32_t *rows_b,
diff --git a/s4g_release_amd/_cabi.py b/s4g_release_amd/_cabi.py
--- a/s4g_release_amd/_cabi.py
+++ b/s4g_release_amd/_cabi.py
@@ -39,6 +39,7 @@
         ("W3_f16x2_frag", _vp), ("w3_inv_scale", _vp), ("bias3", _vp), ("Cout3", _i32), ("relu3", _i32),
         ("loader_bias", _vp), ("rows_per_scene", _i32), ("rel_xyz4", _vp), ("seg4", _vp), ("seg_rows", _vp),
         ("out2", _vp), ("ldc2", _i32), ("split_n", _i32), ("out_amax2", _vp),
+        ("aff_w", _vp), ("aff_xyz", _vp), ("ctr_term", _vp), ("aff_N", _i32),
         ("a_L", _i32),
     ]
 
@@ -92,6 +93,7 @@
     "s4g_group_points_backward_det_f32": (_int, [_vp, _vp, _i64, _i64, _i64, _i64, _i64, _vp, _vp, _sz, _vp]),
     "s4g_three_interpolate_backward_det_f32": (_int, [_vp, _vp, _vp, _i64, _i64, _i64, _i64, _vp, _vp, _sz, _vp]),
     "s4g_group_rel_xyz_i32": (_int, [_vp, _vp, _vp, _i64, _i64, _i64, _i64, _vp, _vp]),
+    "s4g_centroid_term_f32": (_int, [_vp, _vp, _vp, _i64, _i64, _i64, _i64, _vp, _vp]),
     "s4g_group_rel_xyz_unique_i32": (_int, [_vp, _vp, _vp, _vp, _i64, _i64, _i64, _i64, _vp, _vp, _vp, _vp, _vp]),
     "s4g_expected_score_f32": (_int, [_vp, _i64, _i64, _i64, _vp, _vp, _vp]),
     "s4g_decode_poses_f32": (_int, [_vp, _vp, _vp, _vp, _i64, _i64, _i64, _i64, _vp, _vp, _vp]),
diff --git a/s4g_release_amd/csrc/group.hip b/s4g_release_amd/csrc/group.hip
--- a/s4g_release_amd/csrc/group.hip
+++ b/s4g_release_amd/csrc/group.hip
@@ -182,6 +182,42 @@
               gout[((size_t)b * C + ch) * MK + t]);
 }
 
+__global__ __launch_bounds__(GP_THREADS) void centroid_term_kernel(const float* __restrict__ xyz,
+                                                                   const float* __restrict__ ctr,
+                                                                   const float4* __restrict__ w4, int N, int M, int C4,
+                                                                   float4* __restrict__ out) {
+  const int b = blockIdx.y;
+  const int64_t t = (int64_t)blockIdx.x * GP_THREADS + threadIdx.x;
+  if (t >= (int64_t)M * C4) return;
+  const int m = (int)(t / C4), q = (int)(t - (int64_t)m * C4);
+  const float* x = xyz + (size_t)b * 3 * N;
+  const float* c = ctr + (size_t)b * 3 * M;
+  const float dx = __fsub_rn(c[m], finite_or_zero(x[0]));
+  const float dy = __fsub_rn(c[M + m], finite_or_zero(x[N]));
+  const float dz = __fsub_rn(c[2 * M + m], finite_or_zero(x[2 * (size_t)N]));
+  float r[4];
+#pragma unroll
+  for (int e = 0; e < 4; ++e) {
+    const float4 w = w4[4 * q + e];
+    r[e] = __fmaf_rn(w.x, dx, __fmaf_rn(w.y, dy, __fmul_rn(w.z, dz)));
+  }
+  out[((size_t)b * M + m) * C4 + q] = make_float4(r[0], r[1], r[2], r[3]);
+}
+
+}
+
+extern "C" int s4g_centroid_term_f32(const float* xyz_b3n, const float* ctr_b3m, const float* w4, int64_t B, int64_t N,
+                                     int64_t M, int64_t C, float* out_bm_c, s4g_stream_t stream) {
+  if (B < 0 || N <= 0 || M < 0 || C < 0 || (C & 3) || B > 65535 || N >= (1ll << 31) || M * C >= (1ll << 31))
+    return S4G_EINVAL;
+  if (B == 0 || M == 0 || C == 0) return S4G_OK;
+  if (!xyz_b3n || !ctr_b3m || !w4 || !out_bm_c || (((uintptr_t)w4 | (uintptr_t)out_bm_c) & 15)) return S4G_EINVAL;
+  const int64_t n = M * (C / 4);
+  hipLaunchKernelGGL(s4g::centroid_term_kernel, dim3((unsigned)((n + s4g::GP_THREADS - 1) / s4g::GP_THREADS), (unsigned)B),
+                     dim3(s4g::GP_THREADS), 0, (hipStream_t)stream, xyz_b3n, ctr_b3m, reinterpret_cast<const float4*>(w4),
+                     (int)N, (int)M, (int)(C / 4), reinterpret_cast<float4*>(out_bm_c));
+  S4G_LAUNCH_CHECK();
+  return S4G_OK;
 }
 
 extern "C" int s4g_group_points_f32(const float* in_bcn,
diff --git a/s4g_release_amd/csrc/mlp_gemm.hip b/s4g_release_amd/csrc/mlp_gemm.hip
--- a/s4g_release_amd/csrc/mlp_gemm.hip
+++ b/s4g_release_amd/csrc/mlp_gemm.hip
@@ -19,6 +19,7 @@
 
 enum { LOAD_PLAIN = 0, LOAD_GATHER = 1, LOAD_INTERP = 2, LOAD_GATHER_MLP1 = 3, LOAD_GATHER_ADD = 4,
        LOAD_INTERP_ADD = 5, LOAD_CHANNEL_FIRST = 6,
+       LOAD_GATHER_CENTRED = 7,
        LOAD_REL_MLP1 = 64,
        LOAD_ADD_MFMA0 = 65 };
 enum { EPI_STORE = 0, EPI_MAX = 1, EPI_CHANNEL_FIRST = 2, EPI_MAX_CF = 3 };
@@ -77,6 +78,10 @@
   const float* w_inv_scale3;
   const float* bias3;
   int Cout3, relu3;
+  const float4* aff_w;
+  const float* aff_xyz;
+  int aff_N;
+  const float* ctr_term;
 };
 
 __device__ __forceinline__ float4 f4zero() { return make_float4(0.f, 0.f, 0.f, 0.f); }
@@ -91,6 +96,28 @@
     ++b;
   }
   m = (K & (K - 1)) == 0 ? rem >> (31 - __clz(K)) : rem / K;
+}
+
+__device__ __forceinline__ void plain_row_bi(int N, int p0, int r, int& b, int& i) {
+  const int b0 = __builtin_amdgcn_readfirstlane(p0 / N);
+  i = p0 - b0 * N + r;
+  b = b0;
+  while (i >= N) {
+    i -= N;
+    ++b;
+  }
+}
+
+__device__ __forceinline__ void aff_row_rel(const GemmParams& p, int p0, int r, float& dx, float& dy, float& dz) {
+  int b, i;
+  plain_row_bi(p.aff_N, p0, r, b, i);
+  const float* x = p.aff_xyz + (size_t)b * 3 * p.aff_N;
+  dx = __fsub_rn(x[i], finite_or_zero(x[0]));
+  dy = __fsub_rn(x[p.aff_N + i], finite_or_zero(x[p.aff_N]));
+  dz = __fsub_rn(x[2 * p.aff_N + i], finite_or_zero(x[2 * p.aff_N]));
+}
+__device__ __forceinline__ float aff_add(float v, float wx, float wy, float wz, float wb, float dx, float dy, float dz) {
+  return __fadd_rn(v, __fmaf_rn(wx, dx, __fmaf_rn(wy, dy, __fmaf_rn(wz, dz, wb))));
 }
 
 template <int LOADER, int RPT = 4, int RS = 32>
@@ -969,10 +996,12 @@
   const int wave = t >> 6;
 
   constexpr bool ADD0 = LOADER == LOAD_ADD_MFMA0;
-  constexpr bool ADD_BOUNDS = LOADER == LOAD_GATHER_ADD || LOADER == LOAD_INTERP_ADD || ADD0;
+  constexpr bool CENT = LOADER == LOAD_GATHER_CENTRED;
+  constexpr bool ADD_BOUNDS = LOADER == LOAD_GATHER_ADD || LOADER == LOAD_INTERP_ADD || ADD0 || CENT;
   constexpr bool MFMA0 = LOADER == LOAD_REL_MLP1;
   static_assert(!(MFMA0 || ADD0) || (PL == 2 && KC == 1), "phase 0 on the matrix cores: f16x2, one panel");
-  static_assert(!ADD0 || EPI2 == EPI_MAX, "a wave's 64 rows are one centroid's neighbours");
+  static_assert(!CENT || (PL == 2 && KC == 1), "the centred gather: f16x2, one panel");
+  static_assert(!(ADD0 || CENT) || EPI2 == EPI_MAX, "a wave's 64 rows are one centroid's neighbours");
   constexpr bool SEGMAX = (LOADER == LOAD_GATHER_MLP1 || MFMA0) && EPI2 == EPI_MAX;
   const int tile = blockIdx.x;
   const int p0 = tile * BM;
@@ -1022,10 +1051,47 @@
   ALoader<LOADER, RPT, RS> ld;
   float4 rv0[NRB];
   float4 wv0 = f4zero();
-  constexpr int NKT0 = ADD0 ? K / 32 : 1, RPT0 = ADD0 ? RPT : 1;
+  constexpr int NKT0 = (ADD0 || CENT) ? K / 32 : 1, RPT0 = (ADD0 || CENT) ? RPT : 1;
   float4 fa[NKT0][RPT0];
   constexpr int fstr = K + 4;
-  if constexpr (ADD0) {
+  constexpr int NG0 = CENT ? BM / 64 : 1, NKTT = CENT ? K / 32 : 1;
+  float4 tt[NG0][NKTT];
+  if constexpr (CENT) {
+    const int rows_left = p.P - p0;
+    const __amdgpu_buffer_rsrc_t ridx = __builtin_amdgcn_make_buffer_rsrc(
+        const_cast<int*>(p.gidx + p0), 0, (rows_left < BM ? rows_left : BM) * 4, 0x00020000);
+    const __amdgpu_buffer_rsrc_t rfeat = __builtin_amdgcn_make_buffer_rsrc(
+        const_cast<float*>(p.feat), 0, p.nscenes * p.N * p.Cf * 4, 0x00020000);
+    const __amdgpu_buffer_rsrc_t rterm = __builtin_amdgcn_make_buffer_rsrc(
+        const_cast<float*>(p.ctr_term), 0, (p.P >> 6) * p.Cf * 4, 0x00020000);
+    constexpr uint32_t OOB = 0x80000000u;
+    int jg[RPT];
+#pragma unroll
+    for (int s = 0; s < RPT; ++s) jg[s] = __builtin_amdgcn_raw_buffer_load_b32(ridx, ((t >> 3) + RS * s) * 4, 0, 0);
+#pragma unroll
+    for (int c = 0; c < NG0; ++c) {
+      const uint32_t to = p0 + 64 * c < p.P ? (uint32_t)(((p0 >> 6) + c) * p.Cf + (t & 7) * 4) * 4u : OOB;
+#pragma unroll
+      for (int kt = 0; kt < NKTT; ++kt)
+        tt[c][kt] = __builtin_bit_cast(float4, __builtin_amdgcn_raw_buffer_load_b128(
+                                                   rterm, kt * 32 + (t & 7) * 4 < p.Cin ? to + kt * 128 : OOB, 0, 0));
+    }
+    uint32_t rowoff[RPT];
+#pragma unroll
+    for (int s = 0; s < RPT; ++s) {
+      const int c64 = (RS * s) / 64 * 64;
+      int bc, mc;
+      gather_row_bm(p.M, p.K, p0, c64, bc, mc);
+      bc = __builtin_amdgcn_readfirstlane(bc);
+      rowoff[s] = p0 + c64 < p.P ? (uint32_t)((bc * p.N + jg[s]) * p.Cf + (t & 7) * 4) * 4u : OOB;
+    }
+#pragma unroll
+    for (int kt = 0; kt < NKT0; ++kt)
+#pragma unroll
+      for (int s = 0; s < RPT; ++s)
+        fa[kt][s] = __builtin_bit_cast(float4, __builtin_amdgcn_raw_buffer_load_b128(
+                                                   rfeat, kt * 32 + (t & 7) * 4 < p.Cin ? rowoff[s] + kt * 128 : OOB, 0, 0));
+  } else if constexpr (ADD0) {
     const int rows_left = p.P - p0;
     const __amdgpu_buffer_rsrc_t ridx = __builtin_amdgcn_make_buffer_rsrc(
         const_cast<int*>(p.gidx + p0), 0, (rows_left < BM ? rows_left : BM) * 4, 0x00020000);
@@ -1252,6 +1318,20 @@
           }
         }
     }
+  } else if constexpr (CENT) {
+#pragma unroll
+    for (int kt = 0; kt < NKT0; ++kt)
+#pragma unroll
+      for (int s = 0; s < RPT; ++s) {
+        const float4 f = fa[kt][s], c = tt[(RS * s) / 64][kt];
+        const float4 v = make_float4(fmaxf(__fsub_rn(f.x, c.x), 0.f), fmaxf(__fsub_rn(f.y, c.y), 0.f),
+                                     fmaxf(__fsub_rn(f.z, c.z), 0.f), fmaxf(__fsub_rn(f.w, c.w), 0.f));
+        uint16_t* dst = Ah + ((t >> 3) + RS * s) * astr + kt * 32 + (t & 7) * 4;
+        uint2 h, l;
+        split2_h<false>(v, sa, h, l);
+        *reinterpret_cast<uint2*>(dst) = h;
+        *reinterpret_cast<uint2*>(dst + aplane) = l;
+      }
   } else {
     if (!(S4G_CHAIN_ABLATE & 16)) load_panel(0, std::integral_constant<int, (K / 32) / (NRB / 2)>{});
   }
@@ -1396,6 +1476,37 @@
       float* __restrict__ obase = second ? p.out2 - p.split_n : p.out + p.c_coff;
       const int old = second ? p.ldc2 : p.ldc;
       uint32_t* __restrict__ oamax = second ? p.out_amax2 : p.out_amax;
+      if (p.aff_w && !second) {
+        const float4 aff_wv = p.aff_w[g * p.c_gcol + wc * 64 + lane];
+        float aff_dx[NRB], aff_dy[NRB], aff_dz[NRB];
+#pragma unroll
+        for (int pb = 0; pb < NRB; ++pb) {
+          const int r = wr * WROWS + pb * 32 + li;
+          aff_row_rel(p, p0, p0 + r < p.P ? r : 0, aff_dx[pb], aff_dy[pb], aff_dz[pb]);
+        }
+        __syncthreads();
+        float* ws = smemf + wave * 256;
+        ws[lane] = aff_wv.x;
+        ws[64 + lane] = aff_wv.y;
+        ws[128 + lane] = aff_wv.z;
+        ws[192 + lane] = aff_wv.w;
+#pragma unroll
+        for (int nb = 0; nb < 2; ++nb)
+#pragma unroll
+          for (int j = 0; j < 4; ++j) {
+            const int c = nb * 32 + 8 * j + 4 * lh;
+            const float4 wx = *reinterpret_cast<const float4*>(ws + c), wy = *reinterpret_cast<const float4*>(ws + 64 + c);
+            const float4 wz = *reinterpret_cast<const float4*>(ws + 128 + c), wb = *reinterpret_cast<const float4*>(ws + 192 + c);
+#pragma unroll
+            for (int pb = 0; pb < NRB; ++pb) {
+              const float dx = aff_dx[pb], dy = aff_dy[pb], dz = aff_dz[pb];
+              acc[nb][pb][4 * j] = aff_add(acc[nb][pb][4 * j], wx.x, wy.x, wz.x, wb.x, dx, dy, dz);
+              acc[nb][pb][4 * j + 1] = aff_add(acc[nb][pb][4 * j + 1], wx.y, wy.y, wz.y, wb.y, dx, dy, dz);
+              acc[nb][pb][4 * j + 2] = aff_add(acc[nb][pb][4 * j + 2], wx.z, wy.z, wz.z, wb.z, dx, dy, dz);
+              acc[nb][pb][4 * j + 3] = aff_add(acc[nb][pb][4 * j + 3], wx.w, wy.w, wz.w, wb.w, dx, dy, dz);
+            }
+          }
+      }
 #pragma unroll
       for (int nb = 0; nb < 2; ++nb)
 #pragma unroll
@@ -1713,6 +1824,7 @@
   const int r = C == 128 ? 2 : (C == 256 ? 1 : (C == 512 ? 8 : 0));
   if (r == 0 || Kpad16 <= 0 || Kpad16 % C) return 0;
   const int kc = Kpad16 / C;
+  if (loader == LOAD_GATHER_CENTRED) return epilogue == (int)EPI_MAX && kc == 1;
 #define S4G_FUSED2_Q(L, E, R, KCH) \
   if (loader == L && epilogue == (int)E && r == R && kc == KCH) return 1;
   S4G_FUSED2_LIST(S4G_FUSED2_Q)
@@ -1780,6 +1892,10 @@
   p.bias3 = d->bias3;
   p.Cout3 = d->Cout3;
   p.relu3 = d->relu3;
+  p.aff_w = (const float4*)d->aff_w;
+  p.aff_xyz = d->aff_xyz;
+  p.aff_N = d->aff_N;
+  p.ctr_term = d->ctr_term;
   p.mtiles = (d->P + GM_BM - 1) / GM_BM;
   p.ntiles = (d->Cout + GM_BN - 1) / GM_BN;
   hipStream_t st = (hipStream_t)stream;
@@ -1804,6 +1920,14 @@
         d->K <= 0 || d->M <= 0 || d->N <= 0 || d->groups != 1 || ((uintptr_t)d->mlp1_w & 15) ||
         ((uintptr_t)d->feat & 15))
       return S4G_EINVAL;
+  } else if (d->loader == S4G_GEMM_LOAD_GATHER_CENTRED) {
+    if (!d->gidx || !d->feat || !d->ctr_term || (d->Cin & 3) || d->Cf != d->Cin || d->K <= 0 || d->M <= 0 || d->N <= 0 ||
+        d->groups != 1 || (((uintptr_t)d->feat | (uintptr_t)d->ctr_term) & 15))
+      return S4G_EINVAL;
+    if (!h2 || !d->W2_f16x2_frag || d->epilogue != S4G_GEMM_EPI_MAX || d->K != 64 || (d->P & 63) || d->Kpad16 != d->Cout ||
+        !(d->Cout == 128 || d->Cout == 256 || d->Cout == 512) || d->Cin > d->Cout ||
+        (int64_t)p.nscenes * d->N * d->Cf * 4 >= (1ll << 31) || (int64_t)(d->P >> 6) * d->Cf * 4 >= (1ll << 31))
+      return S4G_EUNSUPPORTED;
   } else if (d->loader == S4G_GEMM_LOAD_INTERP_ADD) {
     if (!d->nidx || !d->nw || !d->sparse || !d->loader_bias || (d->Cin & 3) || d->C2 != d->Cin ||
         d->N1 <= 0 || d->N2 <= 0 || d->groups != 1 ||
@@ -1827,6 +1951,16 @@
         d->groups != 1 || d->split_n <= 0 || (d->split_n & 255) || d->split_n >= d->Cout || (d->Cout & 255) ||
         (d->ldc2 & 3) || ((uintptr_t)d->out2 & 15) || d->c_coff != 0 || (d->ldc & 3) || ((uintptr_t)d->out & 15))
       return S4G_EINVAL;
+  }
+  if (d->aff_w) {
+    const bool bf1_ = d->precision == S4G_GEMM_BF16;
+    if (!(h2 || bf1_) || d->loader != S4G_GEMM_LOAD_PLAIN || d->epilogue != S4G_GEMM_EPI_STORE || d->W2_f16x2_frag ||
+        d->groups != 1 || d->relu || !d->aff_xyz || d->aff_N <= 0 || d->P % d->aff_N || ((uintptr_t)d->aff_w & 15) ||
+        ((d->ldc | d->c_coff | d->c_gcol | d->Cout) & 3) || ((uintptr_t)d->out & 15))
+      return S4G_EINVAL;
+    const int kc_ = d->Kpad16 / 256;
+    if (!d->W_f16x2_frag || d->Cout % 256 || d->Kpad16 % 256 || !(kc_ == 1 || kc_ == 2 || kc_ == 4))
+      return S4G_EUNSUPPORTED;
   }
   if (d->epilogue == S4G_GEMM_EPI_MAX) {
     if (!(d->K == 16 || d->K == 32 || d->K == 64) || d->groups != 1 || !d->out) return S4G_EINVAL;
@@ -1868,6 +2002,10 @@
       return c128   ? launch_mlp_chain<LOAD_ADD_MFMA0, EPI_MAX, 2, 1, 2>(p, d->groups, st)
              : c256 ? launch_mlp_chain<LOAD_ADD_MFMA0, EPI_MAX, 1, 1, 2>(p, d->groups, st)
                     : launch_mlp_chain<LOAD_ADD_MFMA0, EPI_MAX, 8, 1, 2>(p, d->groups, st);
+    if (d->loader == S4G_GEMM_LOAD_GATHER_CENTRED)
+      return c128   ? launch_mlp_chain<LOAD_GATHER_CENTRED, EPI_MAX, 2, 1, 2>(p, d->groups, st)
+             : c256 ? launch_mlp_chain<LOAD_GATHER_CENTRED, EPI_MAX, 1, 1, 2>(p, d->groups, st)
+                    : launch_mlp_chain<LOAD_GATHER_CENTRED, EPI_MAX, 8, 1, 2>(p, d->groups, st);
 #define S4G_FUSED2_CASE(L, E, R, KCH)                                                        \
   if (d->loader == L && (int)d->epilogue == (int)E && (c128 ? 2 : (c256 ? 1 : 8)) == R &&     \
       d->Kpad16 / d->Cout == KCH)                                                             \
@@ -1879,13 +2017,13 @@
   }
   {
     const char* sc_env = s4g::knob("S4G_GEMM_SINGLE_CHAIN");
-    const bool single_chain = !(sc_env && sc_env[0] == '0');
+    const bool single_chain = !(sc_env && sc_env[0] == '0') || d->aff_w;
     const bool bf1 = d->precision == S4G_GEMM_BF16;
     const int kc = d->Kpad16 / 256;
     if (single_chain && (h2 || bf1) && d->loader == S4G_GEMM_LOAD_PLAIN && d->epilogue == S4G_GEMM_EPI_STORE &&
         d->W_f16x2_frag && d->groups == 1 && d->Cout % 256 == 0 && d->Kpad16 % 256 == 0 &&
         (kc == 1 || kc == 2 || kc == 4) && ((d->ldc | d->c_coff) & 3) == 0 && ((uintptr_t)d->out & 15) == 0 &&
-        (d->Cout >= 1024 || d->Kpad16 >= 1024 || (sc_env && sc_env[0] == '1'))) {
+        (d->Cout >= 1024 || d->Kpad16 >= 1024 || (sc_env && sc_env[0] == '1') || d->aff_w)) {
       GemmParams q = p;
       q.Cout = 256;
       q.a_gcol = 0;
diff --git a/s4g_release_amd/csrc/s4g_common.h b/s4g_release_amd/csrc/s4g_common.h
--- a/s4g_release_amd/csrc/s4g_common.h
+++ b/s4g_release_amd/csrc/s4g_common.h
@@ -39,6 +39,10 @@
   if (e != hipSuccess) return (int)e;
   if (slot) cache.bytes[dev].store((int)lds_bytes, std::memory_order_relaxed);
   return 0;
+}
+
+__device__ __forceinline__ float finite_or_zero(float v) {
+  return (__float_as_uint(v) & 0x7f800000u) == 0x7f800000u ? 0.f : v;
 }
 
 template <bool FMAD>
diff --git a/s4g_release_amd/fused.py b/s4g_release_amd/fused.py
--- a/s4g_release_amd/fused.py
+++ b/s4g_release_amd/fused.py
@@ -12,6 +12,7 @@
 HeadsDesc = _cabi.HeadsDesc
 
 LOAD_PLAIN, LOAD_GATHER, LOAD_INTERP, LOAD_GATHER_MLP1, LOAD_GATHER_ADD, LOAD_INTERP_ADD = 0, 1, 2, 3, 4, 5
+LOAD_GATHER_CENTRED = 7
 EPI_STORE, EPI_MAX, EPI_CF = 0, 1, 2
 
 NETWORK_KINDS = {(9, 4): "PN2_CLS", (6, 3): "PN2"}
@@ -436,6 +437,25 @@
         _cabi.check(rc, "ball_query_i32")
         return idx, cnt
 
+    def _sa_centred(self, sa):
+        layers = sa["layers"]
+        la = None if sa["pre"] is None else sa["pre"]["la"]
+        if la is None or la.Wfrag is None or la.cout % 256 or la.kpad16 not in (256, 512, 1024):
+            return False
+        return (self.precision == "f16x2" and sa["pre"] is not None and sa["K"] == 64 and len(layers) == 3 and
+                layers[-1].groups == 1 and layers[-2].kpad16 == layers[-2].cout and
+                self._fusable(layers[-2], layers[-1], LOAD_GATHER_CENTRED, EPI_MAX))
+
+    def _centroid_term(self, xyz, ctr, w1):
+        B, _, N = xyz.shape
+        M, C = ctr.shape[2], w1.shape[0]
+        out = torch.empty((B * M, C), dtype=torch.float32, device=xyz.device)
+        with _F._timed("centroid_term[M=%d,C=%d]" % (M, C), B * M * (12 + 4 * C)):
+            rc = _cabi.lib().s4g_centroid_term_f32(xyz.data_ptr(), ctr.data_ptr(), w1.data_ptr(), B, N, M, C,
+                                                   out.data_ptr(), _F._stream())
+        _cabi.check(rc, "centroid_term_f32")
+        return out
+
     def _group_rel_xyz(self, xyz, ctr, gidx):
         B, _, N = xyz.shape
         _, M, K = gidx.shape
@@ -495,7 +515,7 @@
 
     def _geometry(self, xyz):
         B, _, N0 = xyz.shape
-        geo = dict(level_xyz=[xyz], level_n=[N0], sa=[], fp=[], sa_events=[], rel=[])
+        geo = dict(level_xyz=[xyz], level_n=[N0], sa=[], fp=[], sa_events=[], rel=[], cterm=[])
         n_cur = N0
         run = None
         for li, sa in enumerate(self.sa):
@@ -519,6 +539,8 @@
                 if rel is None:
                     rel = self._group_rel_xyz(geo["level_xyz"][-1], ctr, gidx)
             geo["rel"].append(rel)
+            centred = self._sa_centred(sa) and 4 * B * max(n_cur, M) * sa["layers"][0].cout < 2 ** 31
+            geo["cterm"].append(self._centroid_term(geo["level_xyz"][-1], ctr, sa["pre"]["w1"]) if centred else None)
             geo["sa_events"].append(torch.cuda.current_stream().record_event())
             if dist is not None and all(self.sa[l + 1]["M"] <= self.sa[l]["M"] for l in range(1, len(self.sa) - 1)):
                 run = self._fps_prefix_check(ctr, dist, self.sa[1]["M"])
@@ -559,6 +581,8 @@
                             LOAD_GATHER_ADD if (lp == 1 and pre is not None) else LOAD_PLAIN)
             fuse2 = (K == 64 and len(layers) >= 3 and layers[-1].groups == 1 and
                      self._fusable(layers[-2], layers[-1], first_loader, EPI_MAX))
+            cterm = geo["cterm"][li]
+            aff = {} if cterm is None else dict(aff_w=pre["w1"], aff_xyz=level_xyz[li], aff_N=level_n[li])
             if pre is not None:
                 fpre = torch.empty((B * level_n[li], layers[0].cout), dtype=torch.float32, device=dev)
                 fpre_amax = next(rows)
@@ -570,12 +594,12 @@
                     self._gemm("sa%d.0f|fp%d.0d" % (li, fi), mg[0], B * level_n[li], LOAD_PLAIN, EPI_STORE,
                                relu=False, out=fpre, ldc=layers[0].cout, A=feat, lda=feat.shape[1],
                                a_amax=feat_amax, out_amax=fpre_amax, out2=y, ldc2=mg[1].cout,
-                               split_n=layers[0].cout, out_amax2=y_amax)
+                               split_n=layers[0].cout, out_amax2=y_amax, **aff)
                     shared[fi] = (y, y_amax)
                 else:
                     self._gemm("sa%d.0f" % li, pre["la"], B * level_n[li], LOAD_PLAIN, EPI_STORE, relu=False,
                                out=fpre, ldc=layers[0].cout, A=feat, lda=feat.shape[1], a_amax=feat_amax,
-                               out_amax=fpre_amax)
+                               out_amax=fpre_amax, **aff)
             for l, layer in enumerate(layers):
                 if l == 0 and (sa["mlp1"] is not None or pre is not None):
                     continue
@@ -600,6 +624,12 @@
                     elif rel is not None:
                         kw.update(rel_xyz4=rel)
                     loader = LOAD_GATHER_MLP1
+                elif l == 1 and cterm is not None:
+                    if l2 is None:
+                        raise RuntimeError("centroid terms without the fused chain that consumes them")
+                    kw.update(gidx=gidx, feat=fpre, Cf=layers[0].cout, ctr_term=cterm, N=level_n[li], M=M,
+                              a_amax=fpre_amax, a_amax_floor=pre["bound"])
+                    loader = LOAD_GATHER_CENTRED
                 elif l == 1 and pre is not None:
                     kw.update(gidx=gidx, feat=fpre, Cf=layers[0].cout, xyz=level_xyz[li], ctr=ctr,
                               N=level_n[li], M=M, mlp1_w=pre["w1"], a_amax=fpre_amax,
@@ -872,6 +902,9 @@
                 for u in (t if isinstance(t, tuple) else (t,)):
                     if u is not None:
                         u.record_stream(ds)
+            for t in geo["cterm"]:
+                if t is not None:
+                    t.record_stream(ds)
             for nidx, nw in geo["fp"]:
                 nidx.record_stream(ds)
                 nw.record_stream(ds)
```

Result: no change. 2062 (median of 6 runs) (+0.6%).
